# Intelligent-Microsystems-Lab/SNNQuantPrune

Measured on AMD Instinct MI355X. Metric: samples/sec/node (DVS128 T=20, 4-bit/90%-pruned), higher is better.
Workload: dtype fp6*fp4->f32 (integer-exact); 1 GPU; C3 topology: 3x(qconv3x3+BN+LIF+pool2) + qdense(32768->110)+LIF + vote, DVS128 128x128x2, T=20, bits 4/4/4/4, 90% pruned; batch_per_gpu=1024, global_batch=1024, frames=20, parallelism=dp1 (batch-sharded, all-gather logits)

## Files before the change

include/snnqp.h:

```cpp
#ifndef SNNQP_H_
#define SNNQP_H_

#include <stdint.h>

#ifdef __cplusplus
extern "C" {
#endif

typedef void *snnqp_stream_t;

enum {
  SNNQP_OK = 0,
  SNNQP_EINVAL = -1,
  SNNQP_EUNSUPPORTED = -2,
  SNNQP_EHIP = -3
};

enum { SNNQP_F32 = 0, SNNQP_U8 = 1, SNNQP_BITS = 2, SNNQP_EV1 = 3, SNNQP_EV4 = 4 };
enum { SNNQP_W_F32 = 0, SNNQP_W_I8 = 1 };
enum {
  SNNQP_NEURON_NONE = 0,
  SNNQP_NEURON_MULTI_STEP_LIF = 1,
  SNNQP_NEURON_PARAMETRIC_LEAKY_IF = 2,
  SNNQP_NEURON_LIF = 3
};
enum {
  SNNQP_SURR_FAST_SIGMOID = 0,
  SNNQP_SURR_ATAN = 1,
  SNNQP_SURR_SLAYER = 2,
  SNNQP_SURR_SMOOTH_STEP = 3,
  SNNQP_SURR_PIECEWISE_LINEAR = 4
};
enum {
  SNNQP_Q_DUQ = 0,
  SNNQP_Q_UNIFORM_STATIC = 1,
  SNNQP_Q_PARAMETRIC_D = 2,
  SNNQP_Q_PARAMETRIC_D_XMAX = 3
};
enum { SNNQP_IMPL_AUTO = 0, SNNQP_IMPL_GENERIC = 1, SNNQP_IMPL_MFMA = 2 };

enum {
  SNNQP_FLAG_CODE_OVERFLOW = 1,
  SNNQP_FLAG_MASK_NOT_BINARY = 2,
  SNNQP_FLAG_NOT_INTEGER = 4,
  SNNQP_FLAG_GT_ONE = 8,
  SNNQP_FLAG_GT_127 = 16,
  SNNQP_FLAG_GT_15 = 32
};

typedef struct {
  int32_t wtype;
  const void *w;
  float L;
  float m;
  int32_t abs_sum_max;
  int32_t code_max;
  const int32_t *col_sum;
  const void *wt_fp6;
  uint32_t min_current_bits;
  int32_t ch_stack_max;
  const int32_t *ch_slots;
  int32_t wt_cin;
} snnqp_weight_t;

#define SNNQP_BN_MEAN_ZERO 1
#define SNNQP_BN_BIAS_ZERO 2
#define SNNQP_BN_MUL_UNIFORM 4
typedef struct {
  const float *mean;
  const float *mul;
  const float *bias;
  int32_t flags;
} snnqp_bn_t;

typedef struct {
  int32_t kind;
  float k;
  float v_threshold;
  float v_reset;
  const float *decay;
} snnqp_neuron_t;

typedef struct {
  int32_t H, W, Cin, Cout;
  int32_t KH, KW;
  int32_t stride_h, stride_w;
  int32_t pad_h_lo, pad_h_hi, pad_w_lo, pad_w_hi;
  int32_t in_dil_h, in_dil_w;
  int32_t k_dil_h, k_dil_w;
  int32_t groups;
} snnqp_conv_geom_t;

typedef struct {
  int32_t D, H, W, Cin, Cout;
  int32_t KD, KH, KW;
  int32_t stride[3];
  int32_t pad_lo[3], pad_hi[3];
  int32_t in_dil[3];
  int32_t k_dil[3];
  int32_t groups;
} snnqp_conv3d_geom_t;

#define SNNQP_VERSION 505
int snnqp_version(void);
const char *snnqp_last_error(void);
const char *snnqp_build_flags(void);

int snnqp_conv_out_shape(const snnqp_conv_geom_t *g, int32_t *OH, int32_t *OW);

int snnqp_quantize(int kind, const float *w, const float *mask, int64_t n,
                   int bits, float p0, float p1, float *fq_out,
                   int8_t *codes_out, int32_t *flags, snnqp_stream_t stream);
int snnqp_quantize_ex(int kind, const float *w, const float *mask, int64_t n,
                      int bits, int sign, float p0, float p1, float *fq_out,
                      int8_t *codes_out, int32_t *flags, snnqp_stream_t stream);

int snnqp_pack_codes_mfma(const int8_t *w, int64_t K, int32_t N, int32_t Npad,
                          int8_t *wt, snnqp_stream_t stream);

int snnqp_pack_codes_fp6(const int8_t *w, int64_t K, int32_t N, int32_t Npad, void *wt6,
                         snnqp_stream_t stream);

int snnqp_inspect_f32(const float *x, int64_t n, int32_t *flags,
                      snnqp_stream_t stream);
int snnqp_inspect_u8(const uint8_t *x, int64_t n, int32_t *flags,
                     snnqp_stream_t stream);
int snnqp_f32_to_u8(const float *x, uint8_t *y, int64_t n,
                    snnqp_stream_t stream);
int snnqp_narrow_f32(const float *x, uint8_t *y, int64_t n, int32_t *flags,
                     snnqp_stream_t stream);
int snnqp_pack_frames(const uint8_t *x, int64_t frames, int32_t H, int32_t W, int fmt,
                      void *y, int32_t *flags, snnqp_stream_t stream);
int snnqp_unpack_frames(const void *x, int fmt, int64_t frames, int32_t H, int32_t W,
                        uint8_t *y, snnqp_stream_t stream);
int snnqp_pack_frames_checked(const void *x, int in_type, int64_t frames, int32_t H, int32_t W,
                              uint32_t *y, int32_t *flags, snnqp_stream_t stream);
int snnqp_pack_bits(const void *x, int in_type, int64_t rows, int32_t C,
                    uint32_t *bits, snnqp_stream_t stream);
int snnqp_pack_bits_checked(const void *x, int in_type, int64_t rows, int32_t C,
                            uint32_t *bits, int32_t *flags, snnqp_stream_t stream);
int snnqp_unpack_bits(const uint32_t *bits, int64_t rows, int32_t C, float *y,
                      snnqp_stream_t stream);

int snnqp_conv_forward(const void *x, int in_type, int64_t NB,
                       const snnqp_conv_geom_t *g, const snnqp_weight_t *w,
                       float *y, int32_t *acc, snnqp_stream_t stream);
int snnqp_conv_forward_if(const int32_t *pred, const void *x, int in_type, int64_t NB,
                          const snnqp_conv_geom_t *g, const snnqp_weight_t *w, float *y,
                          snnqp_stream_t stream);

int snnqp_conv3d_out_shape(const snnqp_conv3d_geom_t *g, int32_t *OD, int32_t *OH, int32_t *OW);
int snnqp_conv3d_lif_forward(const int32_t *pred, const void *x, int in_type, int64_t x_stride_t,
                             int64_t x_stride_b, int32_t T, int32_t B,
                             const snnqp_conv3d_geom_t *g, const snnqp_weight_t *w,
                             const snnqp_bn_t *bn, const snnqp_neuron_t *nrn, const float *u0,
                             float *u_out, void *s_out, int s_type, snnqp_stream_t stream);

int64_t snnqp_conv_gated_packed_bytes(int32_t Cin, int32_t Cout);
int snnqp_pack_codes_gated(const int8_t *w, int32_t Cin, int32_t Cout, void *packed,
                           snnqp_stream_t stream);
int64_t snnqp_conv_gated_packed_bytes_ex(int32_t Cin, int32_t Cout, int32_t code_max);
int snnqp_pack_codes_gated_ex(const int8_t *w, int32_t Cin, int32_t Cout, int32_t code_max,
                              void *packed, snnqp_stream_t stream);
int snnqp_conv_gated_forward(const uint32_t *s, const float *gate, int64_t NB,
                             const snnqp_conv_geom_t *g, const snnqp_weight_t *w,
                             const void *packed, float *y, snnqp_stream_t stream);

int64_t snnqp_dense_gated_packed_bytes(int32_t C, int32_t N);
int snnqp_pack_codes_dense_gated(const int8_t *w, int32_t C, int32_t HW, int32_t N, void *packed,
                                 snnqp_stream_t stream);
int64_t snnqp_dense_gated_packed_bytes_ex(int32_t C, int32_t N, int32_t code_max);
int snnqp_pack_codes_dense_gated_ex(const int8_t *w, int32_t C, int32_t HW, int32_t N, int32_t code_max,
                                    void *packed, snnqp_stream_t stream);
int snnqp_dense_gated_forward(const uint32_t *s, const float *gate, int64_t NB, int32_t HW,
                              int32_t C, int32_t N, const snnqp_weight_t *w,
                              const void *packed, float *y, snnqp_stream_t stream);

int snnqp_conv_lif_forward(const void *x, int in_type, int64_t x_stride_t,
                           int64_t x_stride_b, int32_t T, int32_t B,
                           const snnqp_conv_geom_t *g, const snnqp_weight_t *w,
                           const int8_t *wt, const snnqp_bn_t *bn,
                           const snnqp_neuron_t *nrn, const float *u0,
                           float *u_out, void *s_out, int s_type, int pool,
                           int impl, int x_max, int32_t *x_seen, int32_t *x_flags,
                           snnqp_stream_t stream);

int snnqp_conv_lif_forward_pred(const int32_t *pred, const void *x, int in_type, int64_t x_stride_t,
                                int64_t x_stride_b, int32_t T, int32_t B,
                                const snnqp_conv_geom_t *g, const snnqp_weight_t *w,
                                const int8_t *wt, const snnqp_bn_t *bn,
                                const snnqp_neuron_t *nrn, const float *u0,
                                float *u_out, void *s_out, int s_type, int pool,
                                int x_max, int32_t *x_seen, int32_t *x_flags,
                                snnqp_stream_t stream);

int snnqp_conv_lif_forward_if(const int32_t *pred, const void *x, int in_type, int64_t x_stride_t,
                              int64_t x_stride_b, int32_t T, int32_t B,
                              const snnqp_conv_geom_t *g, const snnqp_weight_t *w,
                              const snnqp_bn_t *bn, const snnqp_neuron_t *nrn, const float *u0,
                              float *u_out, void *s_out, int s_type, int pool,
                              snnqp_stream_t stream);

int snnqp_fallback_counts(int64_t *conv_blocks, int64_t *dense_blocks, char *reason,
                          int32_t reason_len, int reset);

#define SNNQP_STATUS_QUEUE_CORRUPT 1u
#define SNNQP_STATUS_TICKET 2u
#define SNNQP_STATUS_BOUND 4u
int snnqp_device_status(int device, uint32_t *codes, int reset);
int snnqp_workqueue_capture_mark(int device, int64_t *mark);
int snnqp_workqueue_capture_release(int device, int64_t mark_begin, int64_t mark_end);
int snnqp_workqueue_stats(int64_t *captured_static, int64_t *busy_static,
                          int64_t *dequant_fallbacks, int reset);
int snnqp_debug_workqueue_poke(int device, int64_t mark, int word, uint32_t value);

#define SNNQP_DQ_ARITH 1
#define SNNQP_DQ_ONE 2
#define SNNQP_DQ_TABLE 3
int snnqp_conv_dequant_form(const snnqp_weight_t *w, const snnqp_neuron_t *nrn);

int snnqp_current_min(const snnqp_weight_t *w, const snnqp_bn_t *bn, int32_t bound,
                      int32_t Cout, uint32_t *out_bits, snnqp_stream_t stream);

int snnqp_dense_lif_forward(const void *x, int in_type, int64_t x_stride_t,
                            int64_t x_stride_b, int32_t T, int32_t B, int32_t K,
                            int32_t N, const snnqp_weight_t *w,
                            const int8_t *wt, const snnqp_bn_t *bn,
                            const snnqp_neuron_t *nrn, const float *u0,
                            float *u_out, void *s_out, int s_type, int impl,
                            snnqp_stream_t stream);

int64_t snnqp_dense_workspace_bytes(int in_type, int32_t T, int32_t B, int32_t K, int32_t N,
                                    const snnqp_weight_t *w);
int snnqp_dense_lif_forward_ws(const void *x, int in_type, int64_t x_stride_t,
                               int64_t x_stride_b, int32_t T, int32_t B, int32_t K,
                               int32_t N, const snnqp_weight_t *w,
                               const int8_t *wt, const snnqp_bn_t *bn,
                               const snnqp_neuron_t *nrn, const float *u0,
                               float *u_out, void *s_out, int s_type, int impl,
                               int32_t *x_flags, void *ws, int64_t ws_bytes, snnqp_stream_t stream);
int snnqp_dense_lif_forward_if(const int32_t *pred, const void *x, int in_type, int64_t x_stride_t,
                               int64_t x_stride_b, int32_t T, int32_t B, int32_t K, int32_t N,
                               const snnqp_weight_t *w, const snnqp_bn_t *bn,
                               const snnqp_neuron_t *nrn, const float *u0, float *u_out,
                               void *s_out, int s_type, snnqp_stream_t stream);

int64_t snnqp_dense_head_workspace_bytes(int32_t T, int32_t B, int32_t N1);
int snnqp_dense_head_forward(const void *x, int in_type, int64_t x_stride_t,
                             int64_t x_stride_b, int32_t T, int32_t B, int32_t K,
                             int32_t N1, const snnqp_weight_t *w1, const int8_t *wt1,
                             const snnqp_neuron_t *nrn1, int32_t N2,
                             const snnqp_weight_t *w2, const int8_t *wt2,
                             const snnqp_neuron_t *nrn2, int32_t group,
                             uint32_t *s1_out, uint32_t *s2_out, float *logits,
                             int32_t *x_flags, void *ws, int64_t ws_bytes, snnqp_stream_t stream);

int snnqp_lif_forward(const float *x, int32_t T, int64_t R, int32_t C,
                      const snnqp_bn_t *bn, const snnqp_neuron_t *nrn,
                      const float *u0, float *u_out, void *s_out, int s_type,
                      snnqp_stream_t stream);

int snnqp_batchnorm_forward(const float *x, int64_t rows, int32_t C,
                            const snnqp_bn_t *bn, float *y,
                            snnqp_stream_t stream);

int snnqp_maxpool2x2(const void *x, int type, int64_t NB, int32_t H, int32_t W,
                     int32_t C, void *y, snnqp_stream_t stream);

int snnqp_spatial_mean(const void *x, int type, int64_t NB, int32_t HW, int32_t C,
                       float *y, snnqp_stream_t stream);
int snnqp_sigmoid_gate(const float *a, const float *b, int64_t n, float *g,
                       snnqp_stream_t stream);
int snnqp_apply_gate(const void *x, int type, const float *g, int64_t NB, int32_t HW,
                     int32_t C, float *y, snnqp_stream_t stream);

int snnqp_events_to_frames(const int32_t *ex, const int32_t *ey, const int32_t *ep,
                           int64_t N, int32_t T, int32_t H, int32_t W, float scale,
                           int32_t *counts, uint8_t *frames_u8, snnqp_stream_t stream);
int snnqp_density(const void *x, int type, int64_t NB, int64_t n, int32_t C, int32_t *nnz,
                  snnqp_stream_t stream);

int snnqp_vote(const void *s, int type, int32_t T, int32_t B, int32_t N,
               int32_t group, float *logits, snnqp_stream_t stream);
int snnqp_vote_if(const int32_t *pred, const void *s, int type, int32_t T, int32_t B, int32_t N,
                  int32_t group, float *logits, snnqp_stream_t stream);

int snnqp_scatter_spike_channels(const uint32_t *s, int64_t npix, int32_t cin, const int32_t *map,
                                 int32_t cout, uint32_t *out, snnqp_stream_t stream);

int snnqp_lif_forward_save(const float *x, int32_t T, int64_t R, int32_t C,
                           const snnqp_neuron_t *nrn, float *h_out, float *s_out,
                           snnqp_stream_t stream);
int snnqp_lif_backward(const float *h, const float *gs, const float *glogits, int32_t group,
                       int32_t T, int64_t R, int32_t C, const snnqp_neuron_t *nrn,
                       int surrogate, float *gI, snnqp_stream_t stream);
int snnqp_dense_weight_grad(const float *x, const float *gI, int64_t M, int32_t K, int32_t N,
                            float *gw, snnqp_stream_t stream);
int snnqp_dense_input_grad(const float *gI, const float *w, const float *mask, int64_t M,
                           int32_t K, int32_t N, float *gx, snnqp_stream_t stream);

#ifdef __cplusplus
}
#endif
#endif
```

snnquantprune_amd/_lib.py:

```python

from __future__ import annotations

import ctypes
import os
from ctypes import (POINTER, Structure, c_char_p, c_float, c_int, c_int8,
                    c_int32, c_uint32, c_int64, c_void_p)

_HERE = os.path.dirname(os.path.abspath(__file__))
LIB_PATH = os.path.join(_HERE, "csrc", "libsnnqp.so")

ABI_VERSION = 505

F32, U8, BITS, EV1, EV4 = 0, 1, 2, 3, 4
W_F32, W_I8 = 0, 1
NEURON_NONE, NEURON_MULTI_STEP_LIF, NEURON_PARAMETRIC_LEAKY_IF, NEURON_LIF = 0, 1, 2, 3
SURR_FAST_SIGMOID, SURR_ATAN, SURR_SLAYER, SURR_SMOOTH_STEP, SURR_PIECEWISE_LINEAR = 0, 1, 2, 3, 4
Q_DUQ, Q_UNIFORM_STATIC, Q_PARAMETRIC_D, Q_PARAMETRIC_D_XMAX = 0, 1, 2, 3
IMPL_AUTO, IMPL_GENERIC, IMPL_MFMA = 0, 1, 2
FLAG_CODE_OVERFLOW, FLAG_MASK_NOT_BINARY = 1, 2
FLAG_NOT_INTEGER, FLAG_GT_ONE, FLAG_GT_127, FLAG_GT_15 = 4, 8, 16, 32
OK, EINVAL, EUNSUPPORTED, EHIP = 0, -1, -2, -3
STATUS_QUEUE_CORRUPT, STATUS_TICKET, STATUS_BOUND = 1, 2, 4


class WeightT(Structure):
  _fields_ = [("wtype", c_int32), ("w", c_void_p), ("L", c_float), ("m", c_float),
              ("abs_sum_max", c_int32), ("code_max", c_int32), ("col_sum", c_void_p),
              ("wt_fp6", c_void_p), ("min_current_bits", c_uint32), ("ch_stack_max", c_int32),
              ("ch_slots", c_void_p), ("wt_cin", c_int32)]


BN_MEAN_ZERO, BN_BIAS_ZERO, BN_MUL_UNIFORM = 1, 2, 4


class BnT(Structure):
  _fields_ = [("mean", c_void_p), ("mul", c_void_p), ("bias", c_void_p), ("flags", c_int32)]


class NeuronT(Structure):
  _fields_ = [("kind", c_int32), ("k", c_float), ("v_threshold", c_float),
              ("v_reset", c_float), ("decay", c_void_p)]


class ConvGeomT(Structure):
  _fields_ = [(n, c_int32) for n in (
      "H", "W", "Cin", "Cout", "KH", "KW", "stride_h", "stride_w",
      "pad_h_lo", "pad_h_hi", "pad_w_lo", "pad_w_hi",
      "in_dil_h", "in_dil_w", "k_dil_h", "k_dil_w", "groups")]


class Conv3dGeomT(Structure):
  _fields_ = ([(n, c_int32) for n in ("D", "H", "W", "Cin", "Cout", "KD", "KH", "KW")]
              + [(n, c_int32 * 3) for n in ("stride", "pad_lo", "pad_hi", "in_dil", "k_dil")]
              + [("groups", c_int32)])


_PROTOTYPES = {
    "snnqp_version": (c_int, []),
    "snnqp_last_error": (c_char_p, []),
    "snnqp_build_flags": (c_char_p, []),
    "snnqp_conv_out_shape": (c_int, [POINTER(ConvGeomT), POINTER(c_int32),
                                     POINTER(c_int32)]),
    "snnqp_quantize": (c_int, [c_int, c_void_p, c_void_p, c_int64, c_int, c_float,
                               c_float, c_void_p, c_void_p, c_void_p, c_void_p]),
    "snnqp_quantize_ex": (c_int, [c_int, c_void_p, c_void_p, c_int64, c_int, c_int, c_float,
                                  c_float, c_void_p, c_void_p, c_void_p, c_void_p]),
    "snnqp_pack_codes_mfma": (c_int, [c_void_p, c_int64, c_int32, c_int32, c_void_p,
                                      c_void_p]),
    "snnqp_pack_codes_fp6": (c_int, [c_void_p, c_int64, c_int32, c_int32, c_void_p, c_void_p]),
    "snnqp_inspect_f32": (c_int, [c_void_p, c_int64, c_void_p, c_void_p]),
    "snnqp_inspect_u8": (c_int, [c_void_p, c_int64, c_void_p, c_void_p]),
    "snnqp_f32_to_u8": (c_int, [c_void_p, c_void_p, c_int64, c_void_p]),
    "snnqp_narrow_f32": (c_int, [c_void_p, c_void_p, c_int64, c_void_p, c_void_p]),
    "snnqp_pack_frames": (c_int, [c_void_p, c_int64, c_int32, c_int32, c_int, c_void_p, c_void_p,
                                  c_void_p]),
    "snnqp_unpack_frames": (c_int, [c_void_p, c_int, c_int64, c_int32, c_int32, c_void_p,
                                    c_void_p]),
    "snnqp_pack_bits": (c_int, [c_void_p, c_int, c_int64, c_int32, c_void_p,
                                c_void_p]),
    "snnqp_pack_bits_checked": (c_int, [c_void_p, c_int, c_int64, c_int32, c_void_p, c_void_p,
                                        c_void_p]),
    "snnqp_unpack_bits": (c_int, [c_void_p, c_int64, c_int32, c_void_p, c_void_p]),
    "snnqp_conv_forward": (c_int, [c_void_p, c_int, c_int64, POINTER(ConvGeomT),
                                   POINTER(WeightT), c_void_p, c_void_p, c_void_p]),
    "snnqp_conv_forward_if": (c_int, [c_void_p, c_void_p, c_int, c_int64, POINTER(ConvGeomT),
                                      POINTER(WeightT), c_void_p, c_void_p]),
    "snnqp_conv3d_out_shape": (c_int, [POINTER(Conv3dGeomT), POINTER(c_int32), POINTER(c_int32),
                                       POINTER(c_int32)]),
    "snnqp_conv3d_lif_forward": (c_int, [
        c_void_p, c_void_p, c_int, c_int64, c_int64, c_int32, c_int32, POINTER(Conv3dGeomT),
        POINTER(WeightT), POINTER(BnT), POINTER(NeuronT), c_void_p, c_void_p, c_void_p, c_int, c_void_p]),
    "snnqp_conv_gated_packed_bytes": (c_int64, [c_int32, c_int32]),
    "snnqp_pack_codes_gated": (c_int, [c_void_p, c_int32, c_int32, c_void_p, c_void_p]),
    "snnqp_conv_gated_packed_bytes_ex": (c_int64, [c_int32, c_int32, c_int32]),
    "snnqp_pack_codes_gated_ex": (c_int, [c_void_p, c_int32, c_int32, c_int32, c_void_p, c_void_p]),
    "snnqp_conv_gated_forward": (c_int, [c_void_p, c_void_p, c_int64, POINTER(ConvGeomT),
                                         POINTER(WeightT), c_void_p, c_void_p, c_void_p]),
    "snnqp_dense_gated_packed_bytes": (c_int64, [c_int32, c_int32]),
    "snnqp_pack_codes_dense_gated": (c_int, [c_void_p, c_int32, c_int32, c_int32, c_void_p, c_void_p]),
    "snnqp_dense_gated_packed_bytes_ex": (c_int64, [c_int32, c_int32, c_int32]),
    "snnqp_pack_codes_dense_gated_ex": (c_int, [c_void_p, c_int32, c_int32, c_int32, c_int32, c_void_p, c_void_p]),
    "snnqp_dense_gated_forward": (c_int, [c_void_p, c_void_p, c_int64, c_int32, c_int32, c_int32,
                                          POINTER(WeightT), c_void_p, c_void_p, c_void_p]),
    "snnqp_conv_lif_forward": (c_int, [
        c_void_p, c_int, c_int64, c_int64, c_int32, c_int32, POINTER(ConvGeomT),
        POINTER(WeightT), c_void_p, POINTER(BnT), POINTER(NeuronT), c_void_p,
        c_void_p, c_void_p, c_int, c_int, c_int, c_int, c_void_p, c_void_p, c_void_p]),
    "snnqp_conv_lif_forward_pred": (c_int, [
        c_void_p, c_void_p, c_int, c_int64, c_int64, c_int32, c_int32, POINTER(ConvGeomT),
        POINTER(WeightT), c_void_p, POINTER(BnT), POINTER(NeuronT), c_void_p,
        c_void_p, c_void_p, c_int, c_int, c_int, c_void_p, c_void_p, c_void_p]),
    "snnqp_pack_frames_checked": (c_int, [c_void_p, c_int, c_int64, c_int32, c_int32, c_void_p, c_void_p,
                                          c_void_p]),
    "snnqp_conv_lif_forward_if": (c_int, [
        c_void_p, c_void_p, c_int, c_int64, c_int64, c_int32, c_int32, POINTER(ConvGeomT),
        POINTER(WeightT), POINTER(BnT), POINTER(NeuronT), c_void_p, c_void_p, c_void_p, c_int, c_int,
        c_void_p]),
    "snnqp_dense_lif_forward_if": (c_int, [
        c_void_p, c_void_p, c_int, c_int64, c_int64, c_int32, c_int32, c_int32, c_int32,
        POINTER(WeightT), POINTER(BnT), POINTER(NeuronT), c_void_p, c_void_p, c_void_p, c_int,
        c_void_p]),
    "snnqp_dense_lif_forward": (c_int, [
        c_void_p, c_int, c_int64, c_int64, c_int32, c_int32, c_int32, c_int32,
        POINTER(WeightT), c_void_p, POINTER(BnT), POINTER(NeuronT), c_void_p,
        c_void_p, c_void_p, c_int, c_int, c_void_p]),
    "snnqp_dense_workspace_bytes": (c_int64, [c_int, c_int32, c_int32, c_int32, c_int32, POINTER(WeightT)]),
    "snnqp_dense_lif_forward_ws": (c_int, [
        c_void_p, c_int, c_int64, c_int64, c_int32, c_int32, c_int32, c_int32,
        POINTER(WeightT), c_void_p, POINTER(BnT), POINTER(NeuronT), c_void_p,
        c_void_p, c_void_p, c_int, c_int, c_void_p, c_void_p, c_int64, c_void_p]),
    "snnqp_dense_head_workspace_bytes": (c_int64, [c_int32, c_int32, c_int32]),
    "snnqp_dense_head_forward": (c_int, [
        c_void_p, c_int, c_int64, c_int64, c_int32, c_int32, c_int32, c_int32, POINTER(WeightT),
        c_void_p, POINTER(NeuronT), c_int32, POINTER(WeightT), c_void_p, POINTER(NeuronT), c_int32,
        c_void_p, c_void_p, c_void_p, c_void_p, c_void_p, c_int64, c_void_p]),
    "snnqp_device_status": (c_int, [c_int, POINTER(c_uint32), c_int]),
    "snnqp_workqueue_capture_mark": (c_int, [c_int, POINTER(c_int64)]),
    "snnqp_workqueue_capture_release": (c_int, [c_int, c_int64, c_int64]),
    "snnqp_workqueue_stats": (c_int, [POINTER(c_int64), POINTER(c_int64), POINTER(c_int64), c_int]),
    "snnqp_debug_workqueue_poke": (c_int, [c_int, c_int64, c_int, c_uint32]),
    "snnqp_fallback_counts": (c_int, [POINTER(c_int64), POINTER(c_int64), c_char_p, c_int32, c_int]),
    "snnqp_conv_dequant_form": (c_int, [POINTER(WeightT), POINTER(NeuronT)]),
    "snnqp_current_min": (c_int, [POINTER(WeightT), POINTER(BnT), c_int32, c_int32, c_void_p, c_void_p]),
    "snnqp_lif_forward": (c_int, [c_void_p, c_int32, c_int64, c_int32, POINTER(BnT),
                                  POINTER(NeuronT), c_void_p, c_void_p, c_void_p,
                                  c_int, c_void_p]),
    "snnqp_batchnorm_forward": (c_int, [c_void_p, c_int64, c_int32, POINTER(BnT),
                                        c_void_p, c_void_p]),
    "snnqp_maxpool2x2": (c_int, [c_void_p, c_int, c_int64, c_int32, c_int32, c_int32,
                                 c_void_p, c_void_p]),
    "snnqp_spatial_mean": (c_int, [c_void_p, c_int, c_int64, c_int32, c_int32, c_void_p,
                                   c_void_p]),
    "snnqp_sigmoid_gate": (c_int, [c_void_p, c_void_p, c_int64, c_void_p, c_void_p]),
    "snnqp_apply_gate": (c_int, [c_void_p, c_int, c_void_p, c_int64, c_int32, c_int32,
                                 c_void_p, c_void_p]),
    "snnqp_events_to_frames": (c_int, [c_void_p, c_void_p, c_void_p, c_int64, c_int32, c_int32,
                                       c_int32, c_float, c_void_p, c_void_p, c_void_p]),
    "snnqp_density": (c_int, [c_void_p, c_int, c_int64, c_int64, c_int32, c_void_p, c_void_p]),
    "snnqp_vote": (c_int, [c_void_p, c_int, c_int32, c_int32, c_int32, c_int32,
                           c_void_p, c_void_p]),
    "snnqp_vote_if": (c_int, [c_void_p, c_void_p, c_int, c_int32, c_int32, c_int32, c_int32,
                              c_void_p, c_void_p]),
    "snnqp_scatter_spike_channels": (c_int, [c_void_p, c_int64, c_int32, c_void_p, c_int32,
                                             c_void_p, c_void_p]),
    "snnqp_lif_forward_save": (c_int, [c_void_p, c_int32, c_int64, c_int32, POINTER(NeuronT),
                                       c_void_p, c_void_p, c_void_p]),
    "snnqp_lif_backward": (c_int, [c_void_p, c_void_p, c_void_p, c_int32, c_int32, c_int64,
                                   c_int32, POINTER(NeuronT), c_int, c_void_p, c_void_p]),
    "snnqp_dense_weight_grad": (c_int, [c_void_p, c_void_p, c_int64, c_int32, c_int32, c_void_p,
                                        c_void_p]),
    "snnqp_dense_input_grad": (c_int, [c_void_p, c_void_p, c_void_p, c_int64, c_int32, c_int32,
                                       c_void_p, c_void_p]),
}

EXPORTED_SYMBOLS = tuple(_PROTOTYPES)

_lib = None


class SnnqpError(RuntimeError):
  def __init__(self, code, msg):
    super().__init__("libsnnqp error %d: %s" % (code, msg))
    self.code = code


def lib():
  global _lib
  if _lib is None:
    path = os.environ.get("SNNQP_DIAG_LIB") or LIB_PATH
    if not os.path.exists(path):
      raise ImportError(
          "HIP extension %s not found: build it with `python __graft_entry__.py` "
          "(hipcc --offload-arch=gfx950); there is no CPU fallback." % path)
    import torch
    handle = ctypes.CDLL(path)
    if path != LIB_PATH:
      import sys
      print("snnquantprune_amd: DIAGNOSTIC library %s" % path, file=sys.stderr)
    for name, (res, args) in _PROTOTYPES.items():
      fn = getattr(handle, name)
      fn.restype = res
      fn.argtypes = args
    if handle.snnqp_version() != ABI_VERSION:
      raise ImportError(
          "%s has ABI version %d, this binding was written against %d (include/snnqp.h "
          "SNNQP_VERSION): rebuild it with `python __graft_entry__.py`"
          % (path, handle.snnqp_version(), ABI_VERSION))
    _lib = handle
  return _lib


def build_flags() -> str:
  return lib().snnqp_build_flags().decode("utf-8", "replace")


def require_product_build():
  flags = build_flags()
  if flags or os.environ.get("SNNQP_DIAG_LIB"):
    raise RuntimeError("libsnnqp is a diagnostic build (%s): rebuild with "
                       "`python snnquantprune_amd/csrc/build.py --force`" % (flags or "SNNQP_DIAG_LIB"))


def check(rc):
  if rc != 0:
    raise SnnqpError(rc, lib().snnqp_last_error().decode("utf-8", "replace"))
```

snnquantprune_amd/csrc/conv3x3_u8c2.hip:

```cpp
#include <atomic>
#include <map>
#include <mutex>
#include <tuple>
#include <type_traits>
#include <utility>

#include <vector>

#include "conv_tile.h"

namespace snnqp {

constexpr int HROW2 = 24;
constexpr int HCOPY2 = HALO * HROW2;
constexpr int HCONST2 = 2 * HCOPY2;
constexpr int HIMG2 = 496;
constexpr int TCHUNK = 32;
constexpr int U8C2_WPS = 4;
constexpr int STG_N = TCHUNK / 2;

typedef int v2i_a4 __attribute__((ext_vector_type(2), aligned(4)));
typedef __attribute__((address_space(3))) const v2i_a4 lds_cv2i_t;

__host__ __device__ inline int u8c2_table_bytes(int lutm, int bound, int rows) {
  const int b = lutm == LUT_CHANNEL ? rows * 128 : lutm == LUT_SHARED ? (2 * bound + 2) * 4 : 0;
  return (b + 15) & ~15;
}

#ifndef SNNQP_U8C2_EV1_WPS
#define SNNQP_U8C2_EV1_WPS 5
#endif
#ifndef SNNQP_U8C2_ONE_WPS
#define SNNQP_U8C2_ONE_WPS 4
#endif
#ifndef SNNQP_U8C2_EV1_ONE_WPS
#define SNNQP_U8C2_EV1_ONE_WPS 6
#endif
template <int NF, bool POOL, int LUTM, int IN, bool ONE>
constexpr int u8c2_waves() {
  if (IN == SNNQP_EV1 && ONE && LUTM == LUT_CHANNEL && NF == NF_MUL0 && POOL) return SNNQP_U8C2_EV1_ONE_WPS;
  if (IN == SNNQP_EV1) return SNNQP_U8C2_EV1_WPS;
  return ONE ? SNNQP_U8C2_ONE_WPS : U8C2_WPS;
}
template <int NF, bool POOL, int LUTM, int IN = SNNQP_U8, bool ONE = false>
__global__ void __launch_bounds__(256, (u8c2_waves<NF, POOL, LUTM, IN, ONE>()))
conv3x3_u8c2_kernel(ConvMfmaArgs a) {
  constexpr int FL = OutStage<POOL>::FL;
  constexpr bool EV1 = IN == SNNQP_EV1;
  constexpr bool EV4 = IN == SNNQP_EV4;
  constexpr bool F32IN = IN == SNNQP_F32;
  static_assert(TCHUNK % FL == 0, "flush period must divide the staging chunk");
  if constexpr (!EV1) {
    if (a.pred && *(const volatile int32_t *)a.pred == 0) return;
  }
  extern __shared__ __attribute__((aligned(16))) uint8_t lds[];
  const int tc = a.tchunk;
  const int lut_off = tc * HIMG2;
  uint32_t *obuf = (uint32_t *)(lds + lut_off + u8c2_table_bytes(LUTM, a.lut_bound, a.lut_rows));
  const int tid = threadIdx.x, lane = tid & 63;
  const int wave = __builtin_amdgcn_readfirstlane(tid >> 6);
  const int n = lane & 31, h = lane >> 5;
  const int cout_base = blockIdx.y * 128 + wave * 32;
  const bool wave_on = cout_base < a.Cout;
  const int cout = wave_on ? cout_base + n : n;
  const int cpar = cout < a.Cout ? cout : a.Cout - 1;
  const uint32_t cmask = chan_mask(cout_base, a.Cout);
  uint32_t *wgw = obuf + OutStage<POOL>::BYTES / 4;
  if (tid == 0) { wgw[0] = 0x7F800000u; wgw[1] = 0u; }
  typedef int v2i_a8 __attribute__((ext_vector_type(2)));
  v2i_a8 *xtab = (v2i_a8 *)(wgw + 4);
  if (EV1) {
    const uint32_t one = LUTM == LUT_CHANNEL ? 16u : LUTM == LUT_SHARED ? 4u : 0x81u;
    const uint32_t zero = LUTM == LUT_NONE ? 0x80u : 0u;
    uint32_t e[2] = {0, 0};
#pragma unroll
    for (int j = 0; j < 8; ++j) e[j >> 2] |= (((uint32_t)tid >> j) & 1u ? one : zero) << (8 * (j & 3));
    xtab[tid] = v2i_a8{(int)e[0], (int)e[1]};
  }
  if (LUTM != LUT_NONE) lds_barrier();
  if (LUTM == LUT_SHARED) {
    build_lut((float *)(lds + lut_off), a.lut_bound, a.dq, tid);
    if (NF == NF_MUL0) {
      lds_barrier();
      atomicMin(wgw, lut_bn_min_bits((const float *)(lds + lut_off), a.lut_bound, a.bn,
                                     blockIdx.y * 128, a.Cout, tid, 256));
    }
  }
  int ch_row0 = 0, ch_col = 0;
  if (LUTM == LUT_CHANNEL) {
    int pos = 0, neg = 0;
#pragma unroll
    for (int j = 0; j < 16; ++j) {
      const int k = 16 * h + j, dy = k >> 3, b = k & 7;
      if (k < 24 && b < 6 && wave_on && cout < a.Cout) {
        const int code = a.w[(int64_t)(6 * dy + b) * a.Cout + cout];
        pos += code > 0 ? code : 0;
        neg += code < 0 ? -code : 0;
      }
    }
    pos += __shfl_xor(pos, 32);
    neg += __shfl_xor(neg, 32);
    uint32_t *scr = obuf;
    int slot = 4 * n + wave;
    if (a.ch_slots) slot = a.ch_slots[blockIdx.y * 128 + wave * 32 + n] & 127;
    if (h == 0) {
      scr[slot] = (uint32_t)((pos + neg) * a.x_limit + 1);
      scr[128 + wave * 32 + n] = (uint32_t)(neg * a.x_limit);
      scr[256 + wave * 32 + n] = (uint32_t)slot;
    }
    lds_barrier();
    ch_col = slot >> 2;
    const int start = lut_column_start(scr, slot);
    int total = 0;
#pragma unroll
    for (int k = 0; k < 4; ++k) total += (int)scr[(slot & ~3) + k];
    ch_row0 = start + neg * a.x_limit;
    if (total > a.lut_rows && a.status) *(volatile uint32_t *)a.status = SNNQP_STATUS_BOUND;
    const uint32_t mb = build_lut_channel((float *)(lds + lut_off), scr, a.lut_rows, a.dq, a.bn,
                                          blockIdx.y * 128, a.Cout, tid);
    atomicMin(wgw, mb);
    lds_barrier();
  }
  if (tid < tc) {
    *(uint32_t *)(lds + tid * HIMG2 + HCONST2) = 0x7F7F7F7Fu;
    *(uint32_t *)(lds + tid * HIMG2 + HCONST2 + 4) = 0x00000001u;
  }

  float acc_off = 0.0f;
  v4i bf, bfg;
  {
    int bias = 0;
    if (LUTM == LUT_SHARED) bias = (int)lds_addr(lds) + lut_off + 4 * a.lut_bound;
    if (LUTM == LUT_CHANNEL)
      bias = (int)lds_addr(lds) + lut_off + 4 * (ch_row0 * 32 + ch_col);
    int q = bias / 127;
    const int r = bias - 127 * q;
    int wsum = 0;
    int v[4], vg[4];
#pragma unroll
    for (int d = 0; d < 4; ++d) {
      uint32_t pk = 0, pkg = 0;
#pragma unroll
      for (int j = 0; j < 4; ++j) {
        const int k = 16 * h + 4 * d + j;
        uint32_t bv = 0, bg = 0;
        if (k < 24) {
          const int dy = k >> 3, b = k & 7;
          if (b < 6 && cout < a.Cout) {
            const int code = a.w[(int64_t)(6 * dy + b) * a.Cout + cout];
            wsum += code;
            bg = (uint8_t)code;
            bv = (uint8_t)(LUTM == LUT_CHANNEL ? code * 8 : code);
          }
        } else if (k < 28) {
          const int part = q < 127 ? q : 127;
          q -= part;
          bv = (uint32_t)part;
        } else if (k == 28) {
          bv = (uint32_t)r;
        }
        pk |= bv << (8 * j);
        pkg |= bg << (8 * j);
      }
      v[d] = (int)pk;
      vg[d] = (int)pkg;
    }
    bf = v4i{v[0], v[1], v[2], v[3]};
    bfg = v4i{vg[0], vg[1], vg[2], vg[3]};
    acc_off = 128.0f * (float)(wsum + __shfl_xor(wsum, 32));
  }

  LaneConsts lc = {0.f, 1.f, 0.f, 0.f, a.nrn.vr};
  if (a.bn.mean) { lc.bmean = a.bn.mean[cpar]; lc.bmul = a.bn.mul[cpar]; lc.bbias = a.bn.bias[cpar]; }
  if (a.nrn.kind == SNNQP_NEURON_LIF) lc.dec = a.nrn.decay[cpar];

  const int ty = ((n >> 2) & 1) | ((n >> 4) << 1);
  const int tx = (n & 3) | (((n >> 3) & 1) << 2);
  const int cpy = tx & 1;
  const int px0 = (int)lds_addr(lds) + cpy * HCOPY2 + 2 * tx + 2 * cpy;
  int offA[2], offB[2];
#pragma unroll
  for (int tl = 0; tl < 2; ++tl) {
    offA[tl] = px0 + (ty + 4 * tl + (h ? 2 : 0)) * HROW2;
    offB[tl] = h ? (int)lds_addr(lds) + HCONST2 : px0 + (ty + 4 * tl + 1) * HROW2;
  }
  const uint8_t *xb = (const uint8_t *)a.x;
  const int ob0 = out_pix<POOL>(0, lane) * 4 + wave;
  const int ob1 = out_pix<POOL>(1, lane) * 4 + wave;
  const bool store_lane = POOL ? lane < 8 : lane < 32;
  uint32_t seen = 0;
  uint32_t hist[6] = {0, 0, 0, 0, 0, 0};
  const int s_pix = tid & 127;
  const bool s_task = s_pix < HALO * HALO;
  const int s_half = __builtin_amdgcn_readfirstlane(tid >> 7);
  const int s_dst = (s_pix / HALO) * HROW2 + (s_pix % HALO) * 2;

  PatchWalk pw(a);
  int r = __builtin_amdgcn_readfirstlane((int)pw.first);
  uint32_t processed = 0;
  while (r < (int)pw.count) {
    ++processed;
    int claimed = 0;
    if (pw.queue && tid == 0) claimed = (int)pw.claim();
    int b, y0, x0;
    pw.decode(a, r, b, y0, x0);

    float u[2][16];
    if constexpr (!ONE) {
      if (a.u0 && wave_on) u_io<true>(u, a, b, y0, x0, cout, h);
      else zero_u(u);
    }
    uint32_t pseen = 0;
    const int s_gy = y0 + s_pix / HALO - 1, s_gx = x0 + s_pix % HALO - 1;
    const bool s_valid = s_task && s_gy >= 0 && s_gy < a.H && s_gx >= 0 && s_gx < a.W;
    const uint32_t s_off = s_valid ? (uint32_t)(s_gy * a.W + s_gx) * (EV4 ? 1u : F32IN ? 8u : 2u) : 0u;
    const uint8_t *s_frames = xb + (int64_t)b * a.xs_b * (F32IN ? 4 : 1);
    const uint32_t e_lead = x0 > 0 ? 2u : 0u;
    const int e_hi = min(HALO - 1, a.W - x0);
    const uint32_t e_colmask = ((1u << (2 * (e_hi + 1))) - 1u) & ~((1u << (2 - (int)e_lead)) - 1u);
    const uint32_t e_fwords = (uint32_t)(((int64_t)a.H * a.W * 2 + 31) >> 5);
    const uint32_t *e_frames = (const uint32_t *)a.x + (int64_t)b * a.xs_b;

    for (int t0 = 0; t0 < a.T; t0 += tc) {
      const int nt = min(tc, a.T - t0);
      bool general = LUTM == LUT_NONE;
      if constexpr (EV1) {
        lds_barrier();
        for (int task = tid; task < nt * HALO; task += 256) {
          const int tt = task / HALO, hy = task - tt * HALO;
          const int gy = y0 + hy - 1;
          const bool rv = gy >= 0 && gy < a.H;
          const uint32_t start = (uint32_t)((rv ? gy : 0) * a.W + x0) * 2u - e_lead;
          const uint32_t wi = start >> 5;
          const uint32_t *f = e_frames + (int64_t)(t0 + tt) * a.xs_t;
          const uint32_t lo = f[wi], hi = f[min(wi + 1u, e_fwords - 1u)];
          uint32_t v = __builtin_amdgcn_alignbit(hi, lo, start & 31u);
          v = (v << (2u - e_lead)) & (rv ? e_colmask : 0u);
          const v2i_a8 d0 = xtab[v & 0xFFu], d1 = xtab[(v >> 8) & 0xFFu], d2 = xtab[(v >> 16) & 0xFu];
          uint8_t *row = lds + tt * HIMG2 + hy * HROW2;
          *(v2i_a8 *)row = d0;
          *(v2i_a8 *)(row + 8) = d1;
          *(v2i_a8 *)(row + 16) = d2;
          const uint32_t q0 = (uint32_t)d0.x, q1 = (uint32_t)d0.y, q2 = (uint32_t)d1.x,
                         q3 = (uint32_t)d1.y, q4 = (uint32_t)d2.x, q5 = (uint32_t)d2.y;
          uint8_t *row1 = row + HCOPY2;
          *(v2i_a8 *)row1 = v2i_a8{(int)(q0 << 16), (int)__builtin_amdgcn_alignbit(q1, q0, 16)};
          *(v2i_a8 *)(row1 + 8) = v2i_a8{(int)__builtin_amdgcn_alignbit(q2, q1, 16),
                                         (int)__builtin_amdgcn_alignbit(q3, q2, 16)};
          *(v2i_a8 *)(row1 + 16) = v2i_a8{(int)__builtin_amdgcn_alignbit(q4, q3, 16),
                                          (int)__builtin_amdgcn_alignbit(q5, q4, 16)};
        }
        lds_barrier();
      } else {
      uint32_t v[STG_N];
      uint32_t mx = 0;
      if constexpr (F32IN) {
        uint32_t fbad = 0;
#pragma unroll
        for (int r0 = 0; r0 < STG_N; r0 += STG_N / 2) {
          typedef float f2v __attribute__((ext_vector_type(2)));
          f2v raw[STG_N / 2];
#pragma unroll
          for (int i = r0; i < r0 + STG_N / 2; ++i) {
            const int tt = 2 * i + s_half;
            raw[i - r0] = f2v{0.0f, 0.0f};
            if (tt < nt) raw[i - r0] = *(const f2v *)(s_frames + (int64_t)(t0 + tt) * a.xs_t * 4 + s_off);
          }
#pragma unroll
          for (int i = r0; i < r0 + STG_N / 2; ++i) {
            const f2v f = raw[i - r0];
            const uint32_t ua = __float2uint_rz(f.x), ub = __float2uint_rz(f.y);
            fbad |= __float_as_uint(__uint2float_rn(ua) - f.x) | __float_as_uint(__uint2float_rn(ub) - f.y);
            fbad |= (ua | ub) >> 8;
            v[i] = (ua & 0xFFu) | ((ub & 0xFFu) << 8);
          }
        }
        fbad = s_valid ? fbad : 0u;
        if (__ballot(fbad != 0u) != 0ull && lane == 0 && a.x_flags) atomicOr(a.x_flags, SNNQP_FLAG_NOT_INTEGER);
      } else {
#pragma unroll
      for (int i = 0; i < STG_N; ++i) {
        const int tt = 2 * i + s_half;
        v[i] = 0;
        if (tt < nt) {
          if constexpr (EV4) {
            const uint32_t pb = *(s_frames + (int64_t)(t0 + tt) * a.xs_t + s_off);
            v[i] = (pb | (pb << 4)) & 0x0F0Fu;
          } else {
            v[i] = *(const uint16_t *)(s_frames + (int64_t)(t0 + tt) * a.xs_t + s_off);
          }
        }
      }
      }
#pragma unroll
      for (int i = 0; i < STG_N; ++i) {
        v[i] = s_valid ? v[i] : 0u;
        mx = max(mx, max(v[i] & 0xFFu, v[i] >> 8));
      }
#pragma unroll
      for (int off = 32; off > 0; off >>= 1) mx = max(mx, (uint32_t)__shfl_xor((int)mx, off));
      if (tid == 0) wgw[1] = 0u;
      lds_barrier();
      if (s_task) {
#pragma unroll
        for (int i = 0; i < STG_N; ++i) {
          const int tt = 2 * i + s_half;
          if (tt < nt) {
            const uint16_t val = (uint16_t)(LUTM == LUT_NONE      ? v[i] ^ 0x8080u
                                            : LUTM == LUT_CHANNEL ? v[i] << 4
                                                                  : v[i] << 2);
            uint8_t *p = lds + tt * HIMG2 + s_dst;
            *(uint16_t *)p = val;
            *(uint16_t *)(p + HCOPY2 + 2) = val;
          }
        }
      }
      if (lane == 0 && mx != 0) atomicMax(&wgw[1], mx);
      lds_barrier();
      const uint32_t cmax = (uint32_t)__builtin_amdgcn_readfirstlane((int)wgw[1]);
      seen = max(seen, cmax);
      pseen = max(pseen, cmax);
      hist[0] += cmax <= 1u;
      hist[1] += cmax == 2u;
      hist[2] += cmax > 2u && cmax <= 7u;
      hist[3] += cmax > 7u && cmax <= 31u;
      hist[4] += cmax > 31u;
      hist[5] += cmax == 3u;
      general = LUTM == LUT_NONE || cmax > (uint32_t)a.x_limit;
      if (LUTM != LUT_NONE && general) {
        if (s_task) {
#pragma unroll 1
          for (int tt = s_half; tt < nt; tt += 2) {
            uint32_t w2 = 0;
            if (s_valid) {
              if constexpr (F32IN) {
                typedef float f2v __attribute__((ext_vector_type(2)));
                const f2v f = *(const f2v *)(s_frames + (int64_t)(t0 + tt) * a.xs_t * 4 + s_off);
                w2 = (__float2uint_rz(f.x) & 0xFFu) | ((__float2uint_rz(f.y) & 0xFFu) << 8);
              } else if constexpr (EV4) {
                const uint32_t pb = *(s_frames + (int64_t)(t0 + tt) * a.xs_t + s_off);
                w2 = (pb | (pb << 4)) & 0x0F0Fu;
              } else {
                w2 = *(const uint16_t *)(s_frames + (int64_t)(t0 + tt) * a.xs_t + s_off);
              }
            }
            const uint16_t val = (uint16_t)(w2 ^ 0x8080u);
            uint8_t *p = lds + tt * HIMG2 + s_dst;
            *(uint16_t *)p = val;
            *(uint16_t *)(p + HCOPY2 + 2) = val;
          }
        }
        lds_barrier();
      }
      }
      auto run_chunk = [&](auto mode_tag, auto fma_tag) {
      constexpr int MODE = decltype(mode_tag)::value;
      constexpr bool FMA = decltype(fma_tag)::value;
      constexpr bool OFFS = MODE == LUT_NONE;
      const v4i bw = OFFS ? bfg : bf;
      for (int tf = 0; tf < nt; tf += FL) {
        const int nf = min(FL, nt - tf);
#pragma unroll 1
        for (int tt = tf; tt < (wave_on ? tf + nf : tf); ++tt) {
          const uint32_t img = (uint32_t)(tt * HIMG2);
          uint32_t words[2];
#pragma unroll
          for (int tl = 0; tl < 2; ++tl) {
            const v2i_a4 lo = *(lds_cv2i_t *)(uintptr_t)(img + (uint32_t)offA[0] + (uint32_t)(tl * 4 * HROW2));
            const v2i_a4 hi = *(lds_cv2i_t *)(uintptr_t)(img + (uint32_t)offB[tl]);
            v16i acc = splat16(0);
            acc = __builtin_amdgcn_mfma_i32_32x32x32_i8(v4i{lo.x, lo.y, hi.x, hi.y}, bw, acc,
                                                        0, 0, 0);
            if constexpr (u8c2_waves<NF, POOL, LUTM, IN, ONE>() >= 6)
              words[tl] = tile_epilogue_halves<NF, POOL, MODE, FMA, OFFS>(acc, u[tl], a.dq, lc, a.nrn,
                                                                            lane, acc_off);
            else
              words[tl] = tile_epilogue<NF, POOL, MODE, FMA, OFFS>(acc, u[tl], a.dq, lc, a.nrn,
                                                                     lane, acc_off);
          }
          if (store_lane) {
            uint32_t *o = obuf + ((t0 + tt) % FL) * (OutStage<POOL>::NPIX * 4);
            o[ob0] = words[0] & cmask;
            o[ob0 + (POOL ? 32 : 128)] = words[1] & cmask;
          }
        }
        lds_barrier();
        flush_out<POOL>(obuf, a, t0 + tf, nf, b, y0, x0, tid);
        lds_barrier();
      }
      };
      if constexpr (ONE) zero_u(u);
      if (general) {
        run_chunk(std::integral_constant<int, LUT_NONE>{}, std::false_type{});
      } else if constexpr (LUTM != LUT_NONE) {
        const bool fma_ok = NF == NF_MUL0 && pseen <= (uint32_t)a.x_limit &&
                            lif_fma_is_exact(wgw[0], a.nrn.k_log2, a.T, a.u0 != nullptr);
        if (fma_ok) run_chunk(std::integral_constant<int, LUTM>{}, std::true_type{});
        else run_chunk(std::integral_constant<int, LUTM>{}, std::false_type{});
      }
      if constexpr (ONE) break;
    }
    if (!ONE && a.u_out && wave_on) u_io<false>(u, a, b, y0, x0, cout, h);
    int r_next = r + (int)pw.stride;
    if (pw.queue) {
      if (tid == 0) wgw[2] = (uint32_t)claimed;
      lds_barrier();
      r_next = __builtin_amdgcn_readfirstlane((int)wgw[2]);
    }
    r = r_next;
  }
  if (a.x_seen && tid == 0) {
    if (seen != 0) atomicMax(a.x_seen, seen);
#pragma unroll
    for (int k = 0; k < 6; ++k)
      if (hist[k] != 0) atomicAdd((uint32_t *)a.x_seen + 1 + k, hist[k]);
  }
  if (pw.queue && tid == 0) pw.finish(processed, a.npatch, a.status);
}


__global__ void __launch_bounds__(256)
current_min_kernel(Dequant dq, BnP bn, int bound, int Cout, uint32_t *out) {
  const int c = blockIdx.x * 64 + (threadIdx.x & 63);
  uint32_t mb = 0x7F800000u;
  if (c < Cout) {
    float mean = 0.f, mul = 1.f, bias = 0.f;
    if (bn.mean) { mean = bn.mean[c]; mul = bn.mul[c]; bias = bn.bias[c]; }
    for (int i = (int)(threadIdx.x >> 6) + 4 * (int)blockIdx.y - bound; i <= bound; i += 4 * (int)gridDim.y) {
      float x = dequant_acc_nb(i, dq) - mean;
      x = x * mul;
      x = x + bias;
      const uint32_t b = __float_as_uint(x) & 0x7FFFFFFFu;
      if (b != 0 && b < mb) mb = b;
    }
  }
  for (int off = 32; off > 0; off >>= 1) {
    const uint32_t o = (uint32_t)__shfl_xor((int)mb, off);
    mb = o < mb ? o : mb;
  }
  if ((threadIdx.x & 63) == 0 && mb != 0x7F800000u) atomicMin(out, mb);
}

namespace {
struct SchedPool {
  uint32_t *words = nullptr;
  hipEvent_t busy[SCHED_SLOTS] = {};
  bool has_event[SCHED_SLOTS] = {};
  bool retired[SCHED_SLOTS] = {};
  unsigned next = 0;
  unsigned next_capture = 0;
  std::vector<int> capture_log;
  std::vector<int> capture_free;
};
std::atomic<int64_t> g_static_captured{0}, g_static_busy{0};
std::mutex g_sched_mu;
SchedPool g_sched[64];

struct DeviceGuard {
  int prev = -1;
  bool ok = true;
  explicit DeviceGuard(int dev) {
    int cur = -1;
    if (hipGetDevice(&cur) != hipSuccess) { (void)hipGetLastError(); ok = false; return; }
    if (cur == dev) return;
    if (hipSetDevice(dev) != hipSuccess) { (void)hipGetLastError(); ok = false; return; }
    prev = cur;
  }
  ~DeviceGuard() {
    if (prev >= 0 && hipSetDevice(prev) != hipSuccess) (void)hipGetLastError();
  }
};
}

uint32_t *sched_acquire(hipStream_t st, int *dev_out, int *slot_out) {
  int dev = 0;
  hipStreamCaptureStatus cap = hipStreamCaptureStatusNone;
  if (hipStreamIsCapturing(st, &cap) != hipSuccess) { (void)hipGetLastError(); return nullptr; }
  const bool capturing = cap != hipStreamCaptureStatusNone;
  hipDevice_t sdev;
  if (hipStreamGetDevice(st, &sdev) == hipSuccess) dev = (int)sdev;
  else if (hipGetDevice(&dev) != hipSuccess) return nullptr;
  if (dev < 0 || dev >= 64) return nullptr;
  std::lock_guard<std::mutex> lock(g_sched_mu);
  SchedPool &p = g_sched[dev];
  if (capturing) {
    if (!p.words) { g_static_captured.fetch_add(1, std::memory_order_relaxed); return nullptr; }
    int slot;
    if (!p.capture_free.empty()) {
      slot = p.capture_free.back();
      p.capture_free.pop_back();
    } else if (p.next_capture < (unsigned)SCHED_CAPTURE_SLOTS) {
      slot = SCHED_SLOTS + (int)p.next_capture++;
    } else {
      g_static_captured.fetch_add(1, std::memory_order_relaxed);
      return nullptr;
    }
    p.capture_log.push_back(slot);
    *dev_out = dev;
    *slot_out = slot;
    return p.words + (size_t)slot * SCHED_WORDS;
  }
  if (!p.words) {
    DeviceGuard on(dev);
    if (!on.ok) return nullptr;
    uint32_t *w = nullptr;
    if (hipMalloc((void **)&w, (size_t)(SCHED_SLOTS + SCHED_CAPTURE_SLOTS) * SCHED_WORDS *
                                   sizeof(uint32_t)) != hipSuccess) {
      (void)hipGetLastError();
      return nullptr;
    }
    if (hipMemset(w, 0, (size_t)(SCHED_SLOTS + SCHED_CAPTURE_SLOTS) * SCHED_WORDS * sizeof(uint32_t)) !=
        hipSuccess) {
      (void)hipGetLastError();
      (void)hipFree(w);
      return nullptr;
    }
    p.words = w;
  }
  const int slot = (int)(p.next++ % SCHED_SLOTS);
  if (p.retired[slot]) return nullptr;
  if (!p.has_event[slot]) {
    DeviceGuard on(dev);
    if (!on.ok || hipEventCreateWithFlags(&p.busy[slot], hipEventDisableTiming) != hipSuccess) {
      (void)hipGetLastError();
      p.retired[slot] = true;
      return nullptr;
    }
    p.has_event[slot] = true;
  } else if (hipEventQuery(p.busy[slot]) != hipSuccess) {
    (void)hipGetLastError();
    g_static_busy.fetch_add(1, std::memory_order_relaxed);
    return nullptr;
  }
  uint32_t *words = p.words + (size_t)slot * SCHED_WORDS;
  if (hipMemsetAsync(words, 0, SCHED_WORDS * sizeof(uint32_t), st) != hipSuccess) {
    (void)hipGetLastError();
    return nullptr;
  }
  *dev_out = dev;
  *slot_out = slot;
  return words;
}

void sched_release(int dev, int slot, hipStream_t st) {
  if (slot >= SCHED_SLOTS) return;
  std::lock_guard<std::mutex> lock(g_sched_mu);
  SchedPool &p = g_sched[dev];
  if (hipEventRecord(p.busy[slot], st) != hipSuccess) {
    (void)hipGetLastError();
    p.retired[slot] = true;
  }
}

int stream_device(hipStream_t st) {
  int dev = 0;
  hipDevice_t sdev;
  if (hipStreamGetDevice(st, &sdev) == hipSuccess) return (int)sdev;
  (void)hipGetLastError();
  if (hipGetDevice(&dev) != hipSuccess) { (void)hipGetLastError(); dev = 0; }
  return dev;
}

void persistent_limits(const void *kernel, int threads, size_t dyn_lds, int dev, int *cus_out,
                       int *occ_out) {
  typedef std::tuple<const void *, int, size_t, int> Key;
  static std::mutex mu;
  static std::map<Key, std::pair<int, int>> cache;
  const Key key(kernel, threads, dyn_lds, dev);
  std::lock_guard<std::mutex> lock(mu);
  auto it = cache.find(key);
  if (it == cache.end()) {
    int cus = 256, occ = 1;
    DeviceGuard on(dev);
    if (hipDeviceGetAttribute(&cus, hipDeviceAttributeMultiprocessorCount, dev) != hipSuccess) {
      (void)hipGetLastError();
      cus = 256;
    }
    if (hipOccupancyMaxActiveBlocksPerMultiprocessor(&occ, kernel, threads, dyn_lds) != hipSuccess) {
      (void)hipGetLastError();
      occ = 1;
    }
    if (occ < 1) occ = 1;
    if (occ > 8) occ = 8;
    it = cache.emplace(key, std::make_pair(cus, occ)).first;
  }
  *cus_out = it->second.first;
  *occ_out = it->second.second;
}

int run_current_min(const snnqp_weight_t *w, const snnqp_bn_t *bn, int32_t bound, int32_t Cout,
                    uint32_t *out_bits, hipStream_t st) {
  SNNQP_REQUIRE(w && out_bits && Cout > 0 && bound >= 0, SNNQP_EINVAL, "current_min: bad argument");
  SNNQP_REQUIRE(w->L >= 1.0f, SNNQP_EINVAL, "dequant L must be >= 1");
  SNNQP_CHECK_BN(bn);
  const int slices = bound >= 256 ? 16 : 1;
  hipLaunchKernelGGL(current_min_kernel, dim3((Cout + 63) / 64, slices), dim3(256), 0, st,
                     make_dequant(w->L, w->m), make_bn(bn), bound, Cout, out_bits);
  SNNQP_CHECK_LAUNCH("current_min_kernel");
  return SNNQP_OK;
}

const char *conv3x3_mfma_unsupported(int in_type, const snnqp_conv_geom_t *g,
                                     const snnqp_weight_t *w, const int8_t *wt,
                                     const snnqp_neuron_t *nrn, int s_type) {
  if (w->wtype != SNNQP_W_I8) return "weights are not int8 codes";
  if (g->KH != 3 || g->KW != 3) return "kernel is not 3x3";
  if (g->stride_h != 1 || g->stride_w != 1) return "stride is not 1";
  if (g->pad_h_lo != 1 || g->pad_h_hi != 1 || g->pad_w_lo != 1 || g->pad_w_hi != 1)
    return "padding is not ((1,1),(1,1))";
  if (g->in_dil_h != 1 || g->in_dil_w != 1 || g->k_dil_h != 1 || g->k_dil_w != 1)
    return "dilated convolution";
  if (g->groups != 1) return "grouped convolution";
  if (g->H <= 0 || g->W <= 0) return "empty image";
  if (g->Cout <= 0) return "no output channels";
  if (s_type != SNNQP_BITS) return "spike output must be bit-packed";
  if (in_type == SNNQP_BITS) {
    if (g->Cin < 1 || g->Cin > 128) return "bit input needs Cin <= 128";
  } else if (in_type == SNNQP_U8) {
    if (g->Cin != 2) return "u8 input needs Cin == 2";
    if ((int64_t)g->H * g->W * 2 >= (int64_t)1 << 31) return "u8 frame of 2 GiB or more";
  } else if (in_type == SNNQP_EV1) {
    if (g->Cin != 2) return "EV1 frames have Cin == 2";
    if ((int64_t)g->H * g->W * 2 >= (int64_t)1 << 31) return "EV1 frame of 2^31 bits or more";
  } else if (in_type == SNNQP_EV4) {
    if (g->Cin != 2) return "EV4 frames have Cin == 2";
    if ((int64_t)g->H * g->W >= (int64_t)1 << 31) return "EV4 frame of 2 GiB or more";
  } else if (in_type == SNNQP_F32) {
    if (g->Cin != 2) return "float32 input into integer codes needs Cin == 2";
    if ((int64_t)g->H * g->W * 8 >= (int64_t)1 << 31) return "float32 frame of 2 GiB or more";
  } else {
    return "input must be BITS, U8, EV1, EV4 or (Cin == 2) F32";
  }
  if (nrn->kind == SNNQP_NEURON_LIF && !nrn->decay) return "LIF without decay";
  if (in_type == SNNQP_BITS && !wt) return "MFMA-tiled codes `wt` not given";
  return nullptr;
}

int conv3x3_bits_dequant_form(const snnqp_weight_t *w, const snnqp_neuron_t *nrn) {
  if (w->L == 1.0f) return DQ_ONE;
  const bool fp6 = w->code_max > 0 && w->code_max <= 7;
  const bool tab = fp6 && neuron_form(make_neuron(nrn)) == NF_MUL0 && w->abs_sum_max > 0 &&
                   w->abs_sum_max <= DQT_MAXA;
  return tab ? DQ_TABLE : DQ_ARITH;
}

int run_conv3x3_mfma(const void *x, int in_type, int64_t xs_t, int64_t xs_b,
                     int32_t T, int32_t B, const snnqp_conv_geom_t *g,
                     const snnqp_weight_t *w, const int8_t *wt,
                     const snnqp_bn_t *bn, const snnqp_neuron_t *nrn,
                     const float *u0, float *u_out, uint32_t *s_out, int pool,
                     int x_max, int32_t *x_seen, int32_t *x_flags, hipStream_t st, const int32_t *pred) {
  SNNQP_REQUIRE(w->w && ((x && s_out) || T == 0 || B == 0), SNNQP_EINVAL, "conv3x3 mfma: null pointer");
  SNNQP_REQUIRE(!pred || in_type == SNNQP_U8 || in_type == SNNQP_F32 || in_type == SNNQP_EV4, SNNQP_EUNSUPPORTED,
                "conv3x3 mfma: only the event layer on byte / nibble / float32 frames takes a predicate");
  SNNQP_REQUIRE(in_type != SNNQP_BITS || wt, SNNQP_EINVAL,
                "conv3x3 mfma: bit input needs the MFMA-tiled codes `wt`");
  const int cin_pad = w->wt_cin ? w->wt_cin : (g->Cin + 31) / 32 * 32;
  SNNQP_REQUIRE(in_type != SNNQP_BITS || (cin_pad % 32 == 0 && cin_pad >= g->Cin && cin_pad <= 128),
                SNNQP_EINVAL, "conv3x3 mfma: wt_cin must be a multiple of 32 in [Cin, 128]");
  SNNQP_REQUIRE(T >= 0 && B >= 0, SNNQP_EINVAL, "conv3x3 mfma: negative T/B");
  SNNQP_REQUIRE(w->L >= 1.0f, SNNQP_EINVAL, "dequant L must be >= 1");
  SNNQP_CHECK_BN(bn);
  if (T == 0 || B == 0) return SNNQP_OK;
  SNNQP_REQUIRE((int64_t)B * ((g->H + 3) / 4) * ((g->W + 7) / 8) < ((int64_t)1 << 30),
                SNNQP_EUNSUPPORTED, "conv3x3 mfma: more than 2^30 patches in one launch");
  ConvMfmaArgs a;
  a.x = x; a.xs_t = xs_t; a.xs_b = xs_b; a.T = T; a.B = B;
  a.H = g->H; a.W = g->W; a.Cin = g->Cin; a.Cout = g->Cout;
  a.w = (const int8_t *)w->w;
  a.wt = wt;
  a.dq = make_dequant(w->L, w->m);
  a.bn = make_bn(bn);
  a.nrn = make_neuron(nrn);
  a.u0 = u0; a.u_out = u_out; a.s_out = s_out; a.pool = pool;
  a.x_seen = x_seen;
  a.x_flags = nullptr;
  a.pred = pred;
  if (in_type == SNNQP_F32) {
    SNNQP_REQUIRE(x_flags != nullptr && (((uintptr_t)x) & 7) == 0 && xs_t % 2 == 0 && xs_b % 2 == 0,
                  SNNQP_EINVAL, "conv3x3 mfma: float32 frames need x_flags and 8-byte aligned pixels");
    if (int rc = zero_words_async((uint32_t *)x_flags, 1, st)) return rc;
    a.x_flags = x_flags;
  }
  a.patch_h = 8;
  a.tiles_y = (g->H + 7) / 8; a.tiles_x = (g->W + 7) / 8;
  a.npatch = (int64_t)B * a.tiles_y * a.tiles_x;
  const int nf = neuron_form(a.nrn);
  const bool pl = pool == 2;
  const unsigned gy = (unsigned)((g->Cout + 127) / 128);
  const bool ev1 = in_type == SNNQP_EV1;
  const int64_t xm = (in_type == SNNQP_BITS || ev1) ? 1 : (x_max > 0 ? x_max : 1);
  a.x_limit = (int32_t)(xm > 255 ? 255 : xm);
  const int64_t bound = (int64_t)w->abs_sum_max * xm;
  const bool lut = w->abs_sum_max > 0 && xm > 0 && xm <= LUT_XMAX && bound <= LUT_CAP;
  a.lut_bound = lut ? (int32_t)bound : 0;
  a.tchunk = T >= TCHUNK ? TCHUNK : T;
  const size_t lds_fixed = (size_t)a.tchunk * HIMG2 + 16 + (ev1 ? 2048 : 0) +
                           (pl ? OutStage<true>::BYTES : OutStage<false>::BYTES);
  const int64_t stack = w->ch_stack_max > 0 ? (int64_t)w->ch_stack_max : 8 * (int64_t)w->abs_sum_max;
  const int64_t crows = stack * xm + 4;
  const bool lutc = lut && in_type != SNNQP_BITS && crows <= LUT2_ROWS && xm <= 7 &&
                    w->code_max > 0 && w->code_max <= 15;
  a.lut_rows = lutc ? (int32_t)crows : 0;
  a.ch_slots = lutc && w->ch_stack_max > 0 ? w->ch_slots : nullptr;
#define SNNQP_CONV_LAUNCH_IN(KERN, NFV, PL, LM, LDS)                               \
  do {                                                                             \
    if (ev1 && one) launch_persistent(KERN<NFV, PL, LM, SNNQP_EV1, true>, a, gy, st, LDS); \
    else if (ev1) launch_persistent(KERN<NFV, PL, LM, SNNQP_EV1>, a, gy, st, LDS);       \
    else if (in_type == SNNQP_EV4 && one) launch_persistent(KERN<NFV, PL, LM, SNNQP_EV4, true>, a, gy, st, LDS); \
    else if (in_type == SNNQP_EV4) launch_persistent(KERN<NFV, PL, LM, SNNQP_EV4>, a, gy, st, LDS); \
    else if (in_type == SNNQP_F32 && one) launch_persistent(KERN<NFV, PL, LM, SNNQP_F32, true>, a, gy, st, LDS); \
    else if (in_type == SNNQP_F32) launch_persistent(KERN<NFV, PL, LM, SNNQP_F32>, a, gy, st, LDS); \
    else if (one) launch_persistent(KERN<NFV, PL, LM, SNNQP_U8, true>, a, gy, st, LDS);            \
    else launch_persistent(KERN<NFV, PL, LM, SNNQP_U8>, a, gy, st, LDS);            \
  } while (0)
#define SNNQP_CONV_LAUNCH_NF(KERN, NFV, LM, LDS)                                   \
  do {                                                                             \
    if (pl) SNNQP_CONV_LAUNCH_IN(KERN, NFV, true, LM, LDS);                         \
    else SNNQP_CONV_LAUNCH_IN(KERN, NFV, false, LM, LDS);                           \
  } while (0)
#define SNNQP_CONV_LAUNCH(KERN, LM, LDS)                                           \
  do {                                                                             \
    if (nf == NF_MUL0) SNNQP_CONV_LAUNCH_NF(KERN, NF_MUL0, LM, LDS);                \
    else if (nf == NF_MUL) SNNQP_CONV_LAUNCH_NF(KERN, NF_MUL, LM, LDS);             \
    else if (nf == NF_DIV) SNNQP_CONV_LAUNCH_NF(KERN, NF_DIV, LM, LDS);             \
    else SNNQP_CONV_LAUNCH_NF(KERN, NF_DECAY, LM, LDS);                             \
  } while (0)
  if (in_type == SNNQP_BITS) {
    const bool fma = nf == NF_MUL0 && w->min_current_bits != 0 && w->abs_sum_max > 0 &&
                     lif_fma_is_exact(w->min_current_bits, a.nrn.k_log2, T, u0 != nullptr);
    const bool i8 = !(w->code_max > 0 && w->code_max <= 7);
    int dq = conv3x3_bits_dequant_form(w, nrn);
    if (dq == DQ_TABLE && !dq_table_trusted(stream_device(st), st)) dq = DQ_ARITH;
    const bool tab = dq == DQ_TABLE;
    const bool bnf = (a.bn.flags & (SNNQP_BN_MEAN_ZERO | SNNQP_BN_BIAS_ZERO)) ==
                     (SNNQP_BN_MEAN_ZERO | SNNQP_BN_BIAS_ZERO);
    a.lut_bound = tab ? (int32_t)w->abs_sum_max : 0;
    if (tab) check_code_bound_once(stream_device(st), (const int8_t *)w->w, (int64_t)9 * g->Cin, g->Cout,
                                   w->abs_sum_max, st);
    launch_conv3x3_bits(a, cin_pad, i8, nf, pl, dq, fma, bnf, gy, st);
  } else {
    const int lm = lutc ? LUT_CHANNEL : lut ? LUT_SHARED : LUT_NONE;
    if (lut) check_code_bound_once(stream_device(st), (const int8_t *)w->w, (int64_t)9 * g->Cin, g->Cout,
                                   w->abs_sum_max, st);
    const size_t lds_rest = lds_fixed - (size_t)a.tchunk * HIMG2 + u8c2_table_bytes(lm, a.lut_bound, a.lut_rows);
    for (int wgs = 4; wgs >= 2; --wgs) {
      const size_t per_wg = (size_t)(160 * 1024) / wgs - 512;
      int tc = a.tchunk;
      while (tc > 16 && (size_t)tc * HIMG2 + lds_rest > per_wg) tc -= 1;
      if ((size_t)tc * HIMG2 + lds_rest <= per_wg) {
        a.tchunk = tc;
        break;
      }
    }
    const size_t ldsb = (size_t)a.tchunk * HIMG2 + lds_rest;
    const bool one = !a.u0 && !a.u_out && a.T <= a.tchunk;
    if (lutc) SNNQP_CONV_LAUNCH(conv3x3_u8c2_kernel, LUT_CHANNEL, ldsb);
    else if (lut) SNNQP_CONV_LAUNCH(conv3x3_u8c2_kernel, LUT_SHARED, ldsb);
    else SNNQP_CONV_LAUNCH(conv3x3_u8c2_kernel, LUT_NONE, ldsb);
  }
#undef SNNQP_CONV_LAUNCH
#undef SNNQP_CONV_LAUNCH_NF
#undef SNNQP_CONV_LAUNCH_IN
  SNNQP_CHECK_LAUNCH("conv3x3 mfma kernel");
  return SNNQP_OK;
}

}

extern "C" int snnqp_workqueue_capture_mark(int device, int64_t *mark) {
  using namespace snnqp;
  SNNQP_REQUIRE(device >= 0 && device < 64 && mark, SNNQP_EINVAL, "workqueue_capture_mark: bad argument");
  std::lock_guard<std::mutex> lock(g_sched_mu);
  *mark = (int64_t)g_sched[device].capture_log.size();
  return SNNQP_OK;
}

extern "C" int snnqp_workqueue_capture_release(int device, int64_t mark_begin, int64_t mark_end) {
  using namespace snnqp;
  SNNQP_REQUIRE(device >= 0 && device < 64, SNNQP_EINVAL, "workqueue_capture_release: bad device");
  std::lock_guard<std::mutex> lock(g_sched_mu);
  SchedPool &p = g_sched[device];
  SNNQP_REQUIRE(0 <= mark_begin && mark_begin <= mark_end && mark_end <= (int64_t)p.capture_log.size(),
                SNNQP_EINVAL, "workqueue_capture_release: marks out of range");
  for (int64_t i = mark_begin; i < mark_end; ++i) {
    const int slot = p.capture_log[(size_t)i];
    if (slot < 0) continue;
    p.capture_free.push_back(slot);
    p.capture_log[(size_t)i] = -1;
  }
  return SNNQP_OK;
}

extern "C" int snnqp_workqueue_stats(int64_t *captured_static, int64_t *busy_static,
                                     int64_t *dequant_fallbacks, int reset) {
  using namespace snnqp;
  if (captured_static) *captured_static = g_static_captured.load(std::memory_order_relaxed);
  if (busy_static) *busy_static = g_static_busy.load(std::memory_order_relaxed);
  if (dequant_fallbacks) *dequant_fallbacks = dq_table_fallbacks(reset != 0);
  if (reset) { g_static_captured = 0; g_static_busy = 0; }
  return SNNQP_OK;
}

extern "C" int snnqp_debug_workqueue_poke(int device, int64_t mark, int word, uint32_t value) {
  using namespace snnqp;
  SNNQP_REQUIRE(device >= 0 && device < 64 && word >= 0 && word < SCHED_WORDS, SNNQP_EINVAL,
                "debug_workqueue_poke: bad argument");
  std::lock_guard<std::mutex> lock(g_sched_mu);
  SchedPool &p = g_sched[device];
  SNNQP_REQUIRE(p.words && mark >= 0 && mark < (int64_t)p.capture_log.size() && p.capture_log[(size_t)mark] >= 0,
                SNNQP_EINVAL, "debug_workqueue_poke: no live capture slot at mark %lld", (long long)mark);
  SNNQP_HIP(hipMemcpy(p.words + (size_t)p.capture_log[(size_t)mark] * SCHED_WORDS + word, &value, 4,
                      hipMemcpyHostToDevice));
  return SNNQP_OK;
}
```

snnquantprune_amd/csrc/conv_tile.h:

```cpp
#pragma once
#include "kernels.h"

namespace snnqp {


typedef int v4i __attribute__((ext_vector_type(4)));
typedef int v16i __attribute__((ext_vector_type(16)));
struct v2f {
  float x, y;
};
__device__ __forceinline__ v2f operator+(v2f a, v2f b) { return v2f{a.x + b.x, a.y + b.y}; }
__device__ __forceinline__ v2f operator-(v2f a, v2f b) { return v2f{a.x - b.x, a.y - b.y}; }
__device__ __forceinline__ v2f operator*(v2f a, v2f b) { return v2f{a.x * b.x, a.y * b.y}; }
__device__ __forceinline__ v2f operator+(v2f a, float b) { return v2f{a.x + b, a.y + b}; }
__device__ __forceinline__ v2f operator-(v2f a, float b) { return v2f{a.x - b, a.y - b}; }
__device__ __forceinline__ v2f operator*(v2f a, float b) { return v2f{a.x * b, a.y * b}; }
__device__ __forceinline__ v2f operator-(v2f a) { return v2f{-a.x, -a.y}; }
__device__ __forceinline__ v2f fma2(v2f a, v2f b, v2f c) {
  return v2f{__builtin_fmaf(a.x, b.x, c.x), __builtin_fmaf(a.y, b.y, c.y)};
}


enum { LUT_NONE = 0, LUT_SHARED = 1, LUT_CHANNEL = 2 };
constexpr int LUT_CAP = 4095;
constexpr int LUT2_ROWS = 256;
constexpr int LUT_XMAX = 31;

constexpr int HALO = 10;
constexpr int HPITCH = 12;
constexpr int HPLANE = HALO * HPITCH * 32;

struct ConvMfmaArgs {
  const void *x;
  int64_t xs_t, xs_b;
  int32_t T, B, H, W, Cin, Cout;
  const int8_t *w;
  const int8_t *wt;
  Dequant dq;
  BnP bn;
  NeuronP nrn;
  const float *u0;
  float *u_out;
  uint32_t *s_out;
  int32_t pool;
  int32_t tiles_y, tiles_x;
  int64_t npatch;
  int32_t lut_bound;
  int32_t lut_rows;
  const int32_t *ch_slots;
  int32_t x_limit;
  int32_t *x_seen;
  int32_t *x_flags;
  int32_t xcd_split;
  int32_t tchunk;
  uint32_t *sched;
  uint32_t *status;
  int32_t patch_h;
  const int32_t *pred;
};

constexpr int SCHED_Y = 8;
constexpr int SCHED_WORDS = SCHED_Y * 16;
constexpr int SCHED_SLOTS = 64;
constexpr int SCHED_CAPTURE_SLOTS = 960;

template <bool X4>
__device__ __forceinline__ v4i expand16(uint32_t b) {
  constexpr uint32_t MUL = X4 ? 0x00810204u : 0x00204081u;
  constexpr uint32_t AND = X4 ? 0x04040404u : 0x01010101u;
  v4i o;
  o.x = (int)((((b >> 0) & 0xFu) * MUL) & AND);
  o.y = (int)((((b >> 4) & 0xFu) * MUL) & AND);
  o.z = (int)((((b >> 8) & 0xFu) * MUL) & AND);
  o.w = (int)((((b >> 12) & 0xFu) * MUL) & AND);
  return o;
}

struct PatchWalk {
  int64_t first, count, stride;
  int ppb, xcd;
  bool split;
  uint32_t *queue;
  uint32_t *done;
  __device__ __forceinline__ explicit PatchWalk(const ConvMfmaArgs &a) {
    ppb = a.tiles_y * a.tiles_x;
    split = a.xcd_split != 0;
    if (split) {
      xcd = blockIdx.x & 7;
      first = blockIdx.x >> 3;
      stride = gridDim.x >> 3;
      count = (int64_t)((a.B - xcd + 7) >> 3) * ppb;
    } else {
      xcd = 0;
      first = blockIdx.x;
      stride = gridDim.x;
      count = a.npatch;
    }
    queue = a.sched ? a.sched + blockIdx.y * 16 + xcd : nullptr;
    done = a.sched ? a.sched + blockIdx.y * 16 + 8 : nullptr;
  }
  __device__ __forceinline__ int64_t claim() const {
    const int64_t r = stride + (int64_t)atomicAdd(queue, 1u);
    return r < count ? r : count;
  }
  __device__ __forceinline__ void finish(uint32_t processed, int64_t npatch, uint32_t *status) const {
    atomicAdd(done + 1, processed);
    __threadfence();
    const uint32_t total = gridDim.x;
    if (atomicAdd(done, 1u) + 1u == total) {
      __threadfence();
      const uint32_t tally = atomicAdd(done + 1, 0u);
      if (tally != (uint32_t)npatch && status) *(volatile uint32_t *)status = SNNQP_STATUS_QUEUE_CORRUPT;
      for (int i = 0; i < 8; ++i) done[i - 8] = 0u;
      done[1] = 0u;
      __threadfence();
      *done = 0u;
    }
  }
  __device__ __forceinline__ void decode(const ConvMfmaArgs &a, int64_t r, int &b, int &y0,
                                         int &x0) const {
    const int within = (int)(r % ppb);
    const int bi = (int)(r / ppb);
    b = split ? xcd + 8 * bi : bi;
    y0 = (within / a.tiles_x) * a.patch_h;
    x0 = (within % a.tiles_x) * 8;
  }
};

__device__ __forceinline__ void lds_barrier() {
  __builtin_amdgcn_fence(__ATOMIC_RELEASE, "workgroup", "local");
  __builtin_amdgcn_s_barrier();
  __builtin_amdgcn_fence(__ATOMIC_ACQUIRE, "workgroup", "local");
}

extern "C" __device__ uint32_t snnqp_writelane_i32(uint32_t, uint32_t, uint32_t)
    __asm("llvm.amdgcn.writelane.i32");
__device__ __forceinline__ uint32_t writelane_u32(uint32_t val, int lane, uint32_t old) {
  return snnqp_writelane_i32(val, (uint32_t)lane, old);
}

__device__ __forceinline__ float reset_where(float u, unsigned long long mask) {
  float r;
  asm("v_cndmask_b32_e64 %0, %1, 0, %2" : "=v"(r) : "v"(u), "s"(mask));
  return r;
}

struct LaneConsts {
  float bmean, bmul, bbias, dec;
  float vr;
};

__device__ __forceinline__ uint32_t chan_mask(int cout_base, int Cout) {
  const int valid = Cout - cout_base;
  return valid >= 32 ? 0xFFFFFFFFu : valid <= 0 ? 0u : (1u << valid) - 1u;
}

enum { NF_MUL0 = 1, NF_MUL = 2, NF_DIV = 3, NF_DECAY = 4 };

__host__ inline int neuron_form(const NeuronP &n) {
  if (n.kind == SNNQP_NEURON_LIF) return NF_DECAY;
  if (n.inv_k == 0.0f) return NF_DIV;
  return n.vr == 0.0f ? NF_MUL0 : NF_MUL;
}

typedef __attribute__((address_space(3))) const float lds_cfloat_t;
typedef __attribute__((address_space(3))) const uint8_t lds_cu8_t;
__device__ __forceinline__ uint32_t lds_addr(const void *p) {
  return (uint32_t)(uintptr_t)(lds_cu8_t *)p;
}
__device__ __forceinline__ float lds_read_f32(uint32_t addr) {
  return *(lds_cfloat_t *)(uintptr_t)addr;
}

__device__ __forceinline__ void build_lut(float *lut, int bound, const Dequant &dq,
                                          int tid, int nthreads = 256) {
  for (int i = tid; i <= 2 * bound; i += nthreads) lut[i] = dequant_acc_nb(i - bound, dq);
}

__device__ __forceinline__ int lut_column_start(const uint32_t *scr, int slot) {
  int st = 0;
  for (int k = 0; k < (slot & 3); ++k) st += (int)scr[(slot & ~3) + k];
  return st;
}
__device__ __forceinline__ uint32_t build_lut_channel(float *lut, const uint32_t *scr, int max_rows,
                                                      const Dequant &dq, const BnP &bn, int cout0,
                                                      int Cout, int tid) {
  uint32_t minbits = 0x7F800000u;
  const int c = tid & 127, hf = tid >> 7;
  const int slot = (int)scr[256 + c], col = slot >> 2;
  const int st = lut_column_start(scr, slot);
  const int rows = (int)scr[slot], negx = (int)scr[128 + c];
  if (st + rows > max_rows) return minbits;
  const int co = cout0 + c < Cout ? cout0 + c : Cout - 1;
  float bm = 0.f, bmul = 1.f, bb = 0.f;
  if (bn.mean) { bm = bn.mean[co]; bmul = bn.mul[co]; bb = bn.bias[co]; }
  for (int i = hf; i < rows; i += 2) {
    const float y = bn_apply(dequant_acc_nb(i - negx, dq), bm, bmul, bb);
    lut[(st + i) * 32 + col] = y;
    const uint32_t mag = __float_as_uint(y) & 0x7FFFFFFFu;
    if (mag != 0u && mag < minbits) minbits = mag;
  }
  return minbits;
}

__host__ __device__ __forceinline__ bool lif_fma_is_exact(uint32_t min_x_bits, int j, int T, bool has_u0) {
  if (has_u0 || j < 0) return false;
  const long long e = (long long)j * (T + 1) - 126;
  if (e > 100) return false;
  const uint32_t need = e <= -126 ? 0x00800000u : (uint32_t)(e + 127) << 23;
  return min_x_bits >= need;
}

__device__ __forceinline__ uint32_t lut_bn_min_bits(const float *lut, int bound, const BnP &bn,
                                                    int cout0, int Cout, int tid, int nthreads) {
  int c = cout0 + (tid & 127);
  if (c >= Cout) c = Cout - 1;
  float mean = 0.f, mul = 1.f, bias = 0.f;
  if (bn.mean) { mean = bn.mean[c]; mul = bn.mul[c]; bias = bn.bias[c]; }
  uint32_t mb = 0x7F800000u;
  for (int i = tid >> 7; i <= 2 * bound; i += nthreads >> 7) {
    float x = lut[i] - mean;
    x = x * mul;
    x = x + bias;
    const uint32_t b = __float_as_uint(x) & 0x7FFFFFFFu;
    if (b != 0 && b < mb) mb = b;
  }
  return mb;
}

template <int LUTM, bool OFFS = false>
__device__ __forceinline__ v2f dequant_pair(int a0, int a1, const Dequant &dq, float off = 0.0f) {
  if (LUTM != LUT_NONE) return v2f{lds_read_f32((uint32_t)a0), lds_read_f32((uint32_t)a1)};
  v2f a = {(float)a0, (float)a1};
  if (OFFS) a = a + off;
  const v2f q = fma2(a, v2f{dq.rL, dq.rL}, a * dq.rLlo);
  return q * dq.m;
}

template <int NF, bool FMA = false, bool PACKED = true>
__device__ __forceinline__ v2f neuron_update(v2f x, v2f u, const LaneConsts &lc,
                                             const NeuronP &nrn) {
  if (NF == NF_DECAY) {
    const v2f ud = u * lc.dec;
    return ud + x;
  }
  if (FMA && PACKED) {
    typedef float v2fp __attribute__((ext_vector_type(2)));
    const v2fp up = {u.x, u.y}, xp = {x.x, x.y};
    const v2fp dp = NF == NF_MUL0 ? xp - up : xp - (up - lc.vr);
    const v2fp r = __builtin_elementwise_fma(dp, v2fp{nrn.inv_k, nrn.inv_k}, up);
    return v2f{r.x, r.y};
  }
  const v2f d = NF == NF_MUL0 ? x - u : x - (u - lc.vr);
  if (NF == NF_DIV) return u + v2f{d.x / nrn.k, d.y / nrn.k};
  if (FMA) return fma2(d, v2f{nrn.inv_k, nrn.inv_k}, u);
  const v2f dk = d * nrn.inv_k;
  return u + dk;
}

template <int NF>
__device__ __forceinline__ float neuron_reset(float u, unsigned long long mask,
                                              const LaneConsts &lc) {
  if (NF == NF_MUL0) return reset_where(u, mask);
  float r;
  asm("v_cndmask_b32_e64 %0, %1, %2, %3" : "=v"(r) : "v"(u), "v"(lc.vr), "s"(mask));
  return r;
}

template <int NF, bool BNDONE, bool FMA = false>
__device__ __forceinline__ void neuron_pair(v2f y, float &u0, float &u1,
                                            const LaneConsts &lc, const NeuronP &nrn,
                                            unsigned long long &m0,
                                            unsigned long long &m1) {
  v2f x = y;
  if (!BNDONE) {
    x = x - lc.bmean;
    x = x * lc.bmul;
    x = x + lc.bbias;
  }
  const v2f uu = neuron_update<NF, FMA>(x, v2f{u0, u1}, lc, nrn);
  m0 = __ballot(uu.x >= nrn.vth);
  m1 = __ballot(uu.y >= nrn.vth);
  u0 = neuron_reset<NF>(uu.x, m0, lc);
  u1 = neuron_reset<NF>(uu.y, m1, lc);
}

template <int NF, bool POOL, bool BNDONE, bool FMA = false>
__device__ __forceinline__ uint32_t tile_neurons(const v2f (&y)[8], float (&u)[16],
                                                 const LaneConsts &lc, const NeuronP &nrn) {
  uint32_t myw = 0;
#pragma unroll
  for (int i = 0; i < 16; i += 2) {
    unsigned long long m0, m1;
    neuron_pair<NF, BNDONE, FMA>(y[i >> 1], u[i], u[i + 1], lc, nrn, m0, m1);
    if (POOL) {
      const unsigned long long o = m0 | m1;
      const uint32_t pw = (uint32_t)o | (uint32_t)(o >> 32);
      myw = writelane_u32(pw, i >> 1, myw);
    } else {
      const int r0 = (i & 3) + 8 * (i >> 2);
      myw = writelane_u32((uint32_t)m0, r0, myw);
      myw = writelane_u32((uint32_t)(m0 >> 32), r0 + 4, myw);
      myw = writelane_u32((uint32_t)m1, r0 + 1, myw);
      myw = writelane_u32((uint32_t)(m1 >> 32), r0 + 5, myw);
    }
  }
  return myw;
}

template <int NF, bool POOL, int LUTM, bool FMA = false, bool OFFS = false>
__device__ __forceinline__ uint32_t tile_epilogue(const v16i &acc, float (&u)[16],
                                                  const Dequant &dq,
                                                  const LaneConsts &lc,
                                                  const NeuronP &nrn, int lane,
                                                  float off = 0.0f) {
  v2f y[8];
#pragma unroll
  for (int j = 0; j < 8; ++j) y[j] = dequant_pair<LUTM, OFFS>(acc[2 * j], acc[2 * j + 1], dq, off);
  return tile_neurons<NF, POOL, LUTM == LUT_CHANNEL, FMA>(y, u, lc, nrn);
}

template <int NF, bool POOL, int LUTM, bool FMA = false, bool OFFS = false>
__device__ __forceinline__ uint32_t tile_epilogue_halves(const v16i &acc, float (&u)[16],
                                                         const Dequant &dq, const LaneConsts &lc,
                                                         const NeuronP &nrn, int lane, float off = 0.0f) {
  uint32_t myw = 0;
#pragma unroll
  for (int g = 0; g < 2; ++g) {
    v2f y[4];
#pragma unroll
    for (int j = 0; j < 4; ++j) y[j] = dequant_pair<LUTM, OFFS>(acc[8 * g + 2 * j], acc[8 * g + 2 * j + 1], dq, off);
#pragma unroll
    for (int j = 0; j < 4; ++j) {
      const int i = 8 * g + 2 * j;
      unsigned long long m0, m1;
      neuron_pair<NF, LUTM == LUT_CHANNEL, FMA>(y[j], u[i], u[i + 1], lc, nrn, m0, m1);
      if (POOL) {
        const unsigned long long o = m0 | m1;
        const uint32_t pw = (uint32_t)o | (uint32_t)(o >> 32);
        myw = writelane_u32(pw, i >> 1, myw);
      } else {
        const int r0 = (i & 3) + 8 * (i >> 2);
        myw = writelane_u32((uint32_t)m0, r0, myw);
        myw = writelane_u32((uint32_t)(m0 >> 32), r0 + 4, myw);
        myw = writelane_u32((uint32_t)m1, r0 + 1, myw);
        myw = writelane_u32((uint32_t)(m1 >> 32), r0 + 5, myw);
      }
    }
    __builtin_amdgcn_sched_barrier(0);
  }
  return myw;
}

template <bool POOL>
struct OutStage {
  static constexpr int NPIX = POOL ? 16 : 64;
  static constexpr int FL = POOL ? 32 : 8;
  static constexpr int BYTES = FL * NPIX * 16;
};

template <bool POOL>
__device__ __forceinline__ int out_pix(int tl, int lane) {
  if (POOL) return (tl * 2 + ((lane >> 2) & 1)) * 4 + (lane & 3);
  const int ty = ((lane >> 2) & 1) | (((lane >> 4) & 1) << 1);
  const int tx = (lane & 3) | (((lane >> 3) & 1) << 2);
  return (tl * 4 + ty) * 8 + tx;
}

template <bool POOL, int SLOTS, int NT, int NPIX = OutStage<POOL>::NPIX>
__device__ __forceinline__ void flush_ring(const uint32_t *obuf, const ConvMfmaArgs &a,
                                           int t0, int n, int b, int y0, int x0, int tid) {
  constexpr int PW = POOL ? 4 : 8;
  const int CW = (a.Cout + 31) >> 5;
  const int cwb = blockIdx.y * 4;
  const int nw = min(4, CW - cwb);
  const int OH = POOL ? a.H >> 1 : a.H, OW = POOL ? a.W >> 1 : a.W;
  const int oy0 = POOL ? y0 >> 1 : y0, ox0 = POOL ? x0 >> 1 : x0;
  for (int i = tid; i < n * NPIX; i += NT) {
    const int slot = i / NPIX, pix = i % NPIX;
    const int t = t0 + slot;
    const uint32_t *src = obuf + ((t % SLOTS) * NPIX + pix) * 4;
    const int oy = oy0 + pix / PW, ox = ox0 + pix % PW;
    if (oy >= OH || ox >= OW) continue;
    uint32_t *dst = a.s_out + ((((int64_t)t * a.B + b) * OH + oy) * OW + ox) * CW + cwb;
    if (nw == 4 && (CW & 3) == 0) {
      *(v4i *)dst = *(const v4i *)src;
    } else {
      for (int w = 0; w < nw; ++w) dst[w] = src[w];
    }
  }
}

template <bool POOL>
__device__ __forceinline__ void flush_out(const uint32_t *obuf, const ConvMfmaArgs &a,
                                          int t0, int n, int b, int y0, int x0, int tid) {
  flush_ring<POOL, OutStage<POOL>::FL, 256>(obuf, a, t0, n, b, y0, x0, tid);
}

template <bool LOAD>
__device__ __forceinline__ void u_io_tile(float (&u)[16], const ConvMfmaArgs &a, int b,
                                          int y0, int x0, int cout, int h, int tl) {
  float *uo = a.u_out;
  const float *ui = a.u0;
#pragma unroll
  for (int i = 0; i < 16; ++i) {
    const int y = y0 + tl * 4 + (h | ((i >> 3) << 1));
    const int x = x0 + (i & 7);
    const int64_t o = (((int64_t)b * a.H + y) * a.W + x) * a.Cout + cout;
    const bool in = y < a.H && x < a.W && cout < a.Cout;
    if (LOAD) u[i] = in ? ui[o] : 0.0f;
    else if (in) uo[o] = u[i];
  }
}

template <bool LOAD>
__device__ __forceinline__ void u_io(float (&u)[2][16], const ConvMfmaArgs &a,
                                     int b, int y0, int x0, int cout, int h) {
  float *uo = a.u_out;
  const float *ui = a.u0;
#pragma unroll
  for (int tl = 0; tl < 2; ++tl)
#pragma unroll
    for (int i = 0; i < 16; ++i) {
      const int y = y0 + tl * 4 + (h | ((i >> 3) << 1));
      const int x = x0 + (i & 7);
      const int64_t o = (((int64_t)b * a.H + y) * a.W + x) * a.Cout + cout;
      const bool in = y < a.H && x < a.W && cout < a.Cout;
      if (LOAD) u[tl][i] = in ? ui[o] : 0.0f;
      else if (in) uo[o] = u[tl][i];
    }
}

__device__ __forceinline__ void zero_u(float (&u)[2][16]) {
#pragma unroll
  for (int tl = 0; tl < 2; ++tl)
#pragma unroll
    for (int i = 0; i < 16; ++i) u[tl][i] = 0.0f;
}

__device__ __forceinline__ v16i splat16(int v) {
  return v16i{v, v, v, v, v, v, v, v, v, v, v, v, v, v, v, v};
}

uint32_t *sched_acquire(hipStream_t st, int *dev, int *slot);
void sched_release(int dev, int slot, hipStream_t st);
uint32_t *device_status_word(int dev);

void persistent_limits(const void *kernel, int threads, size_t dyn_lds, int dev, int *cus, int *occ);
int stream_device(hipStream_t st);

template <typename K>
static inline void launch_persistent(K kernel, ConvMfmaArgs a, unsigned gy, hipStream_t st,
                                     size_t dyn_lds = 0, int threads = 256) {
  int dev = 0, cus = 256, occ = 2, slot = -1;
  a.sched = gy <= (unsigned)SCHED_Y ? sched_acquire(st, &dev, &slot) : nullptr;
  if (!a.sched) dev = stream_device(st);
  a.status = a.sched ? device_status_word(dev) : nullptr;
  persistent_limits((const void *)kernel, threads, dyn_lds, dev, &cus, &occ);
  const int64_t gmax = (int64_t)cus * occ;
  unsigned gx = (unsigned)(a.npatch < gmax ? a.npatch : gmax);
  a.xcd_split = 0;
  if (gx >= 64 && a.B >= 8) {
    gx &= ~7u;
    a.xcd_split = 1;
  }
  hipLaunchKernelGGL(kernel, dim3(gx, gy), dim3(threads), dyn_lds, st, a);
  if (a.sched) sched_release(dev, slot, st);
}

enum { DQ_ARITH = 1, DQ_ONE = 2, DQ_TABLE = 3 };
constexpr int DQT_MAXA = 2047;
void launch_conv3x3_bits(const ConvMfmaArgs &a, int cin_pad, bool i8, int nf, bool pool, int dq,
                         bool fma, bool bnf, unsigned gy, hipStream_t st);

}
```

snnquantprune_amd/linen.py:

```python

from __future__ import annotations

import dataclasses
import functools
import hashlib
import math
import threading
from collections.abc import MutableMapping
from typing import Any, Callable, Dict, Iterable, Optional, Sequence

import torch

_tls = threading.local()


def _stack():
  if not hasattr(_tls, "stack"):
    _tls.stack = []
  return _tls.stack


class ConfigDict(MutableMapping):

  def __init__(self, *args, **kwargs):
    object.__setattr__(self, "_d", {})
    for k, v in dict(*args, **kwargs).items():
      self[k] = v

  def __getitem__(self, k):
    return self._d[k]

  def __setitem__(self, k, v):
    if isinstance(v, dict):
      v = ConfigDict(v)
    self._d[k] = v

  def __delitem__(self, k):
    del self._d[k]

  def __iter__(self):
    return iter(self._d)

  def __len__(self):
    return len(self._d)

  def __contains__(self, k):
    return k in self._d

  def __getattr__(self, k):
    try:
      return self._d[k]
    except KeyError:
      raise AttributeError(k)

  def __setattr__(self, k, v):
    self[k] = v

  def __delattr__(self, k):
    del self._d[k]

  def __hash__(self):
    return id(self)

  def __eq__(self, other):
    return self is other

  def __repr__(self):
    return "ConfigDict(%r)" % (self._d,)

  def to_dict(self):
    return {k: (v.to_dict() if isinstance(v, ConfigDict) else v)
            for k, v in self._d.items()}


FrozenConfigDict = ConfigDict



_DTYPE_POLICY = "strict"
_dtype_warned = False


def set_compute_dtype_policy(policy: str):
  global _DTYPE_POLICY
  if policy not in ("strict", "float32"):
    raise ValueError("compute dtype policy must be 'strict' or 'float32'")
  _DTYPE_POLICY = policy


_CHANNEL_COMPACTION = True


def set_channel_compaction(enabled: bool):
  global _CHANNEL_COMPACTION
  _CHANNEL_COMPACTION = bool(enabled)


def channel_compaction() -> bool:
  return _CHANNEL_COMPACTION


_CONV_KPACK = True


def set_conv_kpack(enabled: bool):
  global _CONV_KPACK
  _CONV_KPACK = bool(enabled)


def conv_kpack() -> bool:
  return _CONV_KPACK


def check_compute_dtype(dtype, who: str):
  global _dtype_warned
  if dtype in (torch.float32, None, "float32"):
    return
  if _DTYPE_POLICY == "float32":
    if not _dtype_warned:
      import sys
      print("snnquantprune_amd: %s asked for %r; computing in float32 (nn.set_compute_dtype_policy)"
            % (who, dtype), file=sys.stderr)
      _dtype_warned = True
    return
  raise NotImplementedError(
      "%s computes in float32 (got %r); nn.set_compute_dtype_policy('float32') runs such a "
      "request in float32 instead of refusing it" % (who, dtype))




def _default_device():
  return torch.device("cuda") if torch.cuda.is_available() else torch.device("cpu")


def zeros(key, shape, dtype=torch.float32):
  return torch.zeros(tuple(shape), dtype=dtype, device=_default_device())


def ones(key, shape, dtype=torch.float32):
  return torch.ones(tuple(shape), dtype=dtype, device=_default_device())


def constant(value):
  def init(key, shape, dtype=torch.float32):
    return torch.full(tuple(shape), float(value), dtype=dtype, device=_default_device())
  return init


def lecun_normal():
  def init(key, shape, dtype=torch.float32):
    shape = tuple(shape)
    fan_in = 1
    for d in shape[:-1]:
      fan_in *= d
    std = math.sqrt(1.0 / max(fan_in, 1)) / 0.87962566103423978
    w = torch.empty(shape, dtype=torch.float32)
    torch.nn.init.trunc_normal_(w, mean=0.0, std=std, a=-2 * std, b=2 * std,
                                generator=key)
    return w.to(dtype).to(_default_device())
  return init


class Variable:
  def __init__(self, module, col, name):
    self._m, self._col, self._name = module, col, name

  @property
  def value(self):
    return self._m._get(self._col, self._name)

  @value.setter
  def value(self, v):
    root = self._m._root
    if not (root.initializing or self._col in root.mutable):
      raise RuntimeError("collection %r is immutable" % self._col)
    self._m._set(self._col, self._name, v)


class _Root:
  def __init__(self, variables, mutable, initializing, rngs):
    self.variables = variables
    self.mutable = set(mutable)
    self.initializing = initializing
    self.rngs = rngs
    self.rng_count = 0


def _seed_of(rngs, name):
  key = None
  if isinstance(rngs, dict):
    key = rngs.get(name, rngs.get("params"))
  else:
    key = rngs
  if key is None:
    return 0
  if isinstance(key, torch.Generator):
    return key.initial_seed()
  if isinstance(key, torch.Tensor):
    return int(key.reshape(-1)[0].item())
  return int(key)


class Module:

  name: Optional[str] = dataclasses.field(default=None, kw_only=True)

  def __init_subclass__(cls, **kw):
    super().__init_subclass__(**kw)
    if "__call__" in cls.__dict__:
      cls.__call__ = _wrap_call(cls.__dict__["__call__"])
    dataclasses.dataclass(cls, eq=False, repr=False)

  def __post_init__(self):
    object.__setattr__(self, "_parent", None)
    object.__setattr__(self, "_root", None)
    object.__setattr__(self, "_path", None)
    object.__setattr__(self, "_autoname", {})
    st = _stack()
    if st:
      self._adopt(st[-1], None)

  def _adopt(self, parent, attr_name):
    name = self.name or attr_name
    if name is None:
      base = type(self).__name__
      idx = parent._autoname.get(base, 0)
      parent._autoname[base] = idx + 1
      name = "%s_%d" % (base, idx)
    object.__setattr__(self, "_parent", parent)
    object.__setattr__(self, "_root", parent._root)
    object.__setattr__(self, "_path", parent._path + (name,))

  def _bind_root(self, root):
    object.__setattr__(self, "_parent", None)
    object.__setattr__(self, "_root", root)
    object.__setattr__(self, "_path", ())

  @property
  def is_bound(self):
    return self._root is not None

  def _node(self, col, create):
    d = self._root.variables
    if col not in d:
      if not create:
        return None
      d[col] = {}
    d = d[col]
    for p in self._path:
      if p not in d:
        if not create:
          return None
        d[p] = {}
      d = d[p]
    return d

  def _get(self, col, name):
    node = self._node(col, False)
    if node is None or name not in node:
      raise KeyError("no variable %s/%s/%s" % (col, "/".join(self._path), name))
    return node[name]

  def _set(self, col, name, value):
    self._node(col, True)[name] = value

  def has_variable(self, col, name):
    node = self._node(col, False)
    return node is not None and name in node

  def make_rng(self, name="params"):
    root = self._root
    root.rng_count += 1
    h = hashlib.sha256(("%d/%s/%s/%d" % (_seed_of(root.rngs, name), name,
                                         "/".join(self._path), root.rng_count)
                        ).encode()).digest()
    g = torch.Generator()
    g.manual_seed(int.from_bytes(h[:8], "little") & ((1 << 63) - 1))
    return g

  def param(self, name, init_fn, *init_args):
    if not self.is_bound:
      raise RuntimeError("module %s is not bound; use init()/apply()" % type(self).__name__)
    if not self.has_variable("params", name):
      if not self._root.initializing:
        raise KeyError("parameter %s/%s not found in variables" %
                       ("/".join(self._path), name))
      self._set("params", name, init_fn(self.make_rng("params"), *init_args))
    return self._get("params", name)

  def variable(self, col, name, init_fn=None, *init_args):
    if not self.has_variable(col, name):
      if not (self._root.initializing or col in self._root.mutable):
        raise KeyError("variable %s/%s/%s not found" % (col, "/".join(self._path), name))
      self._set(col, name, init_fn(*init_args) if init_fn is not None else None)
    return Variable(self, col, name)

  def is_mutable_collection(self, col):
    return self._root.initializing or col in self._root.mutable

  def sow(self, col, name, value):
    if not self.is_bound or not (col in self._root.mutable):
      return False
    node = self._node(col, True)
    node[name] = tuple(node.get(name, ())) + (value,)
    return True

  def init(self, rngs, *args, **kwargs):
    root = _Root({}, mutable=(), initializing=True, rngs=rngs)
    return self._run(root, args, kwargs)[1]

  def init_with_output(self, rngs, *args, **kwargs):
    root = _Root({}, mutable=(), initializing=True, rngs=rngs)
    return self._run(root, args, kwargs)

  def apply(self, variables, *args, rngs=None, mutable=False, **kwargs):
    if mutable is True:
      mcols = set(variables.keys()) | {"intermediates"}
    elif not mutable:
      mcols = set()
    elif isinstance(mutable, str):
      mcols = {mutable}
    else:
      mcols = set(mutable)
    vars_copy = {c: (_copy_tree(v) if c in mcols else v) for c, v in variables.items()}
    root = _Root(vars_copy, mutable=mcols, initializing=False, rngs=rngs)
    out, allvars = self._run(root, args, kwargs)
    if mutable:
      return out, {c: allvars.get(c, {}) for c in mcols if c in allvars}
    return out

  def _run(self, root, args, kwargs):
    saved = (self._parent, self._root, self._path)
    st = _stack()
    saved_stack = list(st)
    del st[:]
    self._bind_root(root)
    try:
      out = self(*args, **kwargs)
    finally:
      object.__setattr__(self, "_parent", saved[0])
      object.__setattr__(self, "_root", saved[1])
      object.__setattr__(self, "_path", saved[2])
      st[:] = saved_stack
    return out, root.variables

  def __repr__(self):
    fs = ", ".join("%s=%r" % (f.name, getattr(self, f.name))
                   for f in dataclasses.fields(self)
                   if f.name != "name" and not isinstance(getattr(self, f.name), Module))
    return "%s(%s)" % (type(self).__name__, fs)


dataclasses.dataclass(Module, eq=False, repr=False)


def _copy_tree(t):
  if isinstance(t, dict):
    return {k: _copy_tree(v) for k, v in t.items()}
  return t


def _wrap_call(fn):
  @functools.wraps(fn)
  def wrapped(self, *args, **kwargs):
    st = _stack()
    if not self.is_bound:
      if not st:
        raise RuntimeError(
            "%s called outside init()/apply(): modules are stateless, use "
            "module.apply(variables, ...)" % type(self).__name__)
      parent = st[-1]
      attr = None
      for f in dataclasses.fields(parent):
        if getattr(parent, f.name, None) is self:
          attr = f.name
          break
      self._adopt(parent, attr)
    elif st and self._root is not st[-1]._root:
      parent = st[-1]
      object.__setattr__(self, "_root", parent._root)
    self._autoname.clear()
    st.append(self)
    try:
      return fn(self, *args, **kwargs)
    finally:
      st.pop()
  return wrapped


def compact(fn):
  return fn


compact_method = _wrap_call



from ._cache import TensorCache

_bn_cache = TensorCache(256)


class BatchNorm(Module):
  use_running_average: Optional[bool] = None
  axis: int = -1
  momentum: float = 0.99
  epsilon: float = 1e-5
  dtype: Any = torch.float32
  use_bias: bool = True
  use_scale: bool = True

  @compact_method
  def coeffs(self, features: int):
    from . import ops
    import numpy as np
    feat = (int(features),)
    mean = self.variable("batch_stats", "mean", lambda: zeros(None, feat)).value
    var = self.variable("batch_stats", "var", lambda: ones(None, feat)).value
    scale = self.param("scale", ones, feat) if self.use_scale else None
    bias = self.param("bias", zeros, feat) if self.use_bias else None
    hit = _bn_cache.get((mean, var, scale, bias), float(self.epsilon))
    if hit is not None:
      return hit
    dev = mean.device
    m = mean.detach().cpu().numpy().astype(np.float32)
    v = var.detach().cpu().numpy().astype(np.float32)
    mul = np.float32(1) / np.sqrt(v + np.float32(self.epsilon))
    if scale is not None:
      mul = mul * scale.detach().cpu().numpy().astype(np.float32)
    b = (bias.detach().cpu().numpy().astype(np.float32) if bias is not None
         else np.zeros_like(m))
    from . import _lib as L
    flags = (0 if m.any() else L.BN_MEAN_ZERO) | (0 if b.any() else L.BN_BIAS_ZERO)
    mul32 = mul.astype(np.float32)
    if mul32.size and np.all(mul32.view(np.uint32) == mul32.view(np.uint32).flat[0]) and np.isfinite(mul32.flat[0]):
      flags |= L.BN_MUL_UNIFORM
    out = ops.BnCoeffs(torch.from_numpy(m).to(dev),
                       torch.from_numpy(mul.astype(np.float32)).to(dev),
                       torch.from_numpy(b).to(dev), flags)
    return _bn_cache.put((mean, var, scale, bias), float(self.epsilon), out)

  def __call__(self, x, use_running_average: Optional[bool] = None):
    from . import ops
    ura = self.use_running_average if use_running_average is None else use_running_average
    if ura is None:
      raise ValueError("BatchNorm needs use_running_average")
    if not ura:
      raise NotImplementedError(
          "BatchNorm batch statistics (training mode) are out of scope: this "
          "package implements the eval forward pass")
    if self.axis not in (-1, x.ndim - 1):
      raise NotImplementedError("BatchNorm over a non-last axis")
    return ops.batchnorm_forward(x, self.coeffs(x.shape[-1]))




class CapturedApply:

  def __init__(self, module, variables, example, **kwargs):
    from . import ops
    self._ops = ops
    dev = example.device if not isinstance(example, torch.Tensor) else example.device
    if torch.device(dev).type != "cuda":
      raise RuntimeError("capture needs the inputs on the GPU")
    self.static_input = self._clone(example)
    self._stream = torch.cuda.Stream(device=dev)
    self._graph = torch.cuda.CUDAGraph()
    cur = torch.cuda.current_stream(dev)
    self._stream.wait_stream(cur)
    self._device = torch.device(dev)
    self._slots = None
    with torch.cuda.stream(self._stream):
      for _ in range(2):
        module.apply(variables, self.static_input, **kwargs)
      self._stream.synchronize()
      mark = ops.workqueue_capture_mark(self._device)
      self._workspaces, outer = [], ops._CAPTURE_KEEP
      ops._CAPTURE_KEEP = self._workspaces
      try:
        with torch.cuda.graph(self._graph, stream=self._stream):
          self.static_output = module.apply(variables, self.static_input, **kwargs)
      finally:
        ops._CAPTURE_KEEP = outer
        self._slots = (mark, ops.workqueue_capture_mark(self._device))
    cur.wait_stream(self._stream)

  def close(self):
    slots, self._slots = self._slots, None
    if slots is None or slots[0] == slots[1]:
      self._graph = None
      return
    try:
      torch.cuda.synchronize(self._device)
      self._graph = None
      self._ops.workqueue_capture_release(self._device, slots[0], slots[1])
    except Exception:
      pass

  def __del__(self):
    self.close()

  def _clone(self, x):
    ops = self._ops
    if isinstance(x, ops.PackedFrames):
      return ops.PackedFrames(x.data.clone(), x.H, x.W, x.fmt)
    if isinstance(x, ops.PackedSpikes):
      return ops.PackedSpikes(x.bits.clone(), x.channels)
    return x.clone()

  def _raw(self, x):
    ops = self._ops
    return x.data if isinstance(x, ops.PackedFrames) else x.bits if isinstance(x, ops.PackedSpikes) else x

  def __call__(self, inputs=None):
    if inputs is not None and inputs is not self.static_input:
      src, dst = self._raw(inputs), self._raw(self.static_input)
      if src.shape != dst.shape or src.dtype != dst.dtype:
        raise ValueError("captured for inputs %s %s, got %s %s"
                         % (tuple(dst.shape), dst.dtype, tuple(src.shape), src.dtype))
      dst.copy_(src, non_blocking=True)
    if self._graph is None:
      raise RuntimeError("this CapturedApply has been closed")
    self._graph.replay()
    return self.static_output


def capture(module, variables, example, **kwargs) -> CapturedApply:
  return CapturedApply(module, variables, example, **kwargs)




def tree_map(fn, tree):
  if isinstance(tree, dict):
    return {k: tree_map(fn, v) for k, v in tree.items()}
  if isinstance(tree, (tuple, list)):
    return type(tree)(tree_map(fn, v) for v in tree)
  return fn(tree)


def tree_to_device(tree, device):
  return tree_map(lambda x: x.to(device) if isinstance(x, torch.Tensor) else x, tree)


def tree_from_numpy(tree, device=None):
  import numpy as np
  device = device or _default_device()
  return tree_map(lambda x: torch.as_tensor(np.asarray(x)).to(device)
                  if not isinstance(x, torch.Tensor) else x.to(device), tree)
```

snnquantprune_amd/ops.py:

```python

from __future__ import annotations

import ctypes
from dataclasses import dataclass
from typing import Optional, Sequence, Tuple

import torch

from . import _lib as L




class PackedSpikes:

  def __init__(self, bits: torch.Tensor, channels: int):
    assert bits.dtype == torch.int32 and bits.is_contiguous()
    assert bits.shape[-1] == (channels + 31) // 32
    self.bits = bits
    self.channels = int(channels)
    self.flat_perm = None
    self.chan_map = None

  @property
  def shape(self):
    return tuple(self.bits.shape[:-1]) + (self.channels,)

  @property
  def device(self):
    return self.bits.device

  @property
  def ndim(self):
    return self.bits.ndim

  def __getitem__(self, idx):
    if not isinstance(idx, tuple):
      idx = (idx,)
    assert len(idx) < self.bits.ndim, "cannot index the packed channel axis"
    out = PackedSpikes(self.bits[idx].contiguous(), self.channels)
    out.chan_map = self.chan_map
    return out

  def reshape_leading(self, *lead):
    out = PackedSpikes(self.bits.reshape(*lead, self.bits.shape[-1]), self.channels)
    out.chan_map = self.chan_map
    return out

  def to_dense(self) -> torch.Tensor:
    return unpack_bits(self)

  def __repr__(self):
    return "PackedSpikes(shape=%s, device=%s)" % (self.shape, self.device)


class PackedFrames:

  def __init__(self, data: torch.Tensor, H: int, W: int, fmt: int):
    assert fmt in (L.EV1, L.EV4), fmt
    unit = frame_units(H, W, fmt)
    assert data.dtype == (torch.int32 if fmt == L.EV1 else torch.uint8), data.dtype
    assert data.shape[-1] == unit and data.is_contiguous(), (tuple(data.shape), unit)
    self.data, self.H, self.W, self.fmt = data, int(H), int(W), int(fmt)

  @property
  def shape(self):
    return tuple(self.data.shape[:-1]) + (self.H, self.W, 2)

  @property
  def device(self):
    return self.data.device

  @property
  def ndim(self):
    return self.data.ndim + 2

  @property
  def dtype(self):
    return torch.uint8

  @property
  def is_cuda(self):
    return self.data.is_cuda

  def __getitem__(self, idx):
    if not isinstance(idx, tuple):
      idx = (idx,)
    assert len(idx) < self.data.ndim, "cannot index inside a packed frame"
    return PackedFrames(self.data[idx].contiguous(), self.H, self.W, self.fmt)

  def narrow(self, dim, start, length):
    assert dim < self.data.ndim - 1
    return PackedFrames(self.data.narrow(dim, start, length).contiguous(), self.H, self.W, self.fmt)

  def to(self, device, non_blocking=False):
    return PackedFrames(self.data.to(device, non_blocking=non_blocking), self.H, self.W, self.fmt)

  def to_u8(self) -> torch.Tensor:
    return unpack_frames(self)

  def __repr__(self):
    return "PackedFrames(%s, shape=%s, device=%s)" % (
        "EV1" if self.fmt == L.EV1 else "EV4", self.shape, self.device)


class GatedSpikes:

  def __init__(self, spikes: "PackedSpikes", gate: torch.Tensor, flat: bool = False):
    assert isinstance(spikes, PackedSpikes) and spikes.ndim == 5, "spikes [T, B, H, W, C], bit-packed"
    assert gate.dtype == torch.float32 and tuple(gate.shape) == (spikes.shape[0], spikes.shape[1], spikes.channels)
    self.spikes, self.gate = spikes, gate.contiguous()
    self.flat = bool(flat)

  @property
  def shape(self):
    if self.flat:
      T, B, H, W, C = self.spikes.shape
      return (T, B, C * H * W)
    return self.spikes.shape

  @property
  def ndim(self):
    return 3 if self.flat else 5

  @property
  def device(self):
    return self.spikes.device

  def flattened(self) -> "GatedSpikes":
    return GatedSpikes(self.spikes, self.gate, flat=True)

  def to_dense(self) -> torch.Tensor:
    x = apply_gate(self.spikes, self.gate)
    if self.flat:
      x = x.permute(0, 1, 4, 2, 3)
      x = x.reshape(x.shape[0], x.shape[1], x.shape[2] * x.shape[3] * x.shape[4]).contiguous()
    return x


class ChannelMap:

  def __init__(self, index, live, full: int):
    import numpy as np
    self.index = np.asarray(index, np.int64)
    self.live = np.asarray(live, bool)
    self.full = int(full)
    self._dev = {}

  def device_index(self, device) -> torch.Tensor:
    key = str(device)
    t = self._dev.get(key)
    if t is None:
      t = self._dev[key] = torch.from_numpy(self.index.astype("int32")).to(device)
    return t

  def __repr__(self):
    return "ChannelMap(%d of %d, %d live)" % (self.index.size, self.full, int(self.live.sum()))


def scatter_spike_channels(s: "PackedSpikes", channel_map: torch.Tensor, cout: int) -> "PackedSpikes":
  bits = s.bits.contiguous()
  _require_gpu(bits, channel_map)
  assert channel_map.dtype == torch.int32 and channel_map.numel() == s.channels
  cw = (int(cout) + 31) // 32
  npix = bits.numel() // max(bits.shape[-1], 1) if bits.ndim else 0
  out = torch.empty(tuple(bits.shape[:-1]) + (cw,), dtype=torch.int32, device=bits.device)
  L.check(L.lib().snnqp_scatter_spike_channels(_ptr(bits), npix, s.channels,
                                                _ptr(channel_map.contiguous()), int(cout), _ptr(out),
                                                _stream()))
  return PackedSpikes(out, int(cout))


def expand_channels(x):
  cm = getattr(x, "chan_map", None)
  if cm is None:
    return x
  flat = x.flat_perm
  if flat is not None:
    c, h, w = flat
    lead = tuple(x.bits.shape[:-1])
    blk = PackedSpikes(x.bits.reshape(*lead, h, w, c // 32).contiguous(), c)
    full = scatter_spike_channels(blk, cm.device_index(x.device), cm.full)
    out = PackedSpikes(full.bits.reshape(*lead, h * w * ((cm.full + 31) // 32)), h * w * cm.full)
    out.flat_perm = (cm.full, h, w)
    return out
  return scatter_spike_channels(x, cm.device_index(x.device), cm.full)


def frame_units(H: int, W: int, fmt: int) -> int:
  return (H * W * 2 + 31) // 32 if fmt == L.EV1 else H * W


def pack_frames_host(x, fmt: int) -> PackedFrames:
  import numpy as np
  a = x.numpy() if isinstance(x, torch.Tensor) else np.asarray(x)
  if a.dtype != np.uint8 or a.ndim < 3 or a.shape[-1] != 2:
    raise ValueError("event frames must be uint8 [..., H, W, 2], got %s %s" % (a.dtype, a.shape))
  H, W = a.shape[-3], a.shape[-2]
  lead = a.shape[:-3]
  limit = 1 if fmt == L.EV1 else 15
  if a.size and int(a.max()) > limit:
    raise ValueError("event count %d does not fit the %s frame format (max %d)"
                     % (int(a.max()), "EV1" if fmt == L.EV1 else "EV4", limit))
  if fmt == L.EV1:
    flat = np.ascontiguousarray(a).reshape(lead + (H * W * 2,))
    b = np.packbits(flat, axis=-1, bitorder="little")
    nbytes = frame_units(H, W, fmt) * 4
    if b.shape[-1] != nbytes:
      b = np.concatenate([b, np.zeros(lead + (nbytes - b.shape[-1],), np.uint8)], -1)
    data = torch.from_numpy(np.ascontiguousarray(b).view(np.int32))
  else:
    data = torch.from_numpy(np.ascontiguousarray(a[..., 0] | (a[..., 1] << 4)).reshape(lead + (H * W,)))
  return PackedFrames(data, H, W, fmt)


def pack_frames(x: torch.Tensor, fmt: int, flags: Optional[torch.Tensor] = None) -> PackedFrames:
  _require_gpu(x, flags)
  assert x.dtype == torch.uint8 and x.shape[-1] == 2 and x.ndim >= 3, (x.dtype, tuple(x.shape))
  x = x.contiguous()
  H, W = x.shape[-3], x.shape[-2]
  lead = tuple(x.shape[:-3])
  frames = 1
  for d in lead:
    frames *= d
  data = torch.empty(lead + (frame_units(H, W, fmt),),
                     dtype=torch.int32 if fmt == L.EV1 else torch.uint8, device=x.device)
  L.check(L.lib().snnqp_pack_frames(_ptr(x), frames, H, W, fmt, _ptr(data), _ptr(flags), _stream()))
  return PackedFrames(data, H, W, fmt)


def pack_frames_checked(x: torch.Tensor) -> Tuple[PackedFrames, torch.Tensor]:
  _require_gpu(x)
  assert x.dtype in (torch.uint8, torch.float32) and x.shape[-1] == 2 and x.ndim >= 3, (x.dtype, tuple(x.shape))
  x = x.contiguous()
  H, W = x.shape[-3], x.shape[-2]
  lead = tuple(x.shape[:-3])
  frames = 1
  for d in lead:
    frames *= d
  data = torch.empty(lead + (frame_units(H, W, L.EV1),), dtype=torch.int32, device=x.device)
  flags = torch.empty(1, dtype=torch.int32, device=x.device)
  L.check(L.lib().snnqp_pack_frames_checked(_ptr(x), L.U8 if x.dtype == torch.uint8 else L.F32, frames, H, W,
                                            _ptr(data), _ptr(flags), _stream()))
  return PackedFrames(data, H, W, L.EV1), flags


def unpack_frames(p: PackedFrames) -> torch.Tensor:
  _require_gpu(p.data)
  lead = tuple(p.data.shape[:-1])
  frames = 1
  for d in lead:
    frames *= d
  y = torch.empty(lead + (p.H, p.W, 2), dtype=torch.uint8, device=p.device)
  L.check(L.lib().snnqp_unpack_frames(_ptr(p.data), p.fmt, frames, p.H, p.W, _ptr(y), _stream()))
  return y




def _stream():
  return ctypes.c_void_p(torch.cuda.current_stream().cuda_stream)


def _ptr(t: Optional[torch.Tensor]):
  return None if t is None else ctypes.c_void_p(t.data_ptr())


def _require_gpu(*ts):
  for t in ts:
    if t is None:
      continue
    if not t.is_cuda:
      raise RuntimeError(
          "snnquantprune_amd ops run on the GPU only (tensor on %s); there is no "
          "CPU fallback" % t.device)


def _f32c(t: torch.Tensor) -> torch.Tensor:
  if t.dtype != torch.float32:
    t = t.to(torch.float32)
  return t.contiguous()


def is_pow2(x: float) -> bool:
  import math
  if not (x > 0) or math.isinf(x):
    return False
  m, _ = math.frexp(x)
  return m == 0.5


@dataclass
class Weight:
  wtype: int
  w: torch.Tensor
  L: float = 1.0
  m: float = 1.0
  wt: Optional[torch.Tensor] = None
  abs_sum_max: int = 0
  code_max: int = 0
  min_current_bits: int = 0
  col_sum: Optional[torch.Tensor] = None
  wt6: Optional[torch.Tensor] = None
  ch_stack_max: int = 0
  ch_slots: Optional[torch.Tensor] = None
  wt_cin: int = 0

  def struct(self) -> L.WeightT:
    st = self.__dict__.get("_cstruct")
    if st is None:
      st = L.WeightT(self.wtype, self.w.data_ptr(), float(self.L), float(self.m),
                     int(self.abs_sum_max), int(self.code_max),
                     None if self.col_sum is None else self.col_sum.data_ptr(),
                     None if self.wt6 is None else self.wt6.data_ptr(),
                     int(self.min_current_bits), int(self.ch_stack_max),
                     None if self.ch_slots is None else self.ch_slots.data_ptr(), int(self.wt_cin))
      self.__dict__["_cstruct"] = st
    return st

  @property
  def is_int(self):
    return self.wtype == L.W_I8


@dataclass
class Neuron:
  kind: int
  k: float = 2.0
  v_threshold: float = 1.0
  v_reset: float = 0.0
  decay: Optional[torch.Tensor] = None

  def struct(self) -> L.NeuronT:
    return L.NeuronT(self.kind, float(self.k), float(self.v_threshold),
                     float(self.v_reset),
                     None if self.decay is None else self.decay.data_ptr())


@dataclass
class BnCoeffs:
  mean: torch.Tensor
  mul: torch.Tensor
  bias: torch.Tensor
  flags: int = 0

  def struct(self) -> L.BnT:
    return L.BnT(self.mean.data_ptr(), self.mul.data_ptr(), self.bias.data_ptr(), int(self.flags))


@dataclass
class ConvGeom:
  H: int
  W: int
  Cin: int
  Cout: int
  KH: int
  KW: int
  stride: Tuple[int, int] = (1, 1)
  pad: Tuple[Tuple[int, int], Tuple[int, int]] = ((0, 0), (0, 0))
  in_dil: Tuple[int, int] = (1, 1)
  k_dil: Tuple[int, int] = (1, 1)
  groups: int = 1

  def struct(self) -> L.ConvGeomT:
    return L.ConvGeomT(self.H, self.W, self.Cin, self.Cout, self.KH, self.KW,
                       self.stride[0], self.stride[1], self.pad[0][0],
                       self.pad[0][1], self.pad[1][0], self.pad[1][1],
                       self.in_dil[0], self.in_dil[1], self.k_dil[0],
                       self.k_dil[1], self.groups)

  def tag(self) -> str:
    return "%dx%dx%d->%d" % (self.H, self.W, self.Cin, self.Cout)

  def out_hw(self) -> Tuple[int, int]:
    oh, ow = ctypes.c_int32(), ctypes.c_int32()
    g = self.struct()
    L.check(L.lib().snnqp_conv_out_shape(ctypes.byref(g), ctypes.byref(oh),
                                         ctypes.byref(ow)))
    return oh.value, ow.value


@dataclass(frozen=True)
class Conv3dGeom:
  D: int
  H: int
  W: int
  Cin: int
  Cout: int
  KD: int
  KH: int
  KW: int
  stride: Tuple[int, int, int] = (1, 1, 1)
  pad: Tuple[Tuple[int, int], Tuple[int, int], Tuple[int, int]] = ((0, 0), (0, 0), (0, 0))
  in_dil: Tuple[int, int, int] = (1, 1, 1)
  k_dil: Tuple[int, int, int] = (1, 1, 1)
  groups: int = 1

  def struct(self) -> L.Conv3dGeomT:
    i3 = ctypes.c_int32 * 3
    return L.Conv3dGeomT(self.D, self.H, self.W, self.Cin, self.Cout, self.KD, self.KH, self.KW,
                         i3(*self.stride), i3(*[p[0] for p in self.pad]), i3(*[p[1] for p in self.pad]),
                         i3(*self.in_dil), i3(*self.k_dil), self.groups)

  def tag(self) -> str:
    return "%dx%dx%dx%d->%d" % (self.D, self.H, self.W, self.Cin, self.Cout)

  def out_dhw(self) -> Tuple[int, int, int]:
    od, oh, ow = ctypes.c_int32(), ctypes.c_int32(), ctypes.c_int32()
    g = self.struct()
    L.check(L.lib().snnqp_conv3d_out_shape(ctypes.byref(g), ctypes.byref(od), ctypes.byref(oh), ctypes.byref(ow)))
    return od.value, oh.value, ow.value


def _in_desc(x):
  if isinstance(x, PackedSpikes):
    return x.bits, L.BITS
  if isinstance(x, PackedFrames):
    return x.data, x.fmt
  if x.dtype == torch.uint8:
    return x, L.U8
  if x.dtype == torch.float32:
    return x, L.F32
  raise TypeError("activation dtype %s not supported (float32, uint8 or "
                  "PackedSpikes)" % x.dtype)




def quantize(kind: int, w: torch.Tensor, mask: Optional[torch.Tensor], bits: int,
             p0: float, p1: float = 0.0, want_fq: bool = True,
             want_codes: bool = False, sign: bool = True):
  w = _f32c(w)
  _require_gpu(w, mask)
  if mask is not None:
    mask = _f32c(mask)
    assert mask.shape == w.shape
  fq = torch.empty_like(w) if want_fq else None
  codes = torch.empty(w.shape, dtype=torch.int8, device=w.device) if want_codes else None
  flags = torch.zeros(1, dtype=torch.int32, device=w.device) if (
      want_codes or mask is not None) else None
  L.check(L.lib().snnqp_quantize_ex(kind, _ptr(w), _ptr(mask), w.numel(), int(bits), 1 if sign else 0,
                                    float(p0), float(p1), _ptr(fq), _ptr(codes),
                                    _ptr(flags), _stream()))
  return fq, codes, flags


def pack_codes_mfma(codes: torch.Tensor, n_pad: Optional[int] = None) -> torch.Tensor:
  _require_gpu(codes)
  assert codes.dtype == torch.int8
  c2 = codes.reshape(-1, codes.shape[-1]).contiguous()
  K, N = c2.shape
  n_pad = (N + 31) // 32 * 32 if n_pad is None else n_pad
  if K % 32:
    raise ValueError("MFMA tiling needs K % 32 == 0 (K = %d)" % K)
  wt = torch.empty((n_pad // 32, K // 32, 64, 16), dtype=torch.int8, device=codes.device)
  L.check(L.lib().snnqp_pack_codes_mfma(_ptr(c2), K, N, n_pad, _ptr(wt), _stream()))
  return wt


def pack_codes_fp6(codes: torch.Tensor, n_pad: Optional[int] = None) -> torch.Tensor:
  _require_gpu(codes)
  assert codes.dtype == torch.int8
  c2 = codes.reshape(-1, codes.shape[-1]).contiguous()
  K, N = c2.shape
  n_pad = (N + 31) // 32 * 32 if n_pad is None else n_pad
  wt6 = torch.empty((n_pad // 32, (K + 63) // 64, 1536), dtype=torch.uint8, device=codes.device)
  L.check(L.lib().snnqp_pack_codes_fp6(_ptr(c2), K, N, n_pad, _ptr(wt6), _stream()))
  return wt6




class NotCapturable(RuntimeError):
  """The step needs a value on the host and is being recorded into a hipGraph, which cannot wait
  for one.  (Nothing in this package does any more -- float32 inputs are checked on the device,
  snnqp.h x_flags -- the class stays for callers that catch it.)"""


@dataclass
class FloatFallback:
  weight: "Weight"
  x: Optional[torch.Tensor] = None
  pred: Optional[torch.Tensor] = None


def forget_inputs():
  """Kept for callers of earlier versions (bench.py called it each step to drop cached facts about
  the last batch): nothing about an activation tensor is cached on the host any more."""


class CountHint:

  BOUNDS = (1, 2, 3, 7, 31)
  COST = (1.0, 1.0, 1.0, 1.19, 1.19)
  GENERAL = 1.85

  def __init__(self, device):
    self.value = 1
    self.word = torch.zeros(8, dtype=torch.int32, device=device)
    self._host = torch.zeros(8, dtype=torch.int32).pin_memory()
    self._event = None
    self.max_seen = 0
    self.saw_counts = False

  def binary_so_far(self) -> bool:
    return self.current() == 1 and not self.saw_counts

  @staticmethod
  def capturing() -> bool:
    return torch.cuda.is_current_stream_capturing()

  @classmethod
  def choose(cls, words) -> int:
    w = list(words) + [0] * (6 - len(words))
    hist = [w[0], w[1], w[5], w[2] - w[5], w[3], w[4]]
    total = sum(hist)
    if total == 0:
      return 1
    best, best_cost = 255, cls.GENERAL * total
    below = 0
    for k, (bound, cost) in enumerate(zip(cls.BOUNDS, cls.COST)):
      below += hist[k]
      c = cost * below + cls.GENERAL * (total - below)
      if c < best_cost - 1e-9:
        best, best_cost = bound, c
    return best

  def current(self) -> int:
    if self.capturing():
      return self.value
    if self._event is not None and self._event.query():
      self._event = None
      words = [int(v) for v in self._host]
      self.max_seen = words[0]
      if self.max_seen > 1:
        self.saw_counts = True
      if sum(words[1:6]) > 0:
        self.value = max(1, min(self.choose(words[1:7]), self.max_seen))
    return self.value

  def seen_word(self):
    return None if self.capturing() else self.word

  def launched(self):
    if self.capturing():
      return
    if self._event is None:
      self._host.copy_(self.word, non_blocking=True)
      self.word.zero_()
      self._event = torch.cuda.Event()
      self._event.record()


_count_hints = {}


def count_hint(device) -> CountHint:
  key = torch.device(device).index if torch.device(device).index is not None else torch.cuda.current_device()
  h = _count_hints.get(key)
  if h is None:
    h = _count_hints[key] = CountHint(device)
  return h


def reset_count_hints(device=None):
  if device is None:
    _count_hints.clear()
  else:
    d = torch.device(device)
    _count_hints.pop(d.index if d.index is not None else torch.cuda.current_device(), None)


def f32_to_u8(x: torch.Tensor) -> torch.Tensor:
  x = _f32c(x)
  _require_gpu(x)
  y = torch.empty(x.shape, dtype=torch.uint8, device=x.device)
  L.check(L.lib().snnqp_f32_to_u8(_ptr(x), _ptr(y), x.numel(), _stream()))
  return y


def narrow_f32_async(x: torch.Tensor):
  x = _f32c(x)
  _require_gpu(x)
  y = torch.empty(x.shape, dtype=torch.uint8, device=x.device)
  flags = torch.zeros(2, dtype=torch.int32, device=x.device)
  L.check(L.lib().snnqp_narrow_f32(_ptr(x), _ptr(y), x.numel(), _ptr(flags), _stream()))
  return y, flags[1:2]


def pack_bits_checked(x: torch.Tensor):
  _require_gpu(x)
  if x.dtype not in (torch.float32, torch.uint8):
    x = x.to(torch.float32)
  x = x.contiguous()
  C = x.shape[-1]
  rows = x.numel() // C if C else 0
  bits = torch.empty(tuple(x.shape[:-1]) + ((C + 31) // 32,), dtype=torch.int32, device=x.device)
  flags = torch.zeros(1, dtype=torch.int32, device=x.device)
  L.check(L.lib().snnqp_pack_bits_checked(_ptr(x), L.F32 if x.dtype == torch.float32 else L.U8,
                                          rows, C, _ptr(bits), _ptr(flags), _stream()))
  return PackedSpikes(bits, C), flags


def pack_bits(x: torch.Tensor) -> PackedSpikes:
  _require_gpu(x)
  if x.dtype not in (torch.float32, torch.uint8):
    x = x.to(torch.float32)
  x = x.contiguous()
  C = x.shape[-1]
  rows = x.numel() // C if C else 0
  bits = torch.empty(tuple(x.shape[:-1]) + ((C + 31) // 32,), dtype=torch.int32,
                     device=x.device)
  L.check(L.lib().snnqp_pack_bits(_ptr(x), L.F32 if x.dtype == torch.float32 else L.U8,
                                  rows, C, _ptr(bits), _stream()))
  return PackedSpikes(bits, C)


def unpack_bits(s: PackedSpikes) -> torch.Tensor:
  _require_gpu(s.bits)
  y = torch.empty(s.shape, dtype=torch.float32, device=s.device)
  rows = y.numel() // s.channels
  L.check(L.lib().snnqp_unpack_bits(_ptr(s.bits), rows, s.channels, _ptr(y), _stream()))
  return y




def fseq_gemm_supported(geom: ConvGeom) -> bool:
  (pt, pb), (pl, pr) = geom.pad
  return (geom.groups == 1 and tuple(geom.stride) == (1, 1) and tuple(geom.in_dil) == (1, 1)
          and tuple(geom.k_dil) == (1, 1)
          and pt + pb == geom.KH - 1 and pl + pr == geom.KW - 1)


def conv_forward(x, geom: ConvGeom, weight: Weight, want_acc: bool = False):
  xt, in_type = _in_desc(x)
  xt = xt.contiguous()
  _require_gpu(xt, weight.w)
  NB = xt.shape[0]
  OH, OW = geom.out_hw()
  y = torch.empty((NB, OH, OW, geom.Cout), dtype=torch.float32, device=xt.device)
  acc = torch.empty(y.shape, dtype=torch.int32, device=xt.device) if want_acc else None
  g, w = geom.struct(), weight.struct()
  L.check(L.lib().snnqp_conv_forward(_ptr(xt), in_type, NB, ctypes.byref(g),
                                     ctypes.byref(w), _ptr(y), _ptr(acc), _stream()))
  return (y, acc) if want_acc else y


def conv3d_lif_forward(x, geom: Conv3dGeom, weight: Weight, neuron: Optional[Neuron] = None,
                       bn: Optional[BnCoeffs] = None, u0: Optional[torch.Tensor] = None, want_u: bool = True,
                       packed_out: bool = False, pred: Optional[torch.Tensor] = None, out=None):
  xt, in_type = _in_desc(x)
  xt = xt.contiguous()
  _require_gpu(xt, weight.w, u0)
  OD, OH, OW = geom.out_dhw()
  dev = xt.device
  unit = geom.D * geom.H * geom.W * xt.shape[-1]
  g, w = geom.struct(), weight.struct()
  b = bn.struct() if bn is not None else None
  if neuron is None:
    NB = xt.shape[0]
    y = out if out is not None else torch.empty((NB, OD, OH, OW, geom.Cout), dtype=torch.float32, device=dev)
    with _timed("conv3d[%s]" % geom.tag()):
      L.check(L.lib().snnqp_conv3d_lif_forward(_ptr(pred), _ptr(xt), in_type, 0, unit, 1, NB, ctypes.byref(g),
                                               ctypes.byref(w), None, None, None, None, _ptr(y), L.F32, _stream()))
    return y
  T, B = xt.shape[0], xt.shape[1]
  if out is not None:
    u_out, s = out
    s = s.bits if isinstance(s, PackedSpikes) else s
  else:
    u_out = torch.empty((B, OD, OH, OW, geom.Cout), dtype=torch.float32, device=dev) if want_u else None
    oshape = (T, B, OD, OH, OW)
    s = torch.empty(oshape + (((geom.Cout + 31) // 32,) if packed_out else (geom.Cout,)),
                    dtype=torch.int32 if packed_out else torch.float32, device=dev)
  if u0 is not None:
    u0 = _f32c(u0)
    assert tuple(u0.shape) == (B, OD, OH, OW, geom.Cout), (u0.shape, (B, OD, OH, OW, geom.Cout))
  _zero_step_carry(u_out, u0, T)
  n = neuron.struct()
  with _timed("conv3d[%s]" % geom.tag()):
    L.check(L.lib().snnqp_conv3d_lif_forward(_ptr(pred), _ptr(xt), in_type, B * unit, unit, T, B, ctypes.byref(g),
                                             ctypes.byref(w), ctypes.byref(b) if b is not None else None,
                                             ctypes.byref(n), _ptr(u0), _ptr(u_out), _ptr(s),
                                             L.BITS if packed_out else L.F32, _stream()))
  return u_out, (PackedSpikes(s, geom.Cout) if packed_out else s)


def conv_forward_speculative(x: torch.Tensor, geom: ConvGeom, int_weight: Weight, float_weight: Weight):
  x = _f32c(x)
  x8, pred = narrow_f32_async(x)
  y = conv_forward(x8, geom, int_weight)
  g, w = geom.struct(), float_weight.struct()
  L.check(L.lib().snnqp_conv_forward_if(_ptr(pred), _ptr(x), L.F32, x.shape[0], ctypes.byref(g), ctypes.byref(w),
                                        _ptr(y), _stream()))
  return y


def pack_codes_gated(codes: torch.Tensor, code_max: int = 7) -> torch.Tensor:
  _require_gpu(codes)
  assert codes.dtype == torch.int8 and codes.ndim == 4 and tuple(codes.shape[:2]) == (3, 3)
  codes = codes.contiguous()
  cin, cout = codes.shape[2], codes.shape[3]
  out = torch.empty(int(L.lib().snnqp_conv_gated_packed_bytes_ex(cin, cout, int(code_max))), dtype=torch.uint8,
                    device=codes.device)
  L.check(L.lib().snnqp_pack_codes_gated_ex(_ptr(codes), cin, cout, int(code_max), _ptr(out), _stream()))
  return out


def conv_gated_forward(x: GatedSpikes, geom: ConvGeom, weight: Weight, packed: torch.Tensor) -> torch.Tensor:
  bits, gate = x.spikes.bits.contiguous(), x.gate
  _require_gpu(bits, gate, weight.w, packed)
  T, B, H, W, _ = x.shape
  assert (H, W, x.spikes.channels) == (geom.H, geom.W, geom.Cin), (x.shape, geom)
  y = torch.empty((T, B, H, W, geom.Cout), dtype=torch.float32, device=bits.device)
  g, w = geom.struct(), weight.struct()
  with _timed("conv[gated %s]" % geom.tag()):
    L.check(L.lib().snnqp_conv_gated_forward(_ptr(bits), _ptr(gate), T * B, ctypes.byref(g), ctypes.byref(w),
                                             _ptr(packed), _ptr(y), _stream()))
  return y


def pack_codes_dense_gated(codes: torch.Tensor, C: int, HW: int, code_max: int = 7) -> torch.Tensor:
  _require_gpu(codes)
  assert codes.dtype == torch.int8 and codes.ndim == 2 and codes.shape[0] == C * HW
  codes = codes.contiguous()
  N = codes.shape[1]
  out = torch.empty(int(L.lib().snnqp_dense_gated_packed_bytes_ex(C, N, int(code_max))), dtype=torch.uint8,
                    device=codes.device)
  L.check(L.lib().snnqp_pack_codes_dense_gated_ex(_ptr(codes), C, HW, N, int(code_max), _ptr(out), _stream()))
  return out


def dense_gated_forward(x: GatedSpikes, weight: Weight, packed: torch.Tensor) -> torch.Tensor:
  bits, gate = x.spikes.bits.contiguous(), x.gate
  _require_gpu(bits, gate, weight.w, packed)
  T, B, H, W, C = x.spikes.shape
  N = weight.w.shape[-1]
  assert weight.w.shape[0] == C * H * W, (tuple(weight.w.shape), x.spikes.shape)
  y = torch.empty((T, B, N), dtype=torch.float32, device=bits.device)
  w = weight.struct()
  with _timed("dense[gated K=%d N=%d]" % (C * H * W, N)):
    L.check(L.lib().snnqp_dense_gated_forward(_ptr(bits), _ptr(gate), T * B, H * W, C, N, ctypes.byref(w),
                                              _ptr(packed), _ptr(y), _stream()))
  return y



_PROFILE = None
PROFILE_NOTES = {}


def profile_start():
  global _PROFILE
  _PROFILE = {}
  PROFILE_NOTES.clear()


def profile_stop():
  global _PROFILE
  prof, _PROFILE = _PROFILE or {}, None
  torch.cuda.synchronize()
  return {tag: (len(evs), sum(a.elapsed_time(b) for a, b in evs))
          for tag, evs in prof.items()}


class _timed:
  def __init__(self, tag):
    self.tag = tag

  def __enter__(self):
    if _PROFILE is not None:
      self.a = torch.cuda.Event(enable_timing=True)
      self.b = torch.cuda.Event(enable_timing=True)
      self.a.record()

  def __exit__(self, *exc):
    if _PROFILE is not None and exc[0] is None:
      self.b.record()
      _PROFILE.setdefault(self.tag, []).append((self.a, self.b))
    return False




_current_min_cache = None


def current_min_bits(weight: Weight, bn: Optional[BnCoeffs], bound: int, cout: int) -> int:
  global _current_min_cache
  if _current_min_cache is None:
    from ._cache import TensorCache
    _current_min_cache = TensorCache(64)
  key = (weight.w,) + ((bn.mean, bn.mul, bn.bias) if bn is not None else (None, None, None))
  extra = (int(bound), int(cout), float(weight.L), float(weight.m))
  v = _current_min_cache.get(key, extra)
  if v is None:
    _require_gpu(weight.w)
    out = torch.full((1,), 0x7F800000, dtype=torch.int32, device=weight.w.device)
    w = weight.struct()
    b = bn.struct() if bn is not None else None
    L.check(L.lib().snnqp_current_min(ctypes.byref(w), ctypes.byref(b) if b is not None else None,
                                      int(bound), int(cout), _ptr(out), _stream()))
    v = int(out.item()) & 0xFFFFFFFF
    _current_min_cache.put(key, extra, v)
  return v


def _tb_strides(x, T, B, time_major: bool, unit: int):
  if time_major:
    return B * unit, unit
  return unit, T * unit


def _zero_step_carry(u_out: Optional[torch.Tensor], u0: Optional[torch.Tensor], T: int):
  if u_out is not None and T == 0:
    if u0 is None:
      u_out.zero_()
    else:
      u_out.copy_(u0)


def conv_lif_forward(x, geom: ConvGeom, weight: Weight, neuron: Neuron,
                     bn: Optional[BnCoeffs] = None, u0: Optional[torch.Tensor] = None,
                     want_u: bool = True, packed_out: bool = False, pool: int = 1,
                     impl: int = L.IMPL_AUTO, time_major: bool = True, x_max: int = 0,
                     x_seen: Optional[torch.Tensor] = None,
                     fallback: Optional[FloatFallback] = None, binary_first: bool = False,
                     logical: Optional[Tuple[int, int, int]] = None):
  xt, in_type = _in_desc(x)
  xt = xt.contiguous()
  _require_gpu(xt, weight.w, u0)
  x_flags = None
  if in_type == L.F32 and weight.is_int:
    if fallback is None:
      raise ValueError("float32 input into integer codes needs a FloatFallback (the float32 kernel)")
    x_flags = torch.empty(1, dtype=torch.int32, device=xt.device)
  if x_seen is not None:
    assert x_seen.dtype == torch.int32 and x_seen.numel() >= 8 and x_seen.is_cuda, \
        "x_seen: eight int32 device words (snnqp.h)"
  T, B = (xt.shape[0], xt.shape[1]) if time_major else (xt.shape[1], xt.shape[0])
  if isinstance(x, PackedFrames):
    assert (x.H, x.W, 2) == (geom.H, geom.W, geom.Cin) and xt.ndim == 3, (x.shape, geom)
    unit = xt.shape[-1]
  else:
    unit = geom.H * geom.W * (xt.shape[-1])
  xs_t, xs_b = _tb_strides(xt, T, B, time_major, unit)
  OH, OW = geom.out_hw()
  dev = xt.device
  u_out = torch.empty((B, OH, OW, geom.Cout), dtype=torch.float32, device=dev) \
      if want_u else None
  if u0 is not None:
    u0 = _f32c(u0)
    assert tuple(u0.shape) == (B, OH, OW, geom.Cout), (u0.shape, (B, OH, OW, geom.Cout))
  _zero_step_carry(u_out, u0, T)
  oshape = (T, B, OH // pool, OW // pool)
  if packed_out:
    s = torch.empty(oshape + ((geom.Cout + 31) // 32,), dtype=torch.int32, device=dev)
  else:
    s = torch.empty(oshape + (geom.Cout,), dtype=torch.float32, device=dev)
  g, w, n = geom.struct(), weight.struct(), neuron.struct()
  b = bn.struct() if bn is not None else None
  cin_l, cout_l = (geom.Cin, geom.Cout) if logical is None else logical[:2]
  tag = "conv%dx%d[%dx%dx%d->%d]" % (geom.KH, geom.KW, geom.H, geom.W, cin_l, cout_l)
  if _PROFILE is not None and in_type == L.BITS and weight.is_int and "dequant" not in PROFILE_NOTES.get(tag, {}):
    PROFILE_NOTES.setdefault(tag, {})["dequant"] = conv_dequant_form(weight, neuron)
  if _PROFILE is not None and logical is not None:
    PROFILE_NOTES.setdefault(tag, {})["channels"] = {
        "cin": geom.Cin, "cout": geom.Cout, "live_out": int(logical[2])}
  speculate = (binary_first and packed_out and not isinstance(x, (PackedFrames, PackedSpikes))
               and in_type in (L.U8, L.F32) and geom.Cin == 2 and weight.is_int and impl != L.IMPL_GENERIC
               and xt.ndim == 5)
  with _timed(tag):
    if speculate:
      pf, not_binary = pack_frames_checked(xt)
      ps_t, ps_b = _tb_strides(pf.data, T, B, time_major, pf.data.shape[-1])
      try:
        L.check(L.lib().snnqp_conv_lif_forward(
            _ptr(pf.data), L.EV1, ps_t, ps_b, T, B, ctypes.byref(g), ctypes.byref(w),
            _ptr(weight.wt), ctypes.byref(b) if b is not None else None, ctypes.byref(n),
            _ptr(u0), _ptr(u_out), _ptr(s), L.BITS, pool, impl, 1, None, None, _stream()))
      except L.SnnqpError as e:
        if e.code != L.EUNSUPPORTED:
          raise
        speculate = False
    if speculate:
      L.check(L.lib().snnqp_conv_lif_forward_pred(
          _ptr(not_binary), _ptr(xt), in_type, xs_t, xs_b, T, B, ctypes.byref(g), ctypes.byref(w),
          _ptr(weight.wt), ctypes.byref(b) if b is not None else None, ctypes.byref(n),
          _ptr(u0), _ptr(u_out), _ptr(s), L.BITS, pool,
          int(x_max), _ptr(x_seen), _ptr(x_flags), _stream()))
    else:
      L.check(L.lib().snnqp_conv_lif_forward(
          _ptr(xt), in_type, xs_t, xs_b, T, B, ctypes.byref(g), ctypes.byref(w),
          _ptr(weight.wt), ctypes.byref(b) if b is not None else None, ctypes.byref(n),
          _ptr(u0), _ptr(u_out), _ptr(s), L.BITS if packed_out else L.F32, pool, impl,
          int(x_max), _ptr(x_seen), _ptr(x_flags), _stream()))
  if fallback is not None:
    xf = _f32c(xt if fallback.x is None else fallback.x)
    pred = x_flags if fallback.pred is None else fallback.pred
    fw = fallback.weight.struct()
    fs_t, fs_b = _tb_strides(xf, T, B, time_major, geom.H * geom.W * geom.Cin)
    L.check(L.lib().snnqp_conv_lif_forward_if(
        _ptr(pred), _ptr(xf), L.F32, fs_t, fs_b, T, B, ctypes.byref(g), ctypes.byref(fw),
        ctypes.byref(b) if b is not None else None, ctypes.byref(n), _ptr(u0), _ptr(u_out), _ptr(s),
        L.BITS if packed_out else L.F32, pool, _stream()))
  return u_out, (PackedSpikes(s, geom.Cout) if packed_out else s)


def dense_lif_forward(x, weight: Weight, K: int, N: int, neuron: Neuron,
                      bn: Optional[BnCoeffs] = None, u0: Optional[torch.Tensor] = None,
                      want_u: bool = True, packed_out: bool = False,
                      impl: int = L.IMPL_AUTO, time_major: bool = True,
                      fallback: Optional[FloatFallback] = None):
  xt, in_type = _in_desc(x)
  xt = xt.contiguous()
  _require_gpu(xt, weight.w, u0)
  x_flags = None
  if in_type == L.F32 and weight.is_int:
    if fallback is None:
      raise ValueError("float32 rows into integer codes need a FloatFallback (the float32 kernel)")
    x_flags = torch.empty(1, dtype=torch.int32, device=xt.device)
  T, B = (xt.shape[0], xt.shape[1]) if time_major else (xt.shape[1], xt.shape[0])
  xs_t, xs_b = _tb_strides(xt, T, B, time_major, xt.shape[-1])
  dev = xt.device
  u_out = torch.empty((B, N), dtype=torch.float32, device=dev) if want_u else None
  if u0 is not None:
    u0 = _f32c(u0)
    assert tuple(u0.shape) == (B, N)
  _zero_step_carry(u_out, u0, T)
  if packed_out:
    s = torch.empty((T, B, (N + 31) // 32), dtype=torch.int32, device=dev)
  else:
    s = torch.empty((T, B, N), dtype=torch.float32, device=dev)
  w, n = weight.struct(), neuron.struct()
  b = bn.struct() if bn is not None else None
  ws = _dense_workspace(dev, int(L.lib().snnqp_dense_workspace_bytes(in_type, T, B, K, N, ctypes.byref(w)))) \
      if (packed_out and impl != L.IMPL_GENERIC) else None
  with _timed("dense[%d->%d]" % (K, N)):
    L.check(L.lib().snnqp_dense_lif_forward_ws(
        _ptr(xt), in_type, xs_t, xs_b, T, B, K, N, ctypes.byref(w), _ptr(weight.wt),
        ctypes.byref(b) if b is not None else None, ctypes.byref(n), _ptr(u0),
        _ptr(u_out), _ptr(s), L.BITS if packed_out else L.F32, impl, _ptr(x_flags),
        _ptr(ws), 0 if ws is None else ws.numel(), _stream()))
  if fallback is not None:
    xf = _f32c(xt if fallback.x is None else fallback.x)
    pred = x_flags if fallback.pred is None else fallback.pred
    fw = fallback.weight.struct()
    L.check(L.lib().snnqp_dense_lif_forward_if(
        _ptr(pred), _ptr(xf), L.F32, xs_t, xs_b, T, B, K, N, ctypes.byref(fw),
        ctypes.byref(b) if b is not None else None, ctypes.byref(n), _ptr(u0), _ptr(u_out), _ptr(s),
        L.BITS if packed_out else L.F32, _stream()))
  return u_out, (PackedSpikes(s, N) if packed_out else s)


_dense_ws = {}
_CAPTURE_KEEP = None


def _dense_workspace(dev, nbytes: int):
  if nbytes <= 0:
    return None
  if torch.cuda.is_current_stream_capturing():
    ws = torch.empty(nbytes, dtype=torch.uint8, device=dev)
    if _CAPTURE_KEEP is not None:
      _CAPTURE_KEEP.append(ws)
    return ws
  key = (torch.device(dev).index, torch.cuda.current_stream(dev).cuda_stream)
  ws = _dense_ws.get(key)
  if ws is None or ws.numel() < nbytes:
    ws = _dense_ws[key] = torch.zeros(nbytes, dtype=torch.uint8, device=dev)
  return ws


def dense_head_forward(x, w1: Weight, K: int, N1: int, nrn1: Neuron, w2: Weight, N2: int,
                       nrn2: Neuron, group: int = 10, want_s1: bool = False,
                       want_s2: bool = False, time_major: bool = True,
                       fallback: Optional[FloatFallback] = None):
  xt, in_type = _in_desc(x)
  xt = xt.contiguous()
  _require_gpu(xt, w1.w, w2.w)
  T, B = (xt.shape[0], xt.shape[1]) if time_major else (xt.shape[1], xt.shape[0])
  xs_t, xs_b = _tb_strides(xt, T, B, time_major, xt.shape[-1])
  dev = xt.device
  if N2 % group:
    raise ValueError("vote: %d features not divisible by group %d" % (N2, group))
  logits = torch.empty((B, N2 // group), dtype=torch.float32, device=dev)
  x_flags = None
  if in_type == L.F32:
    if fallback is None or fallback.x is not None:
      raise ValueError("float32 rows into the fused head need a FloatFallback of the first block")
    x_flags = torch.empty(1, dtype=torch.int32, device=dev)
  elif fallback is not None:
    raise ValueError("a FloatFallback goes with float32 rows; uint8 / bit-packed rows have nothing to redo")
  redo = in_type == L.F32
  s1 = torch.empty((T, B, (N1 + 31) // 32), dtype=torch.int32, device=dev) if (want_s1 or redo) else None
  s2 = torch.empty((T, B, (N2 + 31) // 32), dtype=torch.int32, device=dev) if (want_s2 or redo) else None
  a, b, n1, n2 = w1.struct(), w2.struct(), nrn1.struct(), nrn2.struct()
  nws = _head_ws_bytes.get((T, B, N1))
  if nws is None:
    nws = _head_ws_bytes[(T, B, N1)] = int(L.lib().snnqp_dense_head_workspace_bytes(T, B, N1))
  ws = _dense_workspace(dev, nws)
  with _timed("dense_head[%d->%d->%d]" % (K, N1, N2)):
    L.check(L.lib().snnqp_dense_head_forward(
        _ptr(xt), in_type, xs_t, xs_b, T, B, K, N1, ctypes.byref(a), _ptr(w1.wt), ctypes.byref(n1),
        N2, ctypes.byref(b), _ptr(w2.wt), ctypes.byref(n2), int(group),
        _ptr(s1) if (want_s1 or redo) else None, _ptr(s2) if (want_s2 or redo) else None,
        _ptr(logits), _ptr(x_flags), _ptr(ws), 0 if ws is None else ws.numel(), _stream()))
  if redo:
    fw = fallback.weight.struct()
    lib = L.lib()
    L.check(lib.snnqp_dense_lif_forward_if(_ptr(x_flags), _ptr(xt), L.F32, xs_t, xs_b, T, B, K, N1,
                                           ctypes.byref(fw), None, ctypes.byref(n1), None, None, _ptr(s1),
                                           L.BITS, _stream()))
    cw1 = (N1 + 31) // 32
    L.check(lib.snnqp_dense_lif_forward_if(_ptr(x_flags), _ptr(s1), L.BITS, B * cw1, cw1, T, B, N1, N2,
                                           ctypes.byref(b), None, ctypes.byref(n2), None, None, _ptr(s2),
                                           L.BITS, _stream()))
    L.check(lib.snnqp_vote_if(_ptr(x_flags), _ptr(s2), L.BITS, T, B, N2, int(group), _ptr(logits), _stream()))
  return (logits, PackedSpikes(s1, N1) if want_s1 else None,
          PackedSpikes(s2, N2) if want_s2 else None)


_head_ws_bytes = {}


def fallback_counts(reset: bool = False) -> dict:
  conv, dense = ctypes.c_int64(), ctypes.c_int64()
  buf = ctypes.create_string_buffer(256)
  L.check(L.lib().snnqp_fallback_counts(ctypes.byref(conv), ctypes.byref(dense), buf, 256,
                                        1 if reset else 0))
  return {"conv_blocks": conv.value, "dense_blocks": dense.value,
          "last_reason": buf.value.decode("utf-8", "replace")}


def device_status(device=None, reset: bool = False) -> int:
  dev = torch.cuda.current_device() if device is None else torch.device(device).index
  code = ctypes.c_uint32()
  L.check(L.lib().snnqp_device_status(int(dev or 0), ctypes.byref(code), 1 if reset else 0))
  return int(code.value)


def workqueue_stats(reset: bool = False) -> dict:
  a, b, c = ctypes.c_int64(), ctypes.c_int64(), ctypes.c_int64()
  L.check(L.lib().snnqp_workqueue_stats(ctypes.byref(a), ctypes.byref(b), ctypes.byref(c), 1 if reset else 0))
  return {"captured_static_walks": a.value, "busy_static_walks": b.value, "dequant_table_fallbacks": c.value}


def workqueue_capture_mark(device) -> int:
  m = ctypes.c_int64()
  L.check(L.lib().snnqp_workqueue_capture_mark(int(torch.device(device).index or 0), ctypes.byref(m)))
  return int(m.value)


def workqueue_capture_release(device, begin: int, end: int):
  L.check(L.lib().snnqp_workqueue_capture_release(int(torch.device(device).index or 0), int(begin), int(end)))


DQ_FORMS = {1: "arith", 2: "one", 3: "table"}


def conv_dequant_form(w: Weight, nrn: Neuron) -> str:
  ws, ns = w.struct(), nrn.struct()
  rc = L.lib().snnqp_conv_dequant_form(ctypes.byref(ws), ctypes.byref(ns))
  if rc < 0:
    L.check(rc)
  return DQ_FORMS[rc]




def lif_forward(x: torch.Tensor, neuron: Neuron, bn: Optional[BnCoeffs] = None,
                u0: Optional[torch.Tensor] = None, want_u: bool = True,
                packed_out: bool = False):
  x = _f32c(x)
  _require_gpu(x, u0)
  T, C = x.shape[0], x.shape[-1]
  R = (x.numel() // (T * C)) if T * C else 0
  u_out = torch.empty(x.shape[1:], dtype=torch.float32, device=x.device) if want_u else None
  if u0 is not None:
    u0 = _f32c(u0)
    assert tuple(u0.shape) == tuple(x.shape[1:])
  _zero_step_carry(u_out, u0, T)
  if packed_out:
    s = torch.empty(tuple(x.shape[:-1]) + ((C + 31) // 32,), dtype=torch.int32,
                    device=x.device)
  else:
    s = torch.empty_like(x)
  n = neuron.struct()
  b = bn.struct() if bn is not None else None
  L.check(L.lib().snnqp_lif_forward(
      _ptr(x), T, R, C, ctypes.byref(b) if b is not None else None, ctypes.byref(n),
      _ptr(u0), _ptr(u_out), _ptr(s), L.BITS if packed_out else L.F32, _stream()))
  return u_out, (PackedSpikes(s, C) if packed_out else s)


def batchnorm_forward(x: torch.Tensor, bn: BnCoeffs) -> torch.Tensor:
  x = _f32c(x)
  _require_gpu(x)
  C = x.shape[-1]
  y = torch.empty_like(x)
  b = bn.struct()
  L.check(L.lib().snnqp_batchnorm_forward(_ptr(x), x.numel() // C if C else 0, C,
                                          ctypes.byref(b), _ptr(y), _stream()))
  return y


def maxpool2x2(x):
  if isinstance(x, PackedSpikes):
    bits = x.bits
    _require_gpu(bits)
    H, W = bits.shape[-3], bits.shape[-2]
    lead = tuple(bits.shape[:-3])
    NB = 1
    for d in lead:
      NB *= d
    y = torch.empty(lead + (H // 2, W // 2, bits.shape[-1]), dtype=torch.int32,
                    device=bits.device)
    L.check(L.lib().snnqp_maxpool2x2(_ptr(bits), L.BITS, NB, H, W, x.channels, _ptr(y),
                                     _stream()))
    return PackedSpikes(y, x.channels)
  x = _f32c(x)
  _require_gpu(x)
  H, W, C = x.shape[-3:]
  lead = tuple(x.shape[:-3])
  NB = 1
  for d in lead:
    NB *= d
  y = torch.empty(lead + (H // 2, W // 2, C), dtype=torch.float32, device=x.device)
  L.check(L.lib().snnqp_maxpool2x2(_ptr(x), L.F32, NB, H, W, C, _ptr(y), _stream()))
  return y


def spatial_mean(x) -> torch.Tensor:
  if isinstance(x, PackedSpikes):
    t, typ, C = x.bits, L.BITS, x.channels
  else:
    t, typ, C = _f32c(x), L.F32, x.shape[-1]
  _require_gpu(t)
  lead = tuple(t.shape[:-3])
  HW = t.shape[-3] * t.shape[-2]
  NB = 1
  for d in lead:
    NB *= d
  y = torch.empty(lead + (C,), dtype=torch.float32, device=t.device)
  L.check(L.lib().snnqp_spatial_mean(_ptr(t), typ, NB, HW, C, _ptr(y), _stream()))
  return y


def sigmoid_gate(a: torch.Tensor, b: torch.Tensor) -> torch.Tensor:
  a, b = _f32c(a), _f32c(b)
  _require_gpu(a, b)
  assert a.shape == b.shape
  g = torch.empty_like(a)
  L.check(L.lib().snnqp_sigmoid_gate(_ptr(a), _ptr(b), a.numel(), _ptr(g), _stream()))
  return g


def apply_gate(x, g: torch.Tensor) -> torch.Tensor:
  if isinstance(x, PackedSpikes):
    t, typ, C = x.bits, L.BITS, x.channels
  else:
    t, typ, C = _f32c(x), L.F32, x.shape[-1]
  g = _f32c(g)
  _require_gpu(t, g)
  lead = tuple(t.shape[:-3])
  H, W = t.shape[-3], t.shape[-2]
  assert tuple(g.shape) == lead + (C,), (g.shape, lead, C)
  NB = 1
  for d in lead:
    NB *= d
  y = torch.empty(lead + (H, W, C), dtype=torch.float32, device=t.device)
  L.check(L.lib().snnqp_apply_gate(_ptr(t), typ, _ptr(g), NB, H * W, C, _ptr(y), _stream()))
  return y


def events_to_frames(x, y, p, T: int, H: int, W: int, scale: float = 1.0, as_u8=True):
  x = x.to(torch.int32).contiguous()
  y = y.to(torch.int32).contiguous()
  p = p.to(torch.int32).contiguous()
  _require_gpu(x, y, p)
  counts = torch.empty((T, H, W, 2), dtype=torch.int32, device=x.device)
  u8 = torch.empty((T, H, W, 2), dtype=torch.uint8, device=x.device) if as_u8 else None
  L.check(L.lib().snnqp_events_to_frames(_ptr(x), _ptr(y), _ptr(p), x.numel(), T, H, W,
                                         float(scale), _ptr(counts), _ptr(u8), _stream()))
  return u8 if as_u8 else counts


def density(x, lead_dims: int = 2, counts: bool = False) -> torch.Tensor:
  if isinstance(x, PackedFrames):
    x = unpack_frames(x)
  if isinstance(x, GatedSpikes):
    x = x.to_dense()
  if isinstance(x, PackedSpikes):
    t, typ, C, shape = x.bits, L.BITS, x.channels, x.shape
  elif x.dtype == torch.uint8:
    t, typ, C, shape = x.contiguous(), L.U8, x.shape[-1], tuple(x.shape)
  else:
    t, typ, C, shape = _f32c(x), L.F32, x.shape[-1], tuple(x.shape)
  _require_gpu(t)
  lead = tuple(shape[:lead_dims])
  NB = 1
  for d in lead:
    NB *= d
  n = 1
  for d in shape[lead_dims:]:
    n *= d
  nnz = torch.empty(lead, dtype=torch.int32, device=t.device)
  L.check(L.lib().snnqp_density(_ptr(t), typ, NB, n, C, _ptr(nnz), _stream()))
  if counts:
    return nnz
  return nnz.to(torch.float32) / float(n)


def vote(s, group: int = 10) -> torch.Tensor:
  if isinstance(s, PackedSpikes):
    t, typ, N = s.bits, L.BITS, s.channels
  else:
    t, typ, N = _f32c(s), L.F32, s.shape[-1]
  _require_gpu(t)
  T, B = t.shape[0], t.shape[1]
  if N % group:
    raise ValueError("vote: %d features not divisible by group %d" % (N, group))
  out = torch.empty((B, N // group), dtype=torch.float32, device=t.device)
  L.check(L.lib().snnqp_vote(_ptr(t), typ, T, B, N, group, _ptr(out), _stream()))
  return out




def lif_forward_save(x: torch.Tensor, neuron: Neuron):
  x = _f32c(x)
  _require_gpu(x)
  T, C = x.shape[0], x.shape[-1]
  R = (x.numel() // (T * C)) if T * C else 0
  h = torch.empty_like(x)
  s = torch.empty_like(x)
  L.check(L.lib().snnqp_lif_forward_save(_ptr(x), T, R, C, ctypes.byref(neuron.struct()),
                                         _ptr(h), _ptr(s), _stream()))
  return h, s


def lif_backward(h: torch.Tensor, neuron: Neuron, surrogate: int, gs: Optional[torch.Tensor] = None,
                 glogits: Optional[torch.Tensor] = None, group: int = 10) -> torch.Tensor:
  h = _f32c(h)
  gs = None if gs is None else _f32c(gs)
  glogits = None if glogits is None else _f32c(glogits)
  _require_gpu(h, gs, glogits)
  T, C = h.shape[0], h.shape[-1]
  R = (h.numel() // (T * C)) if T * C else 0
  gI = torch.empty_like(h)
  L.check(L.lib().snnqp_lif_backward(_ptr(h), _ptr(gs), _ptr(glogits), int(group), T, R, C,
                                     ctypes.byref(neuron.struct()), int(surrogate), _ptr(gI),
                                     _stream()))
  return gI


def dense_weight_grad(x: torch.Tensor, gI: torch.Tensor) -> torch.Tensor:
  x, gI = _f32c(x), _f32c(gI)
  _require_gpu(x, gI)
  M, K = x.shape
  N = gI.shape[1]
  assert gI.shape[0] == M
  gw = torch.empty((K, N), dtype=torch.float32, device=x.device)
  L.check(L.lib().snnqp_dense_weight_grad(_ptr(x), _ptr(gI), M, K, N, _ptr(gw), _stream()))
  return gw


def dense_input_grad(gI: torch.Tensor, w: torch.Tensor, mask: Optional[torch.Tensor] = None) -> torch.Tensor:
  gI, w = _f32c(gI), _f32c(w)
  mask = None if mask is None else _f32c(mask)
  _require_gpu(gI, w, mask)
  M, N = gI.shape
  K = w.shape[0]
  assert w.shape[1] == N and (mask is None or tuple(mask.shape) == (M, K))
  gx = torch.empty((M, K), dtype=torch.float32, device=gI.device)
  L.check(L.lib().snnqp_dense_input_grad(_ptr(gI), _ptr(w), _ptr(mask), M, K, N, _ptr(gx),
                                         _stream()))
  return gx
```

Before: 93800 samples/s.

## Trim event-input conv3x3 workgroups to live output waves and shrink output ring

New measurement: 93980 samples/s, median of 4. No clear change (+0.2%).

```diff
diff --git a/include/snnqp.h b/include/snnqp.h
--- a/include/snnqp.h
+++ b/include/snnqp.h
@@ -101,7 +101,7 @@
   int32_t groups;
 } snnqp_conv3d_geom_t;
 
-#define SNNQP_VERSION 505
+#define SNNQP_VERSION 506
 int snnqp_version(void);
 const char *snnqp_last_error(void);
 const char *snnqp_build_flags(void);
@@ -185,6 +185,11 @@
                            int impl, int x_max, int32_t *x_seen, int32_t *x_flags,
                            snnqp_stream_t stream);
 
+int snnqp_set_event_wave_trim(int on);
+int snnqp_conv_event_launch_shape(int in_type, int32_t T, const snnqp_conv_geom_t *g,
+                                  const snnqp_weight_t *w, const snnqp_neuron_t *nrn,
+                                  int carries_u, int pool, int x_max, int device, int32_t *shape);
+
 int snnqp_conv_lif_forward_pred(const int32_t *pred, const void *x, int in_type, int64_t x_stride_t,
                                 int64_t x_stride_b, int32_t T, int32_t B,
                                 const snnqp_conv_geom_t *g, const snnqp_weight_t *w,
diff --git a/snnquantprune_amd/_lib.py b/snnquantprune_amd/_lib.py
--- a/snnquantprune_amd/_lib.py
+++ b/snnquantprune_amd/_lib.py
@@ -9,7 +9,7 @@
 _HERE = os.path.dirname(os.path.abspath(__file__))
 LIB_PATH = os.path.join(_HERE, "csrc", "libsnnqp.so")
 
-ABI_VERSION = 505
+ABI_VERSION = 506
 
 F32, U8, BITS, EV1, EV4 = 0, 1, 2, 3, 4
 W_F32, W_I8 = 0, 1
@@ -141,6 +141,9 @@
     "snnqp_debug_workqueue_poke": (c_int, [c_int, c_int64, c_int, c_uint32]),
     "snnqp_fallback_counts": (c_int, [POINTER(c_int64), POINTER(c_int64), c_char_p, c_int32, c_int]),
     "snnqp_conv_dequant_form": (c_int, [POINTER(WeightT), POINTER(NeuronT)]),
+    "snnqp_set_event_wave_trim": (c_int, [c_int]),
+    "snnqp_conv_event_launch_shape": (c_int, [c_int, c_int32, POINTER(ConvGeomT), POINTER(WeightT), POINTER(NeuronT),
+                                              c_int, c_int, c_int, c_int, POINTER(c_int32)]),
     "snnqp_current_min": (c_int, [POINTER(WeightT), POINTER(BnT), c_int32, c_int32, c_void_p, c_void_p]),
     "snnqp_lif_forward": (c_int, [c_void_p, c_int32, c_int64, c_int32, POINTER(BnT),
                                   POINTER(NeuronT), c_void_p, c_void_p, c_void_p,
diff --git a/snnquantprune_amd/csrc/conv3x3_u8c2.hip b/snnquantprune_amd/csrc/conv3x3_u8c2.hip
--- a/snnquantprune_amd/csrc/conv3x3_u8c2.hip
+++ b/snnquantprune_amd/csrc/conv3x3_u8c2.hip
@@ -36,12 +36,13 @@
 #ifndef SNNQP_U8C2_EV1_ONE_WPS
 #define SNNQP_U8C2_EV1_ONE_WPS 6
 #endif
+constexpr int u8c2_waves_of(int nf, bool pool, int lutm, int in, bool one) {
+  if (in == SNNQP_EV1 && one && lutm == LUT_CHANNEL && nf == NF_MUL0 && pool) return SNNQP_U8C2_EV1_ONE_WPS;
+  if (in == SNNQP_EV1) return SNNQP_U8C2_EV1_WPS;
+  return one ? SNNQP_U8C2_ONE_WPS : U8C2_WPS;
+}
 template <int NF, bool POOL, int LUTM, int IN, bool ONE>
-constexpr int u8c2_waves() {
-  if (IN == SNNQP_EV1 && ONE && LUTM == LUT_CHANNEL && NF == NF_MUL0 && POOL) return SNNQP_U8C2_EV1_ONE_WPS;
-  if (IN == SNNQP_EV1) return SNNQP_U8C2_EV1_WPS;
-  return ONE ? SNNQP_U8C2_ONE_WPS : U8C2_WPS;
-}
+constexpr int u8c2_waves() { return u8c2_waves_of(NF, POOL, LUTM, IN, ONE); }
 template <int NF, bool POOL, int LUTM, int IN = SNNQP_U8, bool ONE = false>
 __global__ void __launch_bounds__(256, (u8c2_waves<NF, POOL, LUTM, IN, ONE>()))
 conv3x3_u8c2_kernel(ConvMfmaArgs a) {
@@ -58,6 +59,8 @@
   const int lut_off = tc * HIMG2;
   uint32_t *obuf = (uint32_t *)(lds + lut_off + u8c2_table_bytes(LUTM, a.lut_bound, a.lut_rows));
   const int tid = threadIdx.x, lane = tid & 63;
+  const int nthr = EV1 ? (int)blockDim.x : 256;
+  const int ring_w = EV1 ? a.ring_w : 4;
   const int wave = __builtin_amdgcn_readfirstlane(tid >> 6);
   const int n = lane & 31, h = lane >> 5;
   const int cout_base = blockIdx.y * 128 + wave * 32;
@@ -65,17 +68,21 @@
   const int cout = wave_on ? cout_base + n : n;
   const int cpar = cout < a.Cout ? cout : a.Cout - 1;
   const uint32_t cmask = chan_mask(cout_base, a.Cout);
-  uint32_t *wgw = obuf + OutStage<POOL>::BYTES / 4;
+  uint32_t *wgw = obuf + (EV1 ? a.ring_words : OutStage<POOL>::BYTES / 4);
   if (tid == 0) { wgw[0] = 0x7F800000u; wgw[1] = 0u; }
+  if (EV1 && LUTM == LUT_CHANNEL)
+    for (int i = tid; i < 128; i += nthr) obuf[i] = 0u;
   typedef int v2i_a8 __attribute__((ext_vector_type(2)));
   v2i_a8 *xtab = (v2i_a8 *)(wgw + 4);
   if (EV1) {
     const uint32_t one = LUTM == LUT_CHANNEL ? 16u : LUTM == LUT_SHARED ? 4u : 0x81u;
     const uint32_t zero = LUTM == LUT_NONE ? 0x80u : 0u;
-    uint32_t e[2] = {0, 0};
-#pragma unroll
-    for (int j = 0; j < 8; ++j) e[j >> 2] |= (((uint32_t)tid >> j) & 1u ? one : zero) << (8 * (j & 3));
-    xtab[tid] = v2i_a8{(int)e[0], (int)e[1]};
+    for (int i = tid; i < 256; i += nthr) {
+      uint32_t e[2] = {0, 0};
+#pragma unroll
+      for (int j = 0; j < 8; ++j) e[j >> 2] |= (((uint32_t)i >> j) & 1u ? one : zero) << (8 * (j & 3));
+      xtab[i] = v2i_a8{(int)e[0], (int)e[1]};
+    }
   }
   if (LUTM != LUT_NONE) lds_barrier();
   if (LUTM == LUT_SHARED) {
@@ -117,7 +124,7 @@
     ch_row0 = start + neg * a.x_limit;
     if (total > a.lut_rows && a.status) *(volatile uint32_t *)a.status = SNNQP_STATUS_BOUND;
     const uint32_t mb = build_lut_channel((float *)(lds + lut_off), scr, a.lut_rows, a.dq, a.bn,
-                                          blockIdx.y * 128, a.Cout, tid);
+                                          blockIdx.y * 128, a.Cout, tid, nthr);
     atomicMin(wgw, mb);
     lds_barrier();
   }
@@ -185,8 +192,7 @@
     offB[tl] = h ? (int)lds_addr(lds) + HCONST2 : px0 + (ty + 4 * tl + 1) * HROW2;
   }
   const uint8_t *xb = (const uint8_t *)a.x;
-  const int ob0 = out_pix<POOL>(0, lane) * 4 + wave;
-  const int ob1 = out_pix<POOL>(1, lane) * 4 + wave;
+  const int ob0 = out_pix<POOL>(0, lane) * ring_w + wave;
   const bool store_lane = POOL ? lane < 8 : lane < 32;
   uint32_t seen = 0;
   uint32_t hist[6] = {0, 0, 0, 0, 0, 0};
@@ -226,7 +232,7 @@
       bool general = LUTM == LUT_NONE;
       if constexpr (EV1) {
         lds_barrier();
-        for (int task = tid; task < nt * HALO; task += 256) {
+        for (int task = tid; task < nt * HALO; task += nthr) {
           const int tt = task / HALO, hy = task - tt * HALO;
           const int gy = y0 + hy - 1;
           const bool rv = gy >= 0 && gy < a.H;
@@ -379,13 +385,13 @@
                                                                      lane, acc_off);
           }
           if (store_lane) {
-            uint32_t *o = obuf + ((t0 + tt) % FL) * (OutStage<POOL>::NPIX * 4);
+            uint32_t *o = obuf + ((t0 + tt) % FL) * (OutStage<POOL>::NPIX * ring_w);
             o[ob0] = words[0] & cmask;
-            o[ob0 + (POOL ? 32 : 128)] = words[1] & cmask;
+            o[ob0 + (POOL ? 8 : 32) * ring_w] = words[1] & cmask;
           }
         }
         lds_barrier();
-        flush_out<POOL>(obuf, a, t0 + tf, nf, b, y0, x0, tid);
+        flush_out<POOL>(obuf, a, t0 + tf, nf, b, y0, x0, tid, nthr, ring_w);
         lds_barrier();
       }
       };
@@ -581,7 +587,7 @@
       occ = 1;
     }
     if (occ < 1) occ = 1;
-    if (occ > 8) occ = 8;
+    if (occ > 16) occ = 16;
     it = cache.emplace(key, std::make_pair(cus, occ)).first;
   }
   *cus_out = it->second.first;
@@ -642,6 +648,98 @@
   const bool tab = fp6 && neuron_form(make_neuron(nrn)) == NF_MUL0 && w->abs_sum_max > 0 &&
                    w->abs_sum_max <= DQT_MAXA;
   return tab ? DQ_TABLE : DQ_ARITH;
+}
+
+namespace {
+std::atomic<int> g_event_wave_trim{1};
+
+struct U8c2Plan {
+  int lm = LUT_NONE, lut_bound = 0, lut_rows = 0, x_limit = 1;
+  int nf = NF_MUL0;
+  bool one = false, trimmed = false;
+  int threads = 256, ring_w = 4, ring_bytes = 0, tchunk = 0;
+  int wgs = 1;
+  size_t lds = 0;
+};
+
+typedef void (*u8c2_kernel_t)(ConvMfmaArgs);
+
+template <int NFV, bool PL, int LM>
+u8c2_kernel_t u8c2_kernel_in(int in_type, bool one) {
+  if (in_type == SNNQP_EV1) return one ? conv3x3_u8c2_kernel<NFV, PL, LM, SNNQP_EV1, true> : conv3x3_u8c2_kernel<NFV, PL, LM, SNNQP_EV1>;
+  if (in_type == SNNQP_EV4) return one ? conv3x3_u8c2_kernel<NFV, PL, LM, SNNQP_EV4, true> : conv3x3_u8c2_kernel<NFV, PL, LM, SNNQP_EV4>;
+  if (in_type == SNNQP_F32) return one ? conv3x3_u8c2_kernel<NFV, PL, LM, SNNQP_F32, true> : conv3x3_u8c2_kernel<NFV, PL, LM, SNNQP_F32>;
+  return one ? conv3x3_u8c2_kernel<NFV, PL, LM, SNNQP_U8, true> : conv3x3_u8c2_kernel<NFV, PL, LM, SNNQP_U8>;
+}
+template <int NFV, bool PL>
+u8c2_kernel_t u8c2_kernel_lm(int lm, int in_type, bool one) {
+  if (lm == LUT_CHANNEL) return u8c2_kernel_in<NFV, PL, LUT_CHANNEL>(in_type, one);
+  if (lm == LUT_SHARED) return u8c2_kernel_in<NFV, PL, LUT_SHARED>(in_type, one);
+  return u8c2_kernel_in<NFV, PL, LUT_NONE>(in_type, one);
+}
+template <int NFV>
+u8c2_kernel_t u8c2_kernel_pl(bool pl, int lm, int in_type, bool one) {
+  return pl ? u8c2_kernel_lm<NFV, true>(lm, in_type, one) : u8c2_kernel_lm<NFV, false>(lm, in_type, one);
+}
+u8c2_kernel_t u8c2_kernel_of(const U8c2Plan &p, int in_type, bool pl) {
+  if (p.nf == NF_MUL0) return u8c2_kernel_pl<NF_MUL0>(pl, p.lm, in_type, p.one);
+  if (p.nf == NF_MUL) return u8c2_kernel_pl<NF_MUL>(pl, p.lm, in_type, p.one);
+  if (p.nf == NF_DIV) return u8c2_kernel_pl<NF_DIV>(pl, p.lm, in_type, p.one);
+  return u8c2_kernel_pl<NF_DECAY>(pl, p.lm, in_type, p.one);
+}
+
+U8c2Plan plan_u8c2(int in_type, int T, int Cout, const snnqp_weight_t *w, const snnqp_neuron_t *nrn,
+                   bool carries_u, bool pl, int x_max) {
+  U8c2Plan p;
+  p.nf = neuron_form(make_neuron(nrn));
+  const bool ev1 = in_type == SNNQP_EV1;
+  const int64_t xm = ev1 ? 1 : (x_max > 0 ? x_max : 1);
+  p.x_limit = (int)(xm > 255 ? 255 : xm);
+  const int64_t bound = (int64_t)w->abs_sum_max * xm;
+  const bool lut = w->abs_sum_max > 0 && xm > 0 && xm <= LUT_XMAX && bound <= LUT_CAP;
+  p.lut_bound = lut ? (int)bound : 0;
+  const int64_t stack = w->ch_stack_max > 0 ? (int64_t)w->ch_stack_max : 8 * (int64_t)w->abs_sum_max;
+  const int64_t crows = stack * xm + 4;
+  const bool lutc = lut && crows <= LUT2_ROWS && xm <= 7 && w->code_max > 0 && w->code_max <= 15;
+  p.lut_rows = lutc ? (int)crows : 0;
+  p.lm = lutc ? LUT_CHANNEL : lut ? LUT_SHARED : LUT_NONE;
+  const int nw = (Cout + 31) / 32;
+  p.trimmed = ev1 && Cout <= 96 && g_event_wave_trim.load(std::memory_order_relaxed) != 0;
+  p.threads = p.trimmed ? 64 * nw : 256;
+  p.ring_w = p.trimmed ? nw : 4;
+  const int FL = pl ? OutStage<true>::FL : OutStage<false>::FL;
+  const int NPIX = pl ? OutStage<true>::NPIX : OutStage<false>::NPIX;
+  const int tc0 = T >= TCHUNK ? TCHUNK : T;
+  auto fit = [&](bool one) {
+    p.one = one;
+    p.ring_bytes = FL * NPIX * 16;
+    if (p.trimmed) {
+      p.ring_bytes = (one ? (T < FL ? T : FL) : FL) * NPIX * 4 * nw;
+      if (p.ring_bytes < 1536) p.ring_bytes = 1536;
+    }
+    const size_t rest = u8c2_table_bytes(p.lm, p.lut_bound, p.lut_rows) + (size_t)p.ring_bytes + 16 + (ev1 ? 2048 : 0);
+    int top = 4;
+    if (p.trimmed) {
+      top = 4 * u8c2_waves_of(p.nf, pl, p.lm, in_type, one) / nw;
+      if (top > 16) top = 16;
+    }
+    int tc = tc0;
+    for (int wgs = top; wgs >= 2; --wgs) {
+      const size_t per_wg = (size_t)(160 * 1024) / wgs - 512;
+      const int floor_tc = wgs > 4 && T <= TCHUNK ? tc0 : 16;
+      tc = tc0;
+      while (tc > floor_tc && (size_t)tc * HIMG2 + rest > per_wg) tc -= 1;
+      p.wgs = wgs;
+      if ((size_t)tc * HIMG2 + rest <= per_wg) break;
+      if (wgs == 2) { tc = tc0; p.wgs = 1; }
+    }
+    p.tchunk = tc;
+    p.lds = (size_t)tc * HIMG2 + rest;
+  };
+  fit(!carries_u && T <= tc0);
+  if (p.one && T > p.tchunk) fit(false);
+  return p;
+}
 }
 
 int run_conv3x3_mfma(const void *x, int in_type, int64_t xs_t, int64_t xs_b,
@@ -688,44 +786,12 @@
   const int nf = neuron_form(a.nrn);
   const bool pl = pool == 2;
   const unsigned gy = (unsigned)((g->Cout + 127) / 128);
-  const bool ev1 = in_type == SNNQP_EV1;
-  const int64_t xm = (in_type == SNNQP_BITS || ev1) ? 1 : (x_max > 0 ? x_max : 1);
-  a.x_limit = (int32_t)(xm > 255 ? 255 : xm);
-  const int64_t bound = (int64_t)w->abs_sum_max * xm;
-  const bool lut = w->abs_sum_max > 0 && xm > 0 && xm <= LUT_XMAX && bound <= LUT_CAP;
-  a.lut_bound = lut ? (int32_t)bound : 0;
+  a.x_limit = 1;
+  a.lut_bound = a.lut_rows = 0;
+  a.ch_slots = nullptr;
   a.tchunk = T >= TCHUNK ? TCHUNK : T;
-  const size_t lds_fixed = (size_t)a.tchunk * HIMG2 + 16 + (ev1 ? 2048 : 0) +
-                           (pl ? OutStage<true>::BYTES : OutStage<false>::BYTES);
-  const int64_t stack = w->ch_stack_max > 0 ? (int64_t)w->ch_stack_max : 8 * (int64_t)w->abs_sum_max;
-  const int64_t crows = stack * xm + 4;
-  const bool lutc = lut && in_type != SNNQP_BITS && crows <= LUT2_ROWS && xm <= 7 &&
-                    w->code_max > 0 && w->code_max <= 15;
-  a.lut_rows = lutc ? (int32_t)crows : 0;
-  a.ch_slots = lutc && w->ch_stack_max > 0 ? w->ch_slots : nullptr;
-#define SNNQP_CONV_LAUNCH_IN(KERN, NFV, PL, LM, LDS)                               \
-  do {                                                                             \
-    if (ev1 && one) launch_persistent(KERN<NFV, PL, LM, SNNQP_EV1, true>, a, gy, st, LDS); \
-    else if (ev1) launch_persistent(KERN<NFV, PL, LM, SNNQP_EV1>, a, gy, st, LDS);       \
-    else if (in_type == SNNQP_EV4 && one) launch_persistent(KERN<NFV, PL, LM, SNNQP_EV4, true>, a, gy, st, LDS); \
-    else if (in_type == SNNQP_EV4) launch_persistent(KERN<NFV, PL, LM, SNNQP_EV4>, a, gy, st, LDS); \
-    else if (in_type == SNNQP_F32 && one) launch_persistent(KERN<NFV, PL, LM, SNNQP_F32, true>, a, gy, st, LDS); \
-    else if (in_type == SNNQP_F32) launch_persistent(KERN<NFV, PL, LM, SNNQP_F32>, a, gy, st, LDS); \
-    else if (one) launch_persistent(KERN<NFV, PL, LM, SNNQP_U8, true>, a, gy, st, LDS);            \
-    else launch_persistent(KERN<NFV, PL, LM, SNNQP_U8>, a, gy, st, LDS);            \
-  } while (0)
-#define SNNQP_CONV_LAUNCH_NF(KERN, NFV, LM, LDS)                                   \
-  do {                                                                             \
-    if (pl) SNNQP_CONV_LAUNCH_IN(KERN, NFV, true, LM, LDS);                         \
-    else SNNQP_CONV_LAUNCH_IN(KERN, NFV, false, LM, LDS);                           \
-  } while (0)
-#define SNNQP_CONV_LAUNCH(KERN, LM, LDS)                                           \
-  do {                                                                             \
-    if (nf == NF_MUL0) SNNQP_CONV_LAUNCH_NF(KERN, NF_MUL0, LM, LDS);                \
-    else if (nf == NF_MUL) SNNQP_CONV_LAUNCH_NF(KERN, NF_MUL, LM, LDS);             \
-    else if (nf == NF_DIV) SNNQP_CONV_LAUNCH_NF(KERN, NF_DIV, LM, LDS);             \
-    else SNNQP_CONV_LAUNCH_NF(KERN, NF_DECAY, LM, LDS);                             \
-  } while (0)
+  a.ring_w = 4;
+  a.ring_words = 0;
   if (in_type == SNNQP_BITS) {
     const bool fma = nf == NF_MUL0 && w->min_current_bits != 0 && w->abs_sum_max > 0 &&
                      lif_fma_is_exact(w->min_current_bits, a.nrn.k_log2, T, u0 != nullptr);
@@ -740,32 +806,53 @@
                                    w->abs_sum_max, st);
     launch_conv3x3_bits(a, cin_pad, i8, nf, pl, dq, fma, bnf, gy, st);
   } else {
-    const int lm = lutc ? LUT_CHANNEL : lut ? LUT_SHARED : LUT_NONE;
-    if (lut) check_code_bound_once(stream_device(st), (const int8_t *)w->w, (int64_t)9 * g->Cin, g->Cout,
-                                   w->abs_sum_max, st);
-    const size_t lds_rest = lds_fixed - (size_t)a.tchunk * HIMG2 + u8c2_table_bytes(lm, a.lut_bound, a.lut_rows);
-    for (int wgs = 4; wgs >= 2; --wgs) {
-      const size_t per_wg = (size_t)(160 * 1024) / wgs - 512;
-      int tc = a.tchunk;
-      while (tc > 16 && (size_t)tc * HIMG2 + lds_rest > per_wg) tc -= 1;
-      if ((size_t)tc * HIMG2 + lds_rest <= per_wg) {
-        a.tchunk = tc;
-        break;
-      }
-    }
-    const size_t ldsb = (size_t)a.tchunk * HIMG2 + lds_rest;
-    const bool one = !a.u0 && !a.u_out && a.T <= a.tchunk;
-    if (lutc) SNNQP_CONV_LAUNCH(conv3x3_u8c2_kernel, LUT_CHANNEL, ldsb);
-    else if (lut) SNNQP_CONV_LAUNCH(conv3x3_u8c2_kernel, LUT_SHARED, ldsb);
-    else SNNQP_CONV_LAUNCH(conv3x3_u8c2_kernel, LUT_NONE, ldsb);
-  }
-#undef SNNQP_CONV_LAUNCH
-#undef SNNQP_CONV_LAUNCH_NF
-#undef SNNQP_CONV_LAUNCH_IN
+    const U8c2Plan p = plan_u8c2(in_type, T, gy == 1 ? g->Cout : 128 * (int)gy, w, nrn, u0 || u_out, pl, x_max);
+    a.x_limit = p.x_limit;
+    a.lut_bound = p.lut_bound;
+    a.lut_rows = p.lut_rows;
+    a.ch_slots = p.lm == LUT_CHANNEL && w->ch_stack_max > 0 ? w->ch_slots : nullptr;
+    a.tchunk = p.tchunk;
+    a.ring_w = p.ring_w;
+    a.ring_words = p.ring_bytes / 4;
+    if (p.lm != LUT_NONE) check_code_bound_once(stream_device(st), (const int8_t *)w->w, (int64_t)9 * g->Cin, g->Cout,
+                                                w->abs_sum_max, st);
+    launch_persistent(u8c2_kernel_of(p, in_type, pl), a, gy, st, p.lds, p.threads);
+  }
   SNNQP_CHECK_LAUNCH("conv3x3 mfma kernel");
   return SNNQP_OK;
 }
 
+}
+
+extern "C" int snnqp_set_event_wave_trim(int on) {
+  return snnqp::g_event_wave_trim.exchange(on != 0, std::memory_order_relaxed);
+}
+
+extern "C" int snnqp_conv_event_launch_shape(int in_type, int32_t T, const snnqp_conv_geom_t *g,
+                                             const snnqp_weight_t *w, const snnqp_neuron_t *nrn,
+                                             int carries_u, int pool, int x_max, int device,
+                                             int32_t *shape) {
+  using namespace snnqp;
+  SNNQP_REQUIRE(g && w && nrn && shape && T > 0 && (pool == 1 || pool == 2), SNNQP_EINVAL,
+                "conv_event_launch_shape: bad argument");
+  SNNQP_REQUIRE(in_type == SNNQP_U8 || in_type == SNNQP_EV1 || in_type == SNNQP_EV4 || in_type == SNNQP_F32,
+                SNNQP_EUNSUPPORTED, "conv_event_launch_shape: not an input format of the event layer");
+  if (const char *why = conv3x3_mfma_unsupported(in_type, g, w, nullptr, nrn, SNNQP_BITS)) {
+    set_error("conv_event_launch_shape: %s", why);
+    return SNNQP_EUNSUPPORTED;
+  }
+  const int gy = (g->Cout + 127) / 128;
+  const U8c2Plan p = plan_u8c2(in_type, T, gy == 1 ? g->Cout : 128 * gy, w, nrn, carries_u != 0, pool == 2, x_max);
+  int wgs = p.wgs;
+  if (device >= 0) {
+    int cus = 0;
+    persistent_limits((const void *)u8c2_kernel_of(p, in_type, pool == 2), p.threads, p.lds, device, &cus, &wgs);
+  }
+  shape[0] = p.threads;
+  shape[1] = (int32_t)p.lds;
+  shape[2] = wgs;
+  shape[3] = p.tchunk;
+  return SNNQP_OK;
 }
 
 extern "C" int snnqp_workqueue_capture_mark(int device, int64_t *mark) {
diff --git a/snnquantprune_amd/csrc/conv_tile.h b/snnquantprune_amd/csrc/conv_tile.h
--- a/snnquantprune_amd/csrc/conv_tile.h
+++ b/snnquantprune_amd/csrc/conv_tile.h
@@ -57,6 +57,8 @@
   uint32_t *status;
   int32_t patch_h;
   const int32_t *pred;
+  int32_t ring_w;
+  int32_t ring_words;
 };
 
 constexpr int SCHED_Y = 8;
@@ -184,21 +186,24 @@
 }
 __device__ __forceinline__ uint32_t build_lut_channel(float *lut, const uint32_t *scr, int max_rows,
                                                       const Dequant &dq, const BnP &bn, int cout0,
-                                                      int Cout, int tid) {
+                                                      int Cout, int tid, int nthreads = 256) {
   uint32_t minbits = 0x7F800000u;
-  const int c = tid & 127, hf = tid >> 7;
-  const int slot = (int)scr[256 + c], col = slot >> 2;
-  const int st = lut_column_start(scr, slot);
-  const int rows = (int)scr[slot], negx = (int)scr[128 + c];
-  if (st + rows > max_rows) return minbits;
-  const int co = cout0 + c < Cout ? cout0 + c : Cout - 1;
-  float bm = 0.f, bmul = 1.f, bb = 0.f;
-  if (bn.mean) { bm = bn.mean[co]; bmul = bn.mul[co]; bb = bn.bias[co]; }
-  for (int i = hf; i < rows; i += 2) {
-    const float y = bn_apply(dequant_acc_nb(i - negx, dq), bm, bmul, bb);
-    lut[(st + i) * 32 + col] = y;
-    const uint32_t mag = __float_as_uint(y) & 0x7FFFFFFFu;
-    if (mag != 0u && mag < minbits) minbits = mag;
+  {
+    const int nch = nthreads >> 1;
+    const int c = tid < nch ? tid : tid - nch, hf = tid < nch ? 0 : 1;
+    const int slot = (int)scr[256 + c], col = slot >> 2;
+    const int st = lut_column_start(scr, slot);
+    const int rows = (int)scr[slot], negx = (int)scr[128 + c];
+    if (st + rows > max_rows) return minbits;
+    const int co = cout0 + c < Cout ? cout0 + c : Cout - 1;
+    float bm = 0.f, bmul = 1.f, bb = 0.f;
+    if (bn.mean) { bm = bn.mean[co]; bmul = bn.mul[co]; bb = bn.bias[co]; }
+    for (int i = hf; i < rows; i += 2) {
+      const float y = bn_apply(dequant_acc_nb(i - negx, dq), bm, bmul, bb);
+      lut[(st + i) * 32 + col] = y;
+      const uint32_t mag = __float_as_uint(y) & 0x7FFFFFFFu;
+      if (mag != 0u && mag < minbits) minbits = mag;
+    }
   }
   return minbits;
 }
@@ -369,17 +374,18 @@
 
 template <bool POOL, int SLOTS, int NT, int NPIX = OutStage<POOL>::NPIX>
 __device__ __forceinline__ void flush_ring(const uint32_t *obuf, const ConvMfmaArgs &a,
-                                           int t0, int n, int b, int y0, int x0, int tid) {
+                                           int t0, int n, int b, int y0, int x0, int tid,
+                                           int nthreads = NT, int wstride = 4) {
   constexpr int PW = POOL ? 4 : 8;
   const int CW = (a.Cout + 31) >> 5;
   const int cwb = blockIdx.y * 4;
   const int nw = min(4, CW - cwb);
   const int OH = POOL ? a.H >> 1 : a.H, OW = POOL ? a.W >> 1 : a.W;
   const int oy0 = POOL ? y0 >> 1 : y0, ox0 = POOL ? x0 >> 1 : x0;
-  for (int i = tid; i < n * NPIX; i += NT) {
+  for (int i = tid; i < n * NPIX; i += nthreads) {
     const int slot = i / NPIX, pix = i % NPIX;
     const int t = t0 + slot;
-    const uint32_t *src = obuf + ((t % SLOTS) * NPIX + pix) * 4;
+    const uint32_t *src = obuf + ((t % SLOTS) * NPIX + pix) * wstride;
     const int oy = oy0 + pix / PW, ox = ox0 + pix % PW;
     if (oy >= OH || ox >= OW) continue;
     uint32_t *dst = a.s_out + ((((int64_t)t * a.B + b) * OH + oy) * OW + ox) * CW + cwb;
@@ -393,8 +399,9 @@
 
 template <bool POOL>
 __device__ __forceinline__ void flush_out(const uint32_t *obuf, const ConvMfmaArgs &a,
-                                          int t0, int n, int b, int y0, int x0, int tid) {
-  flush_ring<POOL, OutStage<POOL>::FL, 256>(obuf, a, t0, n, b, y0, x0, tid);
+                                          int t0, int n, int b, int y0, int x0, int tid,
+                                          int nthreads = 256, int wstride = 4) {
+  flush_ring<POOL, OutStage<POOL>::FL, 256>(obuf, a, t0, n, b, y0, x0, tid, nthreads, wstride);
 }
 
 template <bool LOAD>
diff --git a/snnquantprune_amd/linen.py b/snnquantprune_amd/linen.py
--- a/snnquantprune_amd/linen.py
+++ b/snnquantprune_amd/linen.py
@@ -110,6 +110,11 @@
 
 def conv_kpack() -> bool:
   return _CONV_KPACK
+
+
+def set_event_wave_trim(enabled: bool) -> bool:
+  from . import _lib
+  return bool(_lib.lib().snnqp_set_event_wave_trim(int(bool(enabled))))
 
 
 def check_compute_dtype(dtype, who: str):
diff --git a/snnquantprune_amd/ops.py b/snnquantprune_amd/ops.py
--- a/snnquantprune_amd/ops.py
+++ b/snnquantprune_amd/ops.py
@@ -871,6 +871,14 @@
   speculate = (binary_first and packed_out and not isinstance(x, (PackedFrames, PackedSpikes))
                and in_type in (L.U8, L.F32) and geom.Cin == 2 and weight.is_int and impl != L.IMPL_GENERIC
                and xt.ndim == 5)
+  if (_PROFILE is not None and geom.Cin == 2 and weight.is_int and in_type in (L.U8, L.EV1, L.EV4, L.F32)
+      and impl != L.IMPL_GENERIC and "waves" not in PROFILE_NOTES.get(tag, {})):
+    try:
+      shape = conv_event_launch_shape(L.EV1 if speculate else in_type, T, geom, weight, neuron,
+                                      u0 is not None or want_u, pool, 1 if speculate else x_max, dev.index or 0)
+      PROFILE_NOTES.setdefault(tag, {}).update(waves=shape["waves"], wgs_per_cu=shape["wgs_per_cu"])
+    except L.SnnqpError:
+      pass
   with _timed(tag):
     if speculate:
       pf, not_binary = pack_frames_checked(xt)
@@ -1068,6 +1076,17 @@
   return DQ_FORMS[rc]
 
 
+def conv_event_launch_shape(in_type: int, T: int, geom, w: Weight, nrn: Neuron, carries_u: bool = False,
+                            pool: int = 1, x_max: int = 0, device: int = -1) -> dict:
+  g, ws, ns = geom.struct(), w.struct(), nrn.struct()
+  shape = (ctypes.c_int32 * 4)()
+  L.check(L.lib().snnqp_conv_event_launch_shape(int(in_type), int(T), ctypes.byref(g), ctypes.byref(ws),
+                                                ctypes.byref(ns), int(bool(carries_u)), int(pool), int(x_max),
+                                                int(device), shape))
+  return {"threads": shape[0], "waves": shape[0] // 64, "lds_bytes": shape[1], "wgs_per_cu": shape[2],
+          "tchunk": shape[3]}
+
+
 
 
 def lif_forward(x: torch.Tensor, neuron: Neuron, bn: Optional[BnCoeffs] = None,
```
